# Kkuntal990/video-to-video-diffusion

Measured on AMD Instinct MI355X. Metric: ddim_steps_per_sec, higher is better.
Workload: dtype bf16; 1 GPU; DDIM-50 step (U-Net eval + update) on latent [1, 8, 48, 128, 128] = 8->48 slices @512x512, effective 264.66M U-Net (128x(1,2,4,4), latent 8), one volume per GPU, hipGraph-captured step; volumes_per_gpu=1, parallelism=dp1, full=False, finite_outputs=True

## Files before the change

include/ctsi.h:

```cpp
#ifndef CTSI_H
#define CTSI_H

#include <stddef.h>
#include <stdint.h>

#ifdef __cplusplus
extern "C" {
#endif

#define CTSI_OK 0
#define CTSI_ERR_INVALID (-1)
#define CTSI_ERR_UNSUPPORTED (-2)
#define CTSI_ERR_HIP (-3)

int ctsi_version(void);
int ctsi_ablation_build(void);
const char* ctsi_last_error(void);
int ctsi_device_available(void);

int ctsi_ncdhw_f32_to_ndhwc_bf16(const float* src, void* dst, int n, int c, int d, int h, int w,
                                 int c_total, int c_off, void* stream);
int ctsi_ndhwc_bf16_to_ncdhw_f32(const void* src, float* dst, int n, int c, int d, int h, int w,
                                 void* stream);
int ctsi_ncdhw_f32_to_ndhwc_f32(const float* src, float* dst, int n, int c, int d, int h, int w,
                                void* stream);
int ctsi_ndhwc_f32_to_ncdhw_f32(const float* src, float* dst, int n, int c, int d, int h, int w,
                                void* stream);

typedef struct ctsi_conv_plan ctsi_conv_plan;

typedef struct ctsi_conv_desc {
    int transposed;
    int kd, kh, kw;
    int sh, sw;
    int pd, ph, pw;
    int n, c1, c2;
    int cout;
    int di, hi, wi;
    int halo_d;
} ctsi_conv_desc;

typedef struct ctsi_conv_out {
    void* y;
    int mode;
    int cout_stride;
    int c_off;
    long long sn, sc, sd, sh, sw;
    int act;
    float* colsum;
    const void* gn_x;
    const double* gn_sums;
    const float* gn_gamma;
    const float* gn_beta;
    int gn_groups;
    float gn_eps;
    long long gn_count;
    int gn_silu;
    void* workspace;
} ctsi_conv_out;

int ctsi_conv_plan_create(ctsi_conv_plan** plan, const ctsi_conv_desc* desc);
int ctsi_conv_plan_set_weight_cin(ctsi_conv_plan* plan, int cin_w);
int ctsi_conv_plan_set_stream_tail(ctsi_conv_plan* plan, int on);
void ctsi_conv_plan_destroy(ctsi_conv_plan* plan);
int ctsi_conv_plan_out_dims(const ctsi_conv_plan* plan, int* d_out, int* h_out, int* w_out);
size_t ctsi_conv_plan_weight_bytes(const ctsi_conv_plan* plan);
int ctsi_conv_plan_tiles(const ctsi_conv_plan* plan);
int ctsi_conv_plan_tiles_per_sample(const ctsi_conv_plan* plan);
int ctsi_conv_plan_cout_pad(const ctsi_conv_plan* plan);
size_t ctsi_conv_plan_workspace_bytes(const ctsi_conv_plan* plan);
double ctsi_conv_plan_flops(const ctsi_conv_plan* plan);
int ctsi_conv_plan_config(const ctsi_conv_plan* plan, int* bm, int* bn, int* mode);
int ctsi_conv_plan_form(const ctsi_conv_plan* plan, int out[8]);
#define CTSI_PACK_GATHER 1
#define CTSI_PACK_GATHER_SMALL 2
#define CTSI_PACK_HALO 3
#define CTSI_PACK_K32 4
#define CTSI_PACK_HEAD 5
#define CTSI_PACK_STREAM_TAIL 6
#define CTSI_PACK_STEM 7
int ctsi_conv_plan_pack_layout(const ctsi_conv_plan* plan);
int ctsi_conv_plan_pack_weights(const ctsi_conv_plan* plan, const float* w_f32, void* packed,
                                void* stream);
int ctsi_conv_fwd(const ctsi_conv_plan* plan, const void* x1, const void* x2, const void* packed_w,
                  const float* bias, const ctsi_conv_out* out, void* stream);

int ctsi_gn_colsum(const void* x_bf16, float* colsum, int n, int c, int d, int h, int w,
                   int* tiles_per_sample, void* stream);
int ctsi_gn_colsum_tiles(int d, int h, int w);
int ctsi_gn_finalize(const float* colsum, double* sums, int n, int c, int c_pad, int groups,
                     int tiles_per_sample, int nclass, int accumulate, void* stream);
int ctsi_gn_apply(const void* x_bf16, void* y_bf16, const double* sums, const float* gamma,
                  const float* beta, int n, int c, int d, int h, int w, int d_stat, int groups, float eps,
                  int silu_pre, const float* tbias, int tbias_stride, const int* step_ptr,
                  const void* residual_bf16, int silu_post, void* stream);

int ctsi_attn_pv_supported(int c, int groups);
int ctsi_attn_pv(const float* depthsum, const double* sums, const float* gamma, const float* beta, const void* w_bf16,
                 const float* bias, void* out, int n, int c, int d, int h, int w, int groups, float eps, void* stream);

int ctsi_attn_depthsum(const void* x_bf16, float* depthsum, float* colsum, int n, int c, int d,
                       int h, int w, void* stream);
int ctsi_attn_depthsum_tiles(int c, int h, int w);
int ctsi_attn_normsum(const float* depthsum, const double* sums, const float* gamma,
                      const float* beta, void* out_bf16, int n, int c, int d, int h, int w,
                      int groups, float eps, void* stream);
int ctsi_attn_broadcast_add(const void* x_bf16, const void* p_bf16, const float* rowsum, int heads,
                            void* y_bf16, int n, int c, int d, int h, int w, void* stream);
int ctsi_attn_softmax_rowsum(const void* qk_bf16, float* rowsum, int n, int c, int d, int h, int w,
                             int heads, void* stream);

int ctsi_attn_core(const void* qkv_bf16, void* out_bf16, int n, int c, int d, int h, int w, int heads, void* stream);
int ctsi_attn_core_bwd(const void* qkv_bf16, const void* da_bf16, void* dqkv_bf16, int n, int c, int d, int h, int w, int heads,
                       void* stream);

int ctsi_attn_plane(const void* qkv_bf16, void* out_bf16, float* lse, int n, int c, int d, int h, int w, int heads, void* stream);
int ctsi_attn_plane_bwd(const void* qkv_bf16, const void* out_bf16, const void* da_bf16, const float* lse,
                        void* dqkv_bf16, int n, int c, int d, int h, int w, int heads, void* stream);

int ctsi_time_embed_fwd(const int* t_rows, int rows, int dim, int time_dim, const float* w1,
                        const float* b1, const float* w2, const float* b2, const float* w_all,
                        const float* b_all, int total_out, float* scratch, float* tbias_out,
                        void* stream);

int ctsi_time_embed_fwd_tf(const float* t_rows, int rows, int dim, int time_dim, const float* w1,
                           const float* b1, const float* w2, const float* b2, const float* w_all,
                           const float* b_all, int total_out, float* scratch, float* tbias_out,
                           void* stream);

int ctsi_trilinear_depth_fwd(const float* src_f32_ncdhw, void* dst_bf16_ndhwc, int n, int c,
                             int d_in, int d_out, int h, int w, int c_total, int c_off,
                             float* dst_f32_ncdhw, void* stream);

int ctsi_ddim_step(float* z, const float* eps, const float* noise_ncdhw, void* zin_bf16,
                   int c_total, int c_off, const float* coef, const int* step_ptr, int n, int c,
                   int d, int h, int w, int* nonfinite, void* stream);
int ctsi_ddpm_step(float* z, const float* eps, const float* noise_ncdhw, void* zin_bf16,
                   int c_total, int c_off, const float* coef, const int* step_ptr, int n, int c,
                   int d, int h, int w, void* stream);
int ctsi_ddpm_posterior(const float* z, const float* eps, const float* noise, float* z0_out, float* out,
                        const float* coef, int n, long long per_sample, int clip, void* stream);
int ctsi_step_advance(int* step_ptr, void* stream);
int ctsi_nan_to_num_f32(float* x, long long count, void* stream);
int ctsi_count_nonfinite_f32(float* x, long long count, int sanitize, int* counts, void* stream);

typedef struct ctsi_wgrad_desc {
    int kd, kh, kw;
    int sh, sw;
    int pd, ph, pw;
    int n;
    int dr, hr, wr;
    int dg, hg, wg;
    int cr, cr_stride;
    int cg, cg_stride;
} ctsi_wgrad_desc;
size_t ctsi_wgrad_workspace_bytes(const ctsi_wgrad_desc* desc);
double ctsi_wgrad_flops(const ctsi_wgrad_desc* desc);
int ctsi_wgrad(const ctsi_wgrad_desc* desc, const void* r, const void* g, void* workspace, size_t workspace_bytes, float* dw,
               long long stride_r, long long stride_g, long long stride_t, float scale, void* stream);

int ctsi_weight_dgrad_layout(const float* w, float* out, int cout, int cin, int taps, int ci_off, int ci_cnt,
                             void* stream);

int ctsi_linear_wgrad_multi(const void* entries, const void* blocks, int n_blocks, void* stream);

int ctsi_gn_bwd_tiles(int d, int h, int w);
size_t ctsi_gn_bwd_workspace_floats(int n, int c, int d, int h, int w, int groups);
int ctsi_gn_bwd(const void* x, const void* dy, int dy_bcast_d, const double* sums, const float* gamma,
                const float* beta, int n, int c, int d, int h, int w, int groups, float eps, int silu_pre,
                const void* residual, int silu_post, const void* add, void* g_buf, void* dx, float* workspace,
                float* dgamma, float* dbeta, float* dtbias, long long dtbias_stride, float* dxsum, void* stream);

size_t ctsi_channel_sum_workspace_floats(long long rows, int c);
int ctsi_channel_sum(const void* x, long long rows, int c, int c_stride, float* workspace, float* out, float scale,
                     void* stream);
int ctsi_add_bf16(void* a, const void* b, long long count, void* stream);
int ctsi_f32_to_bf16(const float* src, void* dst, long long count, void* stream);

int ctsi_vae_head_grad(const float* g, const float* y, int n, int c, int d, int h, int w, float scale, int mode, void* dst,
                       int c_stride, void* stream);
size_t ctsi_thin_wgrad_workspace_bytes(int n, int c, int d, int h, int w);
int ctsi_thin_wgrad_supported(int c, int w, int kd, int kh, int kw);
int ctsi_thin_wgrad(const void* wide, int c, int c_stride, const void* thin, int thin_stride, int head, int n, int d, int h,
                    int w, int kd, int kh, int kw, void* workspace, size_t workspace_bytes, float* dw, float scale,
                    void* stream);

int ctsi_q_sample(const float* z0, const float* noise, const float* sqrt_ac, const float* sqrt_1mac, const int* t,
                  void* dst, int n, int c, int d, int h, int w, int c_total, int c_off, void* stream);
size_t ctsi_mse_loss_workspace_doubles(int n);
int ctsi_mse_loss_fwd(const float* pred, const float* noise, const float* mask, const float* norm, int n, int c,
                      int d, int h, int w, double* workspace, float* loss_out, void* stream);
int ctsi_mse_loss_bwd(const float* pred, const float* noise, const float* mask, const float* norm,
                      const float* gscale, int n, int c, int d, int h, int w, void* dpred, int c_stride, void* stream);

int ctsi_time_embed_train_fwd(const int* t_rows, int rows, int dim, int time_dim, const float* w1, const float* b1,
                              const float* w2, const float* b2, const float* w_all, const float* b_all,
                              int total_out, float* scratch, float* tbias_out, void* stream);
int ctsi_linear_bwd(const float* x, const float* w, const float* dy, int rows, int in_dim, int out_dim, int silu_in,
                    float* dw, float* db, float* dx, void* stream);

int ctsi_blend_accumulate(float* acc, float* wsum, const float* patch, const float* wd, const float* wh,
                          const float* ww, int nc, int pd, int ph, int pw, int d_full, int h_full, int w_full,
                          int d0, int h0, int w0, void* stream);
int ctsi_blend_normalize(float* acc, const float* wsum, long long count, void* stream);

size_t ctsi_slice_metrics_workspace_doubles(int n, int c, int d, int h, int w);
int ctsi_slice_metrics(const float* a, const float* b, int n, int c, int d, int h, int w, int window, float max_val,
                       double* workspace, double* out, void* stream);

int ctsi_memset_async(void* ptr, int value, size_t bytes, void* stream);

int ctsi_adamw_chunk_elems(void);
int ctsi_adamw_multi(const void* tensors, const void* groups, const void* chunks, int nchunks, void* stream);
int ctsi_copy_scale_multi(const void* segs, const void* pieces, int npieces, void* stream);

int ctsi_ema_multi(const void* tensors, const void* weights, const void* chunks, int nchunks, void* stream);
int ctsi_swap_multi(const void* pairs, const void* chunks, int nchunks, void* stream);
int ctsi_grad_norm_multi(const void* tensors, const void* chunks, int nchunks, double* partials, void* stream);
int ctsi_grad_norm_finalize(const double* partials, int nchunks, float max_norm, float* out, void* stream);
int ctsi_grad_scale_multi(const void* tensors, const void* chunks, int nchunks, const float* dev_scale, void* stream);
int ctsi_adamw_ema_multi(const void* tensors, const void* groups, const void* chunks, int nchunks,
                         const float* dev_grad_scale, const float* ema_weights, void* stream);

size_t ctsi_msssim_workspace_bytes(int planes, int h, int w, int window, int want_grad);
int ctsi_msssim_fwd(const float* pred, const float* target, int planes, int h, int w, int window, int want_grad,
                    void* workspace, float* out, void* stream);
int ctsi_msssim_bwd(const float* pred, const float* target, int planes, int h, int w, int window, void* workspace,
                    const float* grad_loss, float* grad_pred, void* stream);

int ctsi_device_error_status(unsigned int* count, unsigned int* detail, int reset);

int ctsi_conv_f32_supported(const ctsi_conv_desc* desc);
size_t ctsi_conv_f32_weight_bytes(const ctsi_conv_desc* desc);
double ctsi_conv_f32_flops(const ctsi_conv_desc* desc);
int ctsi_conv_f32_geometry(const ctsi_conv_desc* desc, int* d_out, int* h_out, int* w_out, int* tiles_per_sample,
                           int* nclass, int* cout_pad);
int ctsi_conv_f32_pack_weights(const ctsi_conv_desc* desc, const float* w_f32, void* packed, void* stream);
int ctsi_conv_f32_fwd(const ctsi_conv_desc* desc, const float* x1, const float* x2, const void* packed_w, const float* bias,
                      const float* residual, const ctsi_conv_out* out, void* stream);
int ctsi_conv_bf16x3_supported(const ctsi_conv_desc* desc);
size_t ctsi_conv_bf16x3_weight_bytes(const ctsi_conv_desc* desc);
double ctsi_conv_bf16x3_flops(const ctsi_conv_desc* desc);
int ctsi_conv_bf16x3_geometry(const ctsi_conv_desc* desc, int* d_out, int* h_out, int* w_out, int* tiles_per_sample,
                              int* nclass, int* cout_pad);
int ctsi_conv_bf16x3_pack_weights(const ctsi_conv_desc* desc, const float* w_f32, void* packed, void* stream);
int ctsi_conv_bf16x3_fwd(const ctsi_conv_desc* desc, const float* x1, const float* x2, const void* packed_w, const float* bias,
                         const float* residual, const ctsi_conv_out* out, void* stream);
int ctsi_gn_colsum_f32_tiles(int d, int h, int w);
int ctsi_gn_colsum_f32(const float* x, float* colsum, int n, int c, int d, int h, int w, int* tiles_per_sample, void* stream);
int ctsi_gn_apply_f32(const float* x, float* y, const double* sums, const float* gamma, const float* beta, int n, int c,
                      int d, int h, int w, int d_stat, int groups, float eps, int silu_pre, const float* tbias,
                      int tbias_stride, const int* step_ptr, const float* residual, int silu_post, void* stream);
int ctsi_gn_apply_mod(const void* x_bf16, void* y_bf16, const double* sums, const float* gamma, const float* beta, int n,
                      int c, int d, int h, int w, int d_stat, int groups, float eps, int silu_pre, const float* tbias,
                      int tbias_stride, const int* step_ptr, const void* residual_bf16, int silu_post, int film,
                      int p_thr16, float inv_keep, const void* seed, int layer_id, void* stream);
int ctsi_gn_apply_mod_f32(const float* x, float* y, const double* sums, const float* gamma, const float* beta, int n, int c,
                          int d, int h, int w, int d_stat, int groups, float eps, int silu_pre, const float* tbias,
                          int tbias_stride, const int* step_ptr, const float* residual, int silu_post, int film,
                          void* stream);
size_t ctsi_gn_bwd_mod_workspace_floats(int n, int c, int d, int h, int w, int groups);
int ctsi_gn_bwd_mod(const void* x, const void* dy, const double* sums, const float* gamma, const float* beta, int n, int c,
                    int d, int h, int w, int groups, float eps, const float* tbias, int tbias_stride, int film, int p_thr16,
                    float inv_keep, const void* seed, int layer_id, void* dx, float* workspace, float* dgamma,
                    float* dbeta, float* dtbias, long long dtbias_stride, float* dxsum, void* stream);
int ctsi_dropout_mask(const void* seed, int layer_id, int p_thr16, long long count, void* out_u8, void* stream);
int ctsi_dropout_mask_host(unsigned long long seed, int layer_id, int p_thr16, long long count, void* out_u8);
int ctsi_philox4x32_10_host(const uint32_t* ctr, const uint32_t* key, uint32_t* out);
int ctsi_attn_depthsum_f32_tiles(int h, int w);
int ctsi_attn_depthsum_f32(const float* x, float* depthsum, float* colsum, int n, int c, int d, int h, int w, void* stream);
int ctsi_attn_normsum_f32(const float* depthsum, const double* sums, const float* gamma, const float* beta, float* out,
                          int n, int c, int d, int h, int w, int groups, float eps, void* stream);
int ctsi_attn_broadcast_add_f32(const float* x, const float* p, float* y, int n, int c, int d, int h, int w, void* stream);
int ctsi_ddim_step_f32(float* z, const float* eps, const float* noise, float* zin, int c_total, int c_off, const float* coef,
                       const int* step_ptr, int n, int c, int d, int h, int w, int* nonfinite, void* stream);
int ctsi_ddpm_step_f32(float* z, const float* eps, const float* noise, float* zin, int c_total, int c_off, const float* coef,
                       const int* step_ptr, int n, int c, int d, int h, int w, void* stream);

int ctsi_dpm_step(float* z, const float* eps, float* x0_prev, void* zin_bf16, int c_total, int c_off, const float* coef,
                  const int* step_ptr, int n, int c, int d, int h, int w, int* nonfinite, void* stream);
int ctsi_dpm_step_f32(float* z, const float* eps, float* x0_prev, float* zin, int c_total, int c_off, const float* coef,
                      const int* step_ptr, int n, int c, int d, int h, int w, int* nonfinite, void* stream);

int ctsi_heun_step(float* z, const float* eps, float* d1, const float* noise, void* zin_bf16, int c_total, int c_off,
                   const float* coef, const int* step_ptr, int n, int c, int d, int h, int w, int* nonfinite,
                   void* stream);
int ctsi_heun_step_f32(float* z, const float* eps, float* d1, const float* noise, float* zin, int c_total, int c_off,
                       const float* coef, const int* step_ptr, int n, int c, int d, int h, int w, int* nonfinite,
                       void* stream);

int ctsi_cfg_stats_blocks(long long per_sample);
int ctsi_cfg_combine(float* eps, const float* scale, const int* step_ptr, const double* stats, int n, int c, int d, int h,
                     int w, void* stream);
int ctsi_cfg_stats(const float* eps, const float* scale, const int* step_ptr, double* partials, int n, int c, int d, int h,
                   int w, void* stream);
int ctsi_cfg_stats_finalize(const double* partials, double* stats, int n, int c, int d, int h, int w, void* stream);
int ctsi_cfg_mirror(const void* src, void* dst, long long rows, int row_bytes, int stride_bytes, void* stream);

int ctsi_pred_to_eps(float* out, const float* z, const float* hist, const float* rows, const int* step_ptr,
                     int rows_per_step, int n, int z_rows, long long per_sample, void* stream);
int ctsi_q_sample_v(const float* z0, const float* noise, const float* sqrt_ac, const float* sqrt_1mac, const int* t,
                    void* dst, float* v_target, int n, int c, int d, int h, int w, int c_total, int c_off, void* stream);

int ctsi_x0_step(float* z, const float* v, float* hist, const float* noise_ncdhw, void* zin_bf16, int c_total, int c_off,
                 const float* coef, const int* step_ptr, int n, int c, int d, int h, int w, int* nonfinite, void* stream);
int ctsi_x0_step_f32(float* z, const float* v, float* hist, const float* noise_ncdhw, float* zin, int c_total, int c_off,
                     const float* coef, const int* step_ptr, int n, int c, int d, int h, int w, int* nonfinite,
                     void* stream);

int ctsi_sigma_split(const float* out2, float* eps, float* vraw, int n, int n_keep, int L, int d, int h, int w, void* stream);
int ctsi_ddpm_lv_step(float* z, const float* eps, const float* vraw, const float* noise_ncdhw, void* zin_bf16, int c_total,
                      int c_off, const float* coef, const int* step_ptr, int n, int c, int d, int h, int w, void* stream);
int ctsi_ddpm_lv_step_f32(float* z, const float* eps, const float* vraw, const float* noise_ncdhw, float* zin, int c_total,
                          int c_off, const float* coef, const int* step_ptr, int n, int c, int d, int h, int w, void* stream);
int ctsi_ddpm_posterior_lv(const float* z, const float* eps, const float* vraw, const float* noise, float* out,
                           float* logvar_out, const float* coef, int n, long long per_sample, void* stream);
size_t ctsi_hybrid_loss_workspace_doubles(int n);
int ctsi_hybrid_loss_fwd(const float* pred2, const float* z0, const float* noise, const int* t, const float* sched,
                         int timesteps, int v_pred, const float* mask, const float* norm, const float* norm_vb, int n, int L,
                         int d, int h, int w, double* workspace, float* loss_out, void* stream);
int ctsi_hybrid_loss_bwd(const float* pred2, const float* z0, const float* noise, const int* t, const float* sched,
                         int timesteps, int v_pred, const float* mask, const float* norm, const float* norm_vb,
                         const float* gscale, int n, int L, int d, int h, int w, void* dpred_bf16, int c_stride, void* stream);

int ctsi_vgg_prep(const float* x, const int* slices, const float* norm, void* dst, int b, int d, int num, int h, int w,
                  void* stream);
int ctsi_vgg_prep_bwd(const void* g, const int* slices, const float* norm, float* grad_pred, int b, int d, int num, int h,
                      int w, void* stream);
int ctsi_maxpool2_fwd(const void* x, void* y, int n, int h, int w, int c, void* stream);
int ctsi_maxpool2_bwd(const void* x, const void* gy, void* gx, int n, int h, int w, int c, void* stream);
int ctsi_relu_bf16(void* x, long long count, void* stream);
int ctsi_feat_loss_blocks(void);
int ctsi_feat_loss_fwd(const void* pred, const void* target, long long count, int squared, double* partials, void* stream);
int ctsi_feat_loss_finalize(const double* partials, const long long* counts, int layers, float* out, void* stream);
int ctsi_feat_grad_relu_bwd(const void* g_in, const void* y, const void* target, void* g_out, long long count, float coef,
                            int kind, int relu, const float* grad_loss, void* stream);

int ctsi_lpips_blocks(void);
int ctsi_lpips_prep(const float* x, void* dst, int n, int c, int h, int w, int normalize, void* stream);
int ctsi_lpips_prep_bwd(const void* g, float* grad, int n, int c, int h, int w, int normalize, void* stream);
int ctsi_lpips_dist_fwd(const void* y, const void* target, const float* w, int images, long long positions, int c,
                        double* partials, void* stream);
int ctsi_lpips_finalize(const double* partials, const long long* positions, int taps, int images, float* out,
                        float* tap_means, void* stream);
int ctsi_lpips_grad_relu_bwd(const void* g_in, const void* y, const void* target, const float* w, void* g_out, int images,
                             long long positions, int c, const float* grad_out, void* stream);

typedef struct ctsi_graph ctsi_graph;
int ctsi_graph_begin_capture(void* stream);
int ctsi_graph_end_capture(void* stream, ctsi_graph** graph);
int ctsi_graph_launch(ctsi_graph* graph, void* stream);
void ctsi_graph_destroy(ctsi_graph* graph);

int ctsi_window_gather(const void* src_bf16, void* dst_bf16, const int* starts, int batch, int halves, int nw, int D, int H,
                       int W, int td, int lh, int lw, int L, int src_c_total, int dst_c_total, void* stream);
int ctsi_window_gather_f32(const float* src, float* dst, const int* starts, int batch, int halves, int nw, int D, int H, int W,
                           int td, int lh, int lw, int L, int src_c_total, int dst_c_total, void* stream);
int ctsi_window_blend(const float* win, float* full, const int* tab_i, const float* tab_w, int batch, int halves, int nwd,
                      int nwh, int nww, int D, int H, int W, int td, int lh, int lw, int C, int kd, int kh, int kw, void* stream);

int ctsi_z0_pred(const float* z0, const float* noise, const float* pred, int c_stride, const float* sqrt_ac,
                 const float* sqrt_1mac, const int* t, const int* active, int v_prediction, int n, int c, int d, int h, int w,
                 float* out, void* stream);
int ctsi_loss_bwd_z0(const float* pred, const float* target, const float* mask, const float* norm, const float* gscale,
                     const float* g_z0, const int* active, const float* coef, int n, int c, int d, int h, int w, void* dpred,
                     int c_stride, void* stream);

typedef struct ctsi_event ctsi_event;
int ctsi_event_create(ctsi_event** ev);
int ctsi_event_record(ctsi_event* ev, void* stream);
int ctsi_stream_wait_event(void* stream, ctsi_event* ev);
int ctsi_event_elapsed_ms(ctsi_event* start, ctsi_event* stop, float* ms);
void ctsi_event_destroy(ctsi_event* ev);

int ctsi_depth_measure(const float* x, const float* W, const int* band, float* y_out, int planes, int d_in, int d_out,
                       int hw, void* stream);
int ctsi_depth_measure_adj(const float* g_y, const float* W, const int* band, float* g_x, float scale, int accumulate,
                           int planes, int d_in, int d_out, int hw, void* stream);
int ctsi_depth_project(float* x, const float* y, const float* W, const float* P, const int* band_w, const int* band_p,
                       int iters, float clamp_lo, float clamp_hi, int clamp_mode, double* partials, int planes, int d_in,
                       int d_out, int hw, void* stream);
int ctsi_depth_project_blocks(int planes, int hw);
int ctsi_depth_project_finalize(const double* partials, double* stats, int planes, int hw, int d_in, void* stream);

int ctsi_ensemble_accumulate(const float* x, int rows, long long count, int seen, float* mean, float* m2, void* stream);
int ctsi_ensemble_blocks(int planes, long long plane);
int ctsi_ensemble_finalize(const float* m2, float* std_out, int members, int unbiased, int planes, long long plane,
                           double* partials, double* stats, void* stream);
int ctsi_ensemble_calibration(const float* mean, const float* std_in, const float* target, int planes, long long plane,
                              double* partials, double* stats, void* stream);

int ctsi_guide_z0(const float* z_t, const float* eps, float alpha, float sigma, int mode, float clip, float* z0_out, int n,
                  int c, int d, int h, int w, void* stream);
int ctsi_depth_residual_adj(const float* x, const float* y, const float* W, const int* band, float* g_x, double* partials,
                            double* sumsq, int n, int c, int d_in, int d_out, int hw, void* stream);
int ctsi_guide_apply(float* z, float* hist, const float* g_z, const double* sumsq, float coef_z, float coef_hist,
                     int normalize, void* zin, int c_total, int c_off, int n, int c, int d, int h, int w, void* stream);

typedef struct ctsi_comm ctsi_comm;
int ctsi_comm_unique_id(void* id128);
int ctsi_comm_init(ctsi_comm** comm, const void* id128, int rank, int world);
void ctsi_comm_destroy(ctsi_comm* comm);
int ctsi_comm_rank(const ctsi_comm* comm);
int ctsi_comm_world(const ctsi_comm* comm);
int ctsi_halo_exchange(ctsi_comm* comm, const void* lo_own, const void* hi_own, void* lo_halo, void* hi_halo,
                       size_t bytes, void* stream);
int ctsi_halo_exchange_reduce(ctsi_comm* comm, const void* lo_own, const void* hi_own, void* lo_halo, void* hi_halo,
                              size_t bytes, double* sums, int nsums, float* f32, long long nf32, void* stream);
int ctsi_gn_allreduce(ctsi_comm* comm, double* sums, int nsums, float* f32, long long nf32, void* stream);
int ctsi_comm_allgather(ctsi_comm* comm, const void* send, void* recv, size_t bytes, void* stream);

#ifdef __cplusplus
}
#endif
#endif
```

video-to-video-diffusion_amd/csrc/conv3_halo_k32.hip:

```cpp
#include "conv3_halo_common.h"
#include <stdlib.h>
#include <type_traits>

template <int NJ, bool DIRECT>
__device__ __forceinline__ int hk_col(int j, int r16) { return DIRECT ? r16 * NJ + j : j * 16 + r16; }

template <int TD_, int TH_, int TW_ = 32, int BN_ = 128, int UPS_ = 2, bool PL_ = false>
struct HkCfg {
    static constexpr int TD = TD_, TH = TH_, TW = TW_, UPS = UPS_;
    static constexpr int HD = PL_ ? TD : TD + 2, HH = TH + 2, HW = TW + 2;
    static constexpr int HV = HD * HH * HW;
    static constexpr int HALO_INSTR = (HV + 31) / 32;
    static constexpr int HALO_BYTES = HALO_INSTR * 1024;
    static constexpr int BM = TD * TH * TW;
    static constexpr int BN = BN_;
    static constexpr int NJ = BN / 16;
    static constexpr int TAP_BYTES = BN * 32;
    static constexpr int STEP_TAPS = 2 * UPS;
    static constexpr int WSLOT_BYTES = STEP_TAPS * TAP_BYTES;
    static constexpr int NWS = 4;
    static constexpr int NWAVE = 8;
    static constexpr int MA = BM / 128;
    static constexpr int NTH = 64 * NWAVE;
    static constexpr int NPIECE = (HALO_INSTR + NWAVE - 1) / NWAVE;
    static constexpr int OFF_W = 2 * HALO_BYTES;
    static constexpr int LOOP_END = OFF_W + NWS * WSLOT_BYTES;
    static constexpr int BNP = BN + 8;
    static constexpr int OFF_ROW = LOOP_END > BM * BNP * 2 ? LOOP_END : BM * BNP * 2;
    static constexpr int OFF_CS = OFF_ROW + BM * 8;
    static constexpr int LDS_BYTES = OFF_CS + NWAVE * BN * 8;
    static constexpr int LPW = 64 / TW;
    static constexpr bool STRADDLE = TW % 16 != 0;
    static_assert(BM % 128 == 0 && (MA == 3 || (MA == 4 && TH % LPW == 0 && !STRADDLE)) && NPIECE <= 5 && LDS_BYTES <= 160 * 1024 &&
                      WSLOT_BYTES == 16384 && (UPS == 2 || UPS == 4), "unsupported tile");
    static constexpr int a_imm(int i) { return (((16 * i) / TW) * HW + (16 * i) % TW) * 32; }
};

__device__ __forceinline__ void hk_wait_vm(int allowed) {
    switch (allowed) {
        case 0: asm volatile("s_waitcnt vmcnt(0) lgkmcnt(0)" ::: "memory"); break;
        case 1: asm volatile("s_waitcnt vmcnt(1) lgkmcnt(0)" ::: "memory"); break;
        case 2: asm volatile("s_waitcnt vmcnt(2) lgkmcnt(0)" ::: "memory"); break;
        case 3: asm volatile("s_waitcnt vmcnt(3) lgkmcnt(0)" ::: "memory"); break;
        case 4: asm volatile("s_waitcnt vmcnt(4) lgkmcnt(0)" ::: "memory"); break;
        case 5: asm volatile("s_waitcnt vmcnt(5) lgkmcnt(0)" ::: "memory"); break;
        case 6: asm volatile("s_waitcnt vmcnt(6) lgkmcnt(0)" ::: "memory"); break;
        default: asm volatile("s_waitcnt vmcnt(7) lgkmcnt(0)" ::: "memory"); break;
    }
}

__device__ unsigned int g_hk_device_error[2] = {0u, 0u};
#define HK_NSTAMP 4096
__device__ unsigned long long g_hk_stamps[HK_NSTAMP][8];
#define HK_STAMP(K)                                                                                              \
    if ((CTSI_DBG(p.dbg, 4096)) && tid == 0 && blockIdx.x < HK_NSTAMP) g_hk_stamps[blockIdx.x][K] = __builtin_amdgcn_s_memtime();

template <int TD_, int TH_, int TW_ = 32, int BN_ = 128, int UPS_ = 2, bool TR = false, bool SK = false, bool DS = false, bool DIRECT = false>
__global__ void __attribute__((amdgpu_flat_work_group_size(1, 512)))
conv3_halo_k32_kernel(const Conv3HaloParams p) {
    constexpr bool PL = false, RELU = false;
#include "conv3_halo_k32_body.inc"
}

template <int TD_, int TH_, int TW_, bool RELU>
__global__ void __attribute__((amdgpu_flat_work_group_size(1, 512)))
conv3_planar_k32_kernel(const Conv3HaloParams p) {
    constexpr int BN_ = 128, UPS_ = 2;
    constexpr bool TR = false, SK = false, DS = false, DIRECT = true, PL = true;
#include "conv3_halo_k32_body.inc"
}

__global__ void conv3_halo_k32_pack_kernel(const float* __restrict__ w, bf16_t* __restrict__ out, int Cout, int CoutPad,
                                           int CinW, int nchunks, long long per_class, int form, int bn, int direct) {
    const bool transposed = form == 1;
    const int taps = form == 3 ? 9 : form ? 12 : 27;
    const int Q = nchunks * taps;
    const long long total = per_class * (transposed ? 4 : 1);
    for (long long idx = (long long)blockIdx.x * blockDim.x + threadIdx.x; idx < total;
         idx += (long long)gridDim.x * blockDim.x) {
        const int cls = (int)(idx / per_class);
        const long long in_class = idx - cls * per_class;
        const int e = (int)(in_class & 15);
        const long long row = in_class >> 4;
        const int co_p = (int)(row % CoutPad);
        const int co = direct ? (co_p / bn) * bn + (co_p % 16) * (bn / 16) + (co_p % bn) / 16 : co_p;
        const long long q = row / CoutPad;
        float v = 0.0f;
        if (q < Q) {
            const int t = (int)(q % taps), cc = (int)(q / taps);
            const int ci = (form == 2 ? (cc >> 2) : cc) * 16 + e;
            if (co < Cout && ci < CinW) {
                if (form == 2) {
                    const int py = (cc >> 1) & 1, px = cc & 1;
                    const int a = t >> 2, b = (t >> 1) & 1, c = t & 1;
                    v = w[((long long)co * CinW + ci) * 48 + (a * 4 + 2 * b + 1 - py) * 4 + 2 * c + 1 - px];
                } else if (transposed) {
                    const int py = cls >> 1, px = cls & 1;
                    const int a = 2 - (t >> 2), b = (t >> 1) & 1, c = t & 1;
                    const int ky = py ? (b ? 0 : 2) : (b ? 3 : 1), kx = px ? (c ? 0 : 2) : (c ? 3 : 1);
                    v = w[((long long)ci * Cout + co) * 48 + (a * 4 + ky) * 4 + kx];
                } else {
                    v = w[((long long)co * CinW + ci) * taps + t];
                }
            }
        }
        out[idx] = f32_to_bf16(v);
    }
}

extern "C" size_t ctsi_conv3_halo_k32_weight_bytes(int cin, int cout_pad, int bn, int form) {
    const long long q = (long long)(cin / 16) * (form == 3 ? 9 : form == 2 ? 48 : form == 1 ? 12 : 27), step = bn == 64 ? 8 : 4;
    return (size_t)(((q + step - 1) / step) * step * cout_pad * 32) * (form == 1 ? 4 : 1);
}

extern "C" int ctsi_conv3_halo_k32_pack(const float* w, void* packed, int cout, int cout_pad, int cin, int cin_w, int bn,
                                        int form, int direct, void* stream) {
    CTSI_CHECK_ARG(w && packed && cin % 16 == 0 && (bn == 64 || bn == 128) && cout_pad % bn == 0 && (form != 1 || cin_w == cin) &&
                       form >= 0 && form <= 3,
                   "ctsi_conv3_halo_k32_pack: bad arguments");
    const int nchunks = (cin / 16) * (form == 2 ? 4 : 1);
    const int transposed = form;
    const long long total = (long long)ctsi_conv3_halo_k32_weight_bytes(cin, cout_pad, bn, form) / 2;
    const long long per_class = form == 1 ? total / 4 : total;
    const int blocks = (int)((total + 255) / 256 > 4096 ? 4096 : (total + 255) / 256);
    hipLaunchKernelGGL(conv3_halo_k32_pack_kernel, dim3(blocks), dim3(256), 0, (hipStream_t)stream, w, (bf16_t*)packed,
                       cout, cout_pad, cin_w, nchunks, per_class, transposed, bn, direct);
    CTSI_LAUNCH_CHECK();
    return CTSI_OK;
}

extern "C" int ctsi_conv3_halo_k32_direct(int tile, int ksplit, int ds) {
#ifdef HK_STAGED_EPILOGUE
    return 0;
#else
    const bool t512 = tile == 0 || tile == 2, narrow = tile == 6 || tile == 7, planar = tile >= 16;
    return (t512 || narrow || planar || (tile == 5 && ksplit == 2 && !ds)) ? 1 : 0;
#endif
}

template <int TD, int TH, int TW, int BN, int UPS, bool TR, bool SK = false, bool DS = false>
static void hk_launch(const Conv3HaloParams* hp, hipStream_t stream) {
    using Cfg = HkCfg<TD, TH, TW, BN, UPS>;
#ifdef HK_STAGED_EPILOGUE
    constexpr bool DIRECT = false;
#else
    constexpr bool DIRECT = TD * TH * TW == 512 || TW == 24 || TW == 12 || (SK && !DS);
#endif
    auto k = conv3_halo_k32_kernel<TD, TH, TW, BN, UPS, TR, SK, DS, DIRECT>;
    static CtsiPerDeviceOnce attr_once;
    if (attr_once.first()) hipFuncSetAttribute((const void*)k, hipFuncAttributeMaxDynamicSharedMemorySize, 160 * 1024);
    hipLaunchKernelGGL(k, dim3((TR ? 4 : 1) * (SK ? 2 : 1) * hp->mtiles * hp->ntiles_n), dim3(Cfg::NTH), Cfg::LDS_BYTES, stream,
                       *hp);
}

extern "C" size_t ctsi_conv3_halo_k32_splitk_bytes(int tiles) {
    const size_t sync = ((size_t)tiles * 8 + 255) / 256 * 256;
    return sync + (size_t)tiles * (4 * 8 * 4) * 512 * sizeof(float);
}

extern "C" int ctsi_conv3_halo_k32_launch(const Conv3HaloParams* hp, int tile ,
                                          int bn, void* stream) {
    CTSI_CHECK_ARG(bn == 128 && (tile == 0 || tile == 2 || tile == 3 || tile == 5 || tile == 6 || tile == 7),
                   "ctsi_conv3_halo_k32_launch: bad BN %d / tile %d", bn, tile);
    if (tile == 6 || tile == 7) {
        CTSI_CHECK_ARG(!(hp->ds && hp->tr) && !(hp->ksplit == 2 && (hp->ds || hp->tr)),
                       "ctsi_conv3_halo_k32_launch: tile %d has no split-K form for strided / transposed layers", tile);
        if (hp->ksplit == 2) {
            CTSI_CHECK_ARG(hp->sk_ws && hp->sk_sync && hp->nchunks % 8 == 0, "ctsi_conv3_halo_k32_launch: split-K needs its workspace");
            if (tile == 6)
                hk_launch<4, 4, 24, 128, 2, false, true>(hp, (hipStream_t)stream);
            else
                hk_launch<8, 4, 12, 128, 2, false, true>(hp, (hipStream_t)stream);
        } else if (hp->ds) {
            CTSI_CHECK_ARG(hp->Hi == 2 * hp->Ho && hp->Wi == 2 * hp->Wo && hp->C2 == 0 && hp->nchunks % 4 == 0,
                           "ctsi_conv3_halo_k32_launch: the Downsample form needs even input planes and one source");
            if (tile == 6)
                hk_launch<4, 4, 24, 128, 2, false, false, true>(hp, (hipStream_t)stream);
            else
                hk_launch<8, 4, 12, 128, 2, false, false, true>(hp, (hipStream_t)stream);
        } else if (hp->tr) {
            if (tile == 6)
                hk_launch<4, 4, 24, 128, 2, true>(hp, (hipStream_t)stream);
            else
                hk_launch<8, 4, 12, 128, 2, true>(hp, (hipStream_t)stream);
        } else if (tile == 6) {
            hk_launch<4, 4, 24, 128, 2, false>(hp, (hipStream_t)stream);
        } else {
            hk_launch<8, 4, 12, 128, 2, false>(hp, (hipStream_t)stream);
        }
        CTSI_LAUNCH_CHECK();
        return CTSI_OK;
    }
    if (hp->ds) {
        CTSI_CHECK_ARG(!hp->tr && hp->Hi == 2 * hp->Ho && hp->Wi == 2 * hp->Wo && hp->C2 == 0 && hp->nchunks % 4 == 0,
                       "ctsi_conv3_halo_k32_launch: the Downsample form needs even input planes and one source");
        if (hp->ksplit == 2) {
            CTSI_CHECK_ARG(tile == 5 && hp->sk_ws && hp->sk_sync && hp->nchunks % 8 == 0, "ctsi_conv3_halo_k32_launch: split-K needs its workspace");
            hk_launch<3, 8, 16, 128, 2, false, true, true>(hp, (hipStream_t)stream);
        } else if (tile == 5) {
            hk_launch<3, 8, 16, 128, 2, false, false, true>(hp, (hipStream_t)stream);
        } else if (tile == 3) {
            hk_launch<3, 4, 32, 128, 2, false, false, true>(hp, (hipStream_t)stream);
        } else if (tile == 2) {
            hk_launch<4, 8, 16, 128, 2, false, false, true>(hp, (hipStream_t)stream);
        } else {
            hk_launch<4, 4, 32, 128, 2, false, false, true>(hp, (hipStream_t)stream);
        }
    } else if (hp->tr && tile == 5) {
        hk_launch<3, 8, 16, 128, 2, true>(hp, (hipStream_t)stream);
    } else if (hp->tr && tile == 3) {
        hk_launch<3, 4, 32, 128, 2, true>(hp, (hipStream_t)stream);
    } else if (tile == 5) {
        if (hp->ksplit == 2) {
            CTSI_CHECK_ARG(hp->sk_ws && hp->sk_sync && hp->nchunks % 8 == 0, "ctsi_conv3_halo_k32_launch: split-K needs its workspace");
            hk_launch<3, 8, 16, 128, 2, false, true>(hp, (hipStream_t)stream);
        } else {
            hk_launch<3, 8, 16, 128, 2, false, false>(hp, (hipStream_t)stream);
        }
    } else if (tile == 3) {
        hk_launch<3, 4, 32, 128, 2, false>(hp, (hipStream_t)stream);
    } else if (tile == 0 && hp->ksplit == 2) {
        CTSI_CHECK_ARG(hp->sk_ws && hp->sk_sync && hp->nchunks % 8 == 0, "ctsi_conv3_halo_k32_launch: split-K needs its workspace");
        hk_launch<4, 4, 32, 128, 2, false, true>(hp, (hipStream_t)stream);
    } else if (hp->tr) {
        if (tile == 2)
            hk_launch<4, 8, 16, 128, 2, true>(hp, (hipStream_t)stream);
        else
            hk_launch<4, 4, 32, 128, 2, true>(hp, (hipStream_t)stream);
    } else if (tile == 2) {
        hk_launch<4, 8, 16, 128, 2, false>(hp, (hipStream_t)stream);
    } else {
        hk_launch<4, 4, 32, 128, 2, false>(hp, (hipStream_t)stream);
    }
    CTSI_LAUNCH_CHECK();
    return CTSI_OK;
}

template <int TD, int TH, int TW>
static void hk_launch_planar(const Conv3HaloParams* hp, int relu, hipStream_t stream) {
    using Cfg = HkCfg<TD, TH, TW, 128, 2, true>;
    static CtsiPerDeviceOnce attr_once;
    if (attr_once.first()) {
        hipFuncSetAttribute((const void*)conv3_planar_k32_kernel<TD, TH, TW, false>, hipFuncAttributeMaxDynamicSharedMemorySize, 160 * 1024);
        hipFuncSetAttribute((const void*)conv3_planar_k32_kernel<TD, TH, TW, true>, hipFuncAttributeMaxDynamicSharedMemorySize, 160 * 1024);
    }
    const dim3 grid(hp->mtiles * hp->ntiles_n), block(Cfg::NTH);
    if (relu)
        hipLaunchKernelGGL((conv3_planar_k32_kernel<TD, TH, TW, true>), grid, block, Cfg::LDS_BYTES, stream, *hp);
    else
        hipLaunchKernelGGL((conv3_planar_k32_kernel<TD, TH, TW, false>), grid, block, Cfg::LDS_BYTES, stream, *hp);
}

extern "C" int ctsi_conv3_planar_k32_launch(const Conv3HaloParams* hp, int tile, int relu, void* stream) {
    CTSI_CHECK_ARG(tile >= 16 && tile <= 20, "ctsi_conv3_planar_k32_launch: bad tile %d", tile);
    CTSI_CHECK_ARG(!hp->tr && !hp->ds && hp->ksplit != 2 && hp->dshift == 0 && hp->colsum == nullptr && hp->Di == hp->Do &&
                       hp->Hi == hp->Ho && hp->Wi == hp->Wo && hp->C1 % 16 == 0 && hp->C2 % 16 == 0,
                   "ctsi_conv3_planar_k32_launch: the planar form is a plain stride-1 (1,3,3) conv without column sums");
    hipStream_t st = (hipStream_t)stream;
    switch (tile) {
    case 16: hk_launch_planar<1, 16, 32>(hp, relu, st); break;
    case 17: hk_launch_planar<2, 16, 16>(hp, relu, st); break;
    case 18: hk_launch_planar<4, 8, 16>(hp, relu, st); break;
    case 19: hk_launch_planar<4, 4, 24>(hp, relu, st); break;
    default: hk_launch_planar<8, 4, 12>(hp, relu, st); break;
    }
    CTSI_LAUNCH_CHECK();
    return CTSI_OK;
}

extern "C" int ctsi_debug_k32_stamps(unsigned long long* out, int nblocks) {
    if (nblocks > HK_NSTAMP) nblocks = HK_NSTAMP;
    CTSI_HIP(hipMemcpyFromSymbol(out, HIP_SYMBOL(g_hk_stamps), (size_t)nblocks * 8 * sizeof(unsigned long long)));
    return CTSI_OK;
}

extern "C" int ctsi_device_error_status(unsigned int* count, unsigned int* detail, int reset) {
    CTSI_CHECK_ARG(count, "ctsi_device_error_status: null argument");
    unsigned int h[2] = {0u, 0u};
    CTSI_HIP(hipMemcpyFromSymbol(h, HIP_SYMBOL(g_hk_device_error), sizeof(h)));
    *count = h[0];
    if (detail) *detail = h[1];
    if (reset && h[0]) {
        const unsigned int z[2] = {0u, 0u};
        CTSI_HIP(hipMemcpyToSymbol(HIP_SYMBOL(g_hk_device_error), z, sizeof(z)));
    }
    return CTSI_OK;
}
```

video-to-video-diffusion_amd/csrc/conv3_halo_k32_body.inc:

```
#if defined(__HIP_DEVICE_COMPILE__)
    using Cfg = HkCfg<TD_, TH_, TW_, BN_, UPS_, PL>;
    constexpr int UPS = Cfg::UPS, NJ = Cfg::NJ, NJH = Cfg::NJ / 2, STEP_TAPS = Cfg::STEP_TAPS;
    constexpr int TAPS = PL ? 9 : (TR || DS) ? 12 : 27;
    constexpr int DOFF = PL ? 0 : 1;
    static_assert(!(TR && DS) && !(PL && (TR || DS || SK)) && (PL || !RELU) && (!RELU || DIRECT), "one form at a time");
    constexpr int MA = Cfg::MA;
    constexpr int TH = Cfg::TH, TW = Cfg::TW, HH = Cfg::HH, HW = Cfg::HW, HV = Cfg::HV;
    constexpr int HALO_INSTR = Cfg::HALO_INSTR, HALO_BYTES = Cfg::HALO_BYTES, BM = Cfg::BM, BN = Cfg::BN;
    constexpr int TAP_BYTES = Cfg::TAP_BYTES, WSLOT_BYTES = Cfg::WSLOT_BYTES, NWS = Cfg::NWS, NWAVE = Cfg::NWAVE;
    constexpr int NTH = Cfg::NTH, NPIECE = Cfg::NPIECE, OFF_W = Cfg::OFF_W, OFF_ROW = Cfg::OFF_ROW, OFF_CS = Cfg::OFF_CS;
    constexpr int BNP = Cfg::BNP;
    extern __shared__ __attribute__((aligned(16))) char smem[];
    long long* s_rowoff = reinterpret_cast<long long*>(smem + OFF_ROW);
    float* s_cs = reinterpret_cast<float*>(smem + OFF_CS);

    const int tid = threadIdx.x;
    const int lane = tid & 63;
    const int wave = __builtin_amdgcn_readfirstlane(tid >> 6);

    HK_STAMP(0);
    if ((CTSI_DBG(p.dbg, 4096)) && tid == 0 && blockIdx.x < HK_NSTAMP)
        g_hk_stamps[blockIdx.x][7] = ((unsigned long long)__builtin_amdgcn_s_getreg((31 << 11) | (0 << 6) | 20) << 32) |
                                     (unsigned)__builtin_amdgcn_s_getreg((31 << 11) | (0 << 6) | 4);
    int bid = xcd_remap_h(blockIdx.x, gridDim.x);
    const int khalf = SK ? (bid & 1) : 0;
    if (SK) bid >>= 1;
    int mt, nt, cls = 0;
    if (TR) {
        const int ns = 4 * p.ntiles_n;
        const int G = (p.n_major > 0 && p.n_major < ns && ns % p.n_major == 0) ? p.n_major : ns;
        const int per_g = p.mtiles * G;
        const int sg = bid / per_g;
        const int rem = bid - sg * per_g;
        mt = rem / G;
        const int sib = sg * G + (rem - mt * G);
        cls = sib / p.ntiles_n;
        nt = sib - cls * p.ntiles_n;
    } else {
        h3_decode_tile(bid, p.mtiles, p.ntiles_n, p.n_major, &mt, &nt);
    }
    const int py = cls >> 1, px = cls & 1;
    const int n0 = nt * BN;
    const int nchunks = SK ? p.nchunks / 2 : p.nchunks;
    const int cbase = khalf * nchunks;
    const int nb = mt / p.tps;
    int r0 = mt - nb * p.tps;
    int tD, tH, tW;
    if (p.tile_order == 1) {
        tH = r0 / (p.tilesD * p.tilesW);
        r0 -= tH * p.tilesD * p.tilesW;
        tD = r0 / p.tilesW;
        tW = r0 - tD * p.tilesW;
    } else if (p.tile_order == 2 && (p.tilesW & 3) == 0 && (p.tilesH & 7) == 0) {
        tD = r0 / (p.tilesH * p.tilesW);
        r0 -= tD * p.tilesH * p.tilesW;
        const int st = r0 >> 5, in = r0 & 31, spr = p.tilesW >> 2;
        tW = (st % spr) * 4 + (in & 3);
        tH = (st / spr) * 8 + (in >> 2);
    } else {
        tD = r0 / (p.tilesH * p.tilesW);
        r0 -= tD * p.tilesH * p.tilesW;
        tH = r0 / p.tilesW;
        tW = r0 - tH * p.tilesW;
    }
    const int d0 = tD * Cfg::TD, h0 = tH * TH, w0 = tW * TW;

    int dlo = d0 + p.dshift - DOFF;
    dlo = dlo < 0 ? 0 : dlo;
    const long long basevox = ((long long)(nb * p.Di + dlo) * p.Hi) * p.Wi;
    const v4i_t rs1 = h3_make_rsrc(reinterpret_cast<const char*>(p.x1) + basevox * p.C1 * 2, 0x7fffffffu);
    const v4i_t rs2 = h3_make_rsrc(reinterpret_cast<const char*>(p.x2) + basevox * p.C2 * 2, 0x7fffffffu);
    const long long w_class = (long long)((p.nchunks * TAPS + STEP_TAPS - 1) / STEP_TAPS) * STEP_TAPS * p.CoutPad * 32;
    const v4i_t rsw = h3_make_rsrc(reinterpret_cast<const char*>(p.w) + cls * w_class + (long long)n0 * 32 +
                                       (long long)cbase * TAPS * p.CoutPad * 32, 0x7fffffffu);
    const unsigned lds0 = (unsigned)(unsigned long long)(lptr3_t)smem;

    const int C1 = p.C1, C2 = p.C2, CoutPad = p.CoutPad;
    const int Q = nchunks * TAPS;
    const int S = (Q + STEP_TAPS - 1) / STEP_TAPS;
    const unsigned w_voff = (unsigned)lane * 16u;
    auto issue_weights = [&](int s) {
        const unsigned slot = lds0 + OFF_W + (s % NWS) * WSLOT_BYTES;
#pragma unroll
        for (int k = 0; k < 2; ++k) {
            const int piece = wave + NWAVE * k;
            constexpr int PPT = TAP_BYTES / 1024;
            const int e = piece / PPT, quarter = piece % PPT;
            const unsigned soff = (unsigned)__builtin_amdgcn_readfirstlane(((s * STEP_TAPS + e) * CoutPad) * 32 + quarter * 1024);
            const unsigned dst = (unsigned)__builtin_amdgcn_readfirstlane((int)(slot + piece * 1024));
            h3_dma16(rsw, dst, w_voff, soff);
        }
    };

    const bool has_bias = p.bias != nullptr && khalf == 0;
    if (has_bias && wave == 0) {
        const int left = p.Cout - n0;
        const v4i_t rsb = h3_make_rsrc(p.bias + n0, (unsigned)(left > 0 ? left * 4 : 0));
        h3_dma16(rsb, (unsigned)__builtin_amdgcn_readfirstlane((int)(lds0 + OFF_CS)), (unsigned)lane * 16u, 0u);
    }
    if (S > 0) issue_weights(0);

    int hrel[NPIECE];
#pragma unroll
    for (int i = 0; i < NPIECE; ++i) {
        const int j = wave + NWAVE * i;
        const int v = j * 32 + (lane >> 1);
        const int hd = v / (HH * HW), rem = v - hd * (HH * HW);
        const int hh = rem / HW, hw = rem - hh * HW;
        const int gd = d0 + p.dshift - DOFF + hd, gh = h0 - 1 + hh, gw = w0 - 1 + hw;
        if (DS) {
            const bool ok = (j < HALO_INSTR) && (v < HV) && gd >= 0 && gd < p.Di && gh >= 0 && gh < p.Ho && gw >= 0 && gw < p.Wo;
            hrel[i] = ok ? ((gd - dlo) * p.Hi + 2 * gh) * p.Wi + 2 * gw : -1;
        } else {
            const bool ok = (j < HALO_INSTR) && (v < HV) && gd >= 0 && gd < p.Di && gh >= 0 && gh < p.Hi && gw >= 0 && gw < p.Wi;
            hrel[i] = ok ? ((gd - dlo) * p.Hi + gh) * p.Wi + gw : -1;
        }
    }
    const unsigned hq16 = (unsigned)((lane & 1) * 16);

    auto issue_halo = [&](int cc, int i) -> int {
        const int j = wave + NWAVE * i;
        if (j >= HALO_INSTR) return 0;
        const int vc = cbase + cc;
        const int ch0 = (DS ? (vc >> 2) : vc) * 16;
        const int cadd = DS ? ((vc >> 1) & 1) * p.Wi + (vc & 1) : 0;
        const bool second = ch0 >= C1;
        const unsigned cbytes = (unsigned)((second ? C2 : C1) * 2);
        const unsigned soff = (unsigned)__builtin_amdgcn_readfirstlane((second ? ch0 - C1 : ch0) * 2);
        int hsel = hrel[0];
#pragma unroll
        for (int q = 1; q < NPIECE; ++q) {
            int cand = hrel[q];
            asm("" : "+v"(cand));
            hsel = (i == q) ? cand : hsel;
        }
        const unsigned voff = hsel >= 0 ? (unsigned)(hsel + cadd) * cbytes + hq16 : 0x80000000u;
        const unsigned dst = (unsigned)__builtin_amdgcn_readfirstlane((int)(lds0 + (cc & 1) * HALO_BYTES + j * 1024));
        if (second)
            h3_dma16(rs2, dst, voff, soff);
        else
            h3_dma16(rs1, dst, voff, soff);
        return 1;
    };
    const int r16 = lane & 15, kg = lane >> 4;
    const bool tap1 = kg >= 2;
    constexpr bool VPERM = DIRECT && TR;
    const int v16 = VPERM ? 4 * (r16 & 3) + (r16 >> 2) : r16;
    int a_lane, b_lane;
    int aoff[MA];
    {
        auto hv = [&](int row) {
            const int line = row / TW, wofs = row % TW;
            return ((line / TH) * HH + (line % TH)) * HW + wofs;
        };
        const int row0 = wave * 16 * MA;
        const int vbase = hv(row0);
        if constexpr (Cfg::STRADDLE) {
            const int v0 = hv(row0 + v16);
#pragma unroll
            for (int i = 0; i < MA; ++i) aoff[i] = (hv(row0 + 16 * i + v16) - v0) * 32;
            a_lane = v0 * 32 + (kg & 1) * 16;
        } else {
#pragma unroll
            for (int i = 0; i < MA; ++i) {
                if constexpr (MA == 4)
                    aoff[i] = Cfg::a_imm(i);
                else
                    aoff[i] = (hv(row0 + 16 * i) - vbase) * 32;
            }
            a_lane = (vbase + v16) * 32 + (kg & 1) * 16;
        }
        b_lane = OFF_W + (kg >> 1) * TAP_BYTES + r16 * 32 + (kg & 1) * 16;
    }
    auto tap_off = [&](int q) -> int {
        q = q < Q ? q : Q - 1;
        const int cc = q / TAPS, t = q - cc * TAPS;
        int kd, kh, kw;
        if (TR) {
            kd = t >> 2;
            kh = ((t >> 1) & 1) ? (py ? 2 : 0) : 1;
            kw = (t & 1) ? (px ? 2 : 0) : 1;
        } else if (DS) {
            kd = t >> 2;
            kh = ((t >> 1) & 1) + 1 - ((cc >> 1) & 1);
            kw = (t & 1) + 1 - (cc & 1);
        } else if (PL) {
            kd = 0;
            kh = t / 3;
            kw = t - kh * 3;
        } else {
            kd = t / 9;
            const int t2 = t - kd * 9;
            kh = t2 / 3;
            kw = t2 - kh * 3;
        }
        return (cc & 1) * HALO_BYTES + ((kd * HH + kh) * HW + kw) * 32;
    };

    f32x4 acc[MA][NJ];

    bf16x8 fa0[MA], fa1[MA], fbl[NJH], fbh[NJH];

#define HK_LOAD_A(FA, I0, AADDR)                                                                               \
    {                                                                                                          \
        _Pragma("unroll") for (int i_ = (I0); i_ < ((I0) == 0 ? 2 : MA); ++i_)                                 \
            FA[i_] = *reinterpret_cast<const bf16x8*>(smem + (AADDR) + aoff[i_]);                              \
    }
#define HK_LOAD_B(FB, J0, BADDR, UU)                                                                           \
    {                                                                                                          \
        _Pragma("unroll") for (int j_ = 0; j_ < NJH; ++j_)                                                     \
            FB[j_] = *reinterpret_cast<const bf16x8*>(smem + (BADDR) + (UU) * 2 * TAP_BYTES + ((J0) + j_) * 512); \
    }
#define HK_MFMA(FA, FB, J0)                                                                                    \
    {                                                                                                          \
        _Pragma("unroll") for (int j_ = 0; j_ < NJH; ++j_) _Pragma("unroll") for (int i_ = 0; i_ < MA; ++i_)    \
            acc[i_][(J0) + j_] = __builtin_amdgcn_mfma_f32_16x16x32_bf16(FA[i_], FB[j_], acc[i_][(J0) + j_], 0, 0, 0); \
    }
#define HK_SCHED()                                                                                             \
    {                                                                                                          \
        __builtin_amdgcn_sched_group_barrier(0x002, 4, 0);                                                     \
        _Pragma("unroll") for (int q_ = 0; q_ < NJH + 2; ++q_) {                                               \
            __builtin_amdgcn_sched_group_barrier(0x008, 1, 0);                                                 \
            __builtin_amdgcn_sched_group_barrier(0x100, 1, 0);                                                 \
        }                                                                                                      \
        __builtin_amdgcn_sched_group_barrier(0x008, MA * NJH - (NJH + 2), 0);                                  \
        __builtin_amdgcn_sched_barrier(0);                                                                     \
    }

#pragma unroll
    for (int i = 0; i < NPIECE; ++i) issue_halo(0, i);
    int n_trail = 0;
#pragma unroll
    for (int s = 1; s < NWS - 1; ++s)
        if (s < S) {
            issue_weights(s);
            n_trail += 2;
        }
    if (tid < BM) {
        const int mm = tid % TW, line = tid / TW;
        const int d = d0 + line / TH, h = h0 + line % TH, w = w0 + mm;
        long long off = -1;
        if (TR) {
            if (d < p.Do && 2 * h < p.Ho && 2 * w < p.Wo)
                off = ((((long long)nb * p.Do + d) * p.Ho + 2 * h + py) * p.Wo + 2 * w + px) * p.cout_stride + p.c_off;
        } else if (d < p.Do && h < p.Ho && w < p.Wo) {
            off = ((((long long)nb * p.Do + d) * p.Ho + h) * p.Wo + w) * p.cout_stride + p.c_off;
        }
        s_rowoff[tid] = off;
    }

    int n_late = 0;
    {
        constexpr int NEED = (Cfg::TD * HH * HW + 31) / 32;
#pragma unroll
        for (int i = 0; i < NPIECE; ++i) n_late += (wave + NWAVE * i >= NEED && wave + NWAVE * i < HALO_INSTR) ? 1 : 0;
    }
    hk_wait_vm(n_trail == 4 ? n_trail + n_late : n_trail);
    __syncthreads();
    HK_STAMP(1);
#pragma unroll
    for (int j = 0; j < NJ; ++j) {
        const float bv = has_bias ? s_cs[hk_col<NJ, DIRECT>(j, r16)] : 0.0f;
#pragma unroll
        for (int i = 0; i < MA; ++i)
#pragma unroll
            for (int q = 0; q < 4; ++q) acc[i][j][q] = bv;
    }
    {
        const int oa = tap_off(0), ob = tap_off(1);
        const int aaddr = a_lane + (tap1 ? ob : oa);
        HK_LOAD_A(fa0, 0, aaddr);
        HK_LOAD_A(fa0, 2, aaddr);
        HK_LOAD_B(fbl, 0, b_lane, 0);
    }
    if (CTSI_DBG(p.dbg, 128)) {
#pragma unroll
        for (int j = 0; j < NJH; ++j) fbh[j] = fbl[j];
    }
    __builtin_amdgcn_sched_barrier(0);

    int n_prev = n_trail == 4 ? 2 : 0;
    int hc = 1, hp = 0, hfree = 0;
    constexpr int H_FIRST = PL ? NPIECE : (UPS == 2 && !TR && !DS) ? 2 : 3, H_LATER = PL ? NPIECE : (UPS == 2 && !TR && !DS) ? 1 : 3;
    auto issue_group = [&](int s) {
        int n_halo = 0, n_w = 0;
        bool urgent = false;
        if (hc < nchunks && s >= hfree && !(CTSI_DBG(p.dbg, 1))) {
            urgent = s + 2 >= ((TAPS * hc) >> 1) / UPS;
            const int cnt = hp == 0 ? H_FIRST : H_LATER;
#pragma unroll
            for (int k = 0; k < (H_FIRST > H_LATER ? H_FIRST : H_LATER); ++k)
                if (k < cnt && hp < NPIECE) {
                    n_halo += issue_halo(hc, hp);
                    ++hp;
                }
            if (hp >= NPIECE) {
                hp = 0;
                hfree = ((TAPS * hc - 1) >> 1) / UPS;
                ++hc;
            }
        }
        if (s + NWS - 1 < S && !(CTSI_DBG(p.dbg, 2))) {
            issue_weights(s + NWS - 1);
            n_w = 2;
        }
        n_prev = urgent ? n_w : n_w + n_halo;
        __builtin_amdgcn_sched_barrier(0);
    };
#define HK_UNIT(FAc, FAn, BADDR, UU, BADDR_N, UU_N, AADDR_N, MID)                                              \
    {                                                                                                          \
        if (!(CTSI_DBG(p.dbg, 128))) HK_LOAD_B(fbh, NJH, BADDR, UU);    \
        HK_LOAD_A(FAn, 0, AADDR_N);                                                                            \
        HK_MFMA(FAc, fbl, 0);                                                                                  \
        HK_SCHED();                                                                                            \
        MID;                                                                                                   \
        HK_LOAD_A(FAn, 2, AADDR_N);                                                                            \
        HK_LOAD_B(fbl, 0, BADDR_N, UU_N);                                                                      \
        HK_MFMA(FAc, fbh, NJH);                                                                                \
        HK_SCHED();                                                                                            \
    }
    for (int s = 0; s < S; ++s) {
        const int baddr = b_lane + (s % NWS) * WSLOT_BYTES;
        const int baddr_n = b_lane + ((s + 1) % NWS) * WSLOT_BYTES;
        const int q0 = STEP_TAPS * s;
        int an[UPS];
#pragma unroll
        for (int k = 0; k < UPS; ++k) {
            const int oa = tap_off(q0 + 2 * k + 2), ob = tap_off(q0 + 2 * k + 3);
            an[k] = a_lane + (tap1 ? ob : oa);
        }
        HK_UNIT(fa0, fa1, baddr, 0, baddr, 1, an[0], );
        if constexpr (UPS == 4) {
            HK_UNIT(fa1, fa0, baddr, 1, baddr, 2, an[1], );
            HK_UNIT(fa0, fa1, baddr, 2, baddr, 3, an[2], );
        }
        hk_wait_vm(n_prev);
        if (!(CTSI_DBG(p.dbg, 64))) __builtin_amdgcn_s_barrier();
        __builtin_amdgcn_sched_barrier(0);
        HK_UNIT(fa1, fa0, baddr, UPS - 1, baddr_n, 0, an[UPS - 1], if (wave < 4 || (CTSI_DBG(p.dbg, 16))) issue_group(s));
        if (wave >= 4 && !(CTSI_DBG(p.dbg, 16))) issue_group(s);
    }
#undef HK_UNIT
#undef HK_LOAD_A
#undef HK_LOAD_B
#undef HK_MFMA
#undef HK_SCHED
    HK_STAMP(2);
    asm volatile("s_waitcnt vmcnt(0) lgkmcnt(0)" ::: "memory");
    if (!(DIRECT && !SK) || (p.dbg_epi_barrier != 0)) __syncthreads();
    HK_STAMP(3);

    if (CTSI_DBG(p.dbg, 8)) return;
    if (SK) {
        const int tile = mt * p.ntiles_n + nt;
        constexpr int NREG = MA * NJ * 4;
        float* wsl = p.sk_ws + (size_t)tile * NREG * NTH + tid;
        int* s_role = reinterpret_cast<int*>(s_cs);
        if (tid == 0) {
            const int tk = __hip_atomic_fetch_add(p.sk_sync + 2 * tile, 1, __ATOMIC_RELAXED, __HIP_MEMORY_SCOPE_AGENT);
            if (tk >= 2) {
                atomicAdd(&g_hk_device_error[0], 1u);
                g_hk_device_error[1] = (unsigned)tile;
            }
            *s_role = tk & 1;
        }
        __syncthreads();
        const int role = *s_role;
        __syncthreads();
        if (role == 0) {
#pragma unroll
            for (int i = 0; i < MA; ++i)
#pragma unroll
                for (int j = 0; j < NJ; ++j)
#pragma unroll
                    for (int q = 0; q < 4; ++q)
                        __hip_atomic_store(wsl + (size_t)((i * NJ + j) * 4 + q) * NTH, acc[i][j][q], __ATOMIC_RELAXED,
                                           __HIP_MEMORY_SCOPE_AGENT);
            asm volatile("s_waitcnt vmcnt(0)" ::: "memory");
            __syncthreads();
            if (tid == 0) __hip_atomic_store(p.sk_sync + 2 * tile + 1, 1, __ATOMIC_RELAXED, __HIP_MEMORY_SCOPE_AGENT);
            return;
        }
        if (tid == 0) {
            int spins = 0;
            while (__hip_atomic_load(p.sk_sync + 2 * tile + 1, __ATOMIC_RELAXED, __HIP_MEMORY_SCOPE_AGENT) == 0 && spins < (1 << 22)) {
                __builtin_amdgcn_s_sleep(4);
                ++spins;
            }
            if (spins >= (1 << 22)) {
                atomicAdd(&g_hk_device_error[0], 1u);
                g_hk_device_error[1] = (unsigned)tile;
            } else {
                __hip_atomic_store(p.sk_sync + 2 * tile, 0, __ATOMIC_RELAXED, __HIP_MEMORY_SCOPE_AGENT);
                __hip_atomic_store(p.sk_sync + 2 * tile + 1, 0, __ATOMIC_RELAXED, __HIP_MEMORY_SCOPE_AGENT);
            }
        }
        __syncthreads();
#pragma unroll
        for (int i = 0; i < MA; ++i)
#pragma unroll
            for (int j = 0; j < NJ; ++j)
#pragma unroll
                for (int q = 0; q < 4; ++q)
                    acc[i][j][q] += __hip_atomic_load(wsl + (size_t)((i * NJ + j) * 4 + q) * NTH, __ATOMIC_RELAXED,
                                                      __HIP_MEMORY_SCOPE_AGENT);
    }
    bf16_t* s_tile = reinterpret_cast<bf16_t*>(smem);
    const bool want_sums = p.colsum != nullptr;
    unsigned vbits = 0;
#pragma unroll
    for (int i = 0; i < MA; ++i)
#pragma unroll
        for (int q = 0; q < 4; ++q)
            vbits |= (unsigned)(s_rowoff[wave * 16 * MA + 16 * i + (VPERM ? 4 * q + kg : 4 * kg + q)] >= 0) << (4 * i + q);
    auto tile_out = [&](auto masked_tag, auto sums_tag) {
        constexpr bool MASKED = decltype(masked_tag)::value, SUMS = decltype(sums_tag)::value;
#pragma unroll
        for (int j = 0; j < NJ; ++j) {
            const int col = hk_col<NJ, DIRECT>(j, r16);
            float s1 = 0.0f, s2 = 0.0f;
#pragma unroll
            for (int i = 0; i < MA; ++i) {
                bf16_t* trow = s_tile + (wave * 16 * MA + 16 * i + 4 * kg) * BNP + col;
#pragma unroll
                for (int q = 0; q < 4; q += 2) {
                    const float v0 = acc[i][j][q], v1 = acc[i][j][q + 1];
                    const uint32_t pk = pack_bf16x2_v(f32x2_t{v0, v1});
                    trow[q * BNP] = (bf16_t)(pk & 0xffffu);
                    trow[(q + 1) * BNP] = (bf16_t)(pk >> 16);
                    if (SUMS) {
                        const float m0 = (!MASKED || ((vbits >> (4 * i + q)) & 1u)) ? v0 : 0.0f;
                        const float m1 = (!MASKED || ((vbits >> (4 * i + q + 1)) & 1u)) ? v1 : 0.0f;
                        s1 += m0;
                        s2 = __builtin_fmaf(m0, m0, s2);
                        s1 += m1;
                        s2 = __builtin_fmaf(m1, m1, s2);
                    }
                }
            }
            if (SUMS) {
                s1 += __shfl_xor(s1, 16);
                s2 += __shfl_xor(s2, 16);
                s1 += __shfl_xor(s1, 32);
                s2 += __shfl_xor(s2, 32);
                if (kg == 0) {
                    s_cs[(wave * BN + col) * 2 + 0] = s1;
                    s_cs[(wave * BN + col) * 2 + 1] = s2;
                }
            }
        }
    };
    bf16_t* y = reinterpret_cast<bf16_t*>(p.y);
    if constexpr (DIRECT) {
        static_assert(NJ == 8, "a lane's couts of one voxel are one 16-byte piece");
        const int co = n0 + r16 * NJ;
        const bool co_ok = co < p.Cout;
        auto direct_out = [&](auto masked_tag, auto sums_tag) {
            constexpr bool MASKED = decltype(masked_tag)::value, SUMS = decltype(sums_tag)::value;
            float s1[NJ], s2[NJ];
#pragma unroll
            for (int j = 0; j < NJ; ++j) s1[j] = s2[j] = 0.0f;
#pragma unroll
            for (int i = 0; i < MA; ++i)
#pragma unroll
                for (int q = 0; q < 4; ++q) {
                    const long long off = s_rowoff[wave * 16 * MA + 16 * i + (VPERM ? 4 * q + kg : 4 * kg + q)];
                    if (SUMS) {
                        const bool live = !MASKED || ((vbits >> (4 * i + q)) & 1u);
#pragma unroll
                        for (int j = 0; j < NJ; ++j) {
                            const float m = live ? acc[i][j][q] : 0.0f;
                            s1[j] += m;
                            s2[j] = __builtin_fmaf(m, m, s2[j]);
                        }
                    }
                    if (off >= 0 && co_ok && !(CTSI_DBG(p.dbg, 4))) {
                        typedef unsigned int u4_t __attribute__((ext_vector_type(4)));
                        u4_t w4;
                        auto out_v = [](float v) { return RELU ? __builtin_fmaxf(v, 0.0f) : v; };
                        w4.x = pack_bf16x2_v(f32x2_t{out_v(acc[i][0][q]), out_v(acc[i][1][q])});
                        w4.y = pack_bf16x2_v(f32x2_t{out_v(acc[i][2][q]), out_v(acc[i][3][q])});
                        w4.z = pack_bf16x2_v(f32x2_t{out_v(acc[i][4][q]), out_v(acc[i][5][q])});
                        w4.w = pack_bf16x2_v(f32x2_t{out_v(acc[i][6][q]), out_v(acc[i][7][q])});
                        if (p.nt_store)
                            __builtin_nontemporal_store(w4, reinterpret_cast<u4_t*>(y + off + co));
                        else
                            *reinterpret_cast<u4_t*>(y + off + co) = w4;
                    }
                }
            if (SUMS) {
#pragma unroll
                for (int j = 0; j < NJ; ++j) {
                    float a1 = s1[j], a2 = s2[j];
                    a1 += __shfl_xor(a1, 16);
                    a2 += __shfl_xor(a2, 16);
                    a1 += __shfl_xor(a1, 32);
                    a2 += __shfl_xor(a2, 32);
                    if (kg == 0) {
                        s_cs[(wave * BN + r16 * NJ + j) * 2 + 0] = a1;
                        s_cs[(wave * BN + r16 * NJ + j) * 2 + 1] = a2;
                    }
                }
            }
        };
        using T = std::true_type;
        using F = std::false_type;
        const bool ragged = __builtin_amdgcn_ballot_w64(vbits != (1u << (4 * MA)) - 1u) != 0ull;
        if (!want_sums) direct_out(F{}, F{});
        else if (ragged) direct_out(T{}, T{});
        else direct_out(F{}, T{});
    } else {
        using T = std::true_type;
        using F = std::false_type;
        const bool ragged = __builtin_amdgcn_ballot_w64(vbits != (1u << (4 * MA)) - 1u) != 0ull;
        if (!want_sums) tile_out(F{}, F{});
        else if (ragged) tile_out(T{}, T{});
        else tile_out(F{}, T{});
    }
    HK_STAMP(4);
    constexpr int CPR = BN / 8;
    if constexpr (!DIRECT) {
        constexpr int RPW = 16 * MA;
#pragma unroll 4
        for (int k = 0; k < RPW * CPR / 64; ++k) {
            const int c = k * 64 + lane;
            const int row = wave * RPW + c / CPR, ch = c % CPR;
            const long long off = s_rowoff[row];
            const int co = n0 + ch * 8;
            if (off >= 0 && co < p.Cout && !(CTSI_DBG(p.dbg, 4))) {
                const uint4 v = *reinterpret_cast<const uint4*>(s_tile + row * BNP + ch * 8);
                if (p.nt_store) {
                    typedef unsigned int u4_t __attribute__((ext_vector_type(4)));
                    const u4_t w4 = {v.x, v.y, v.z, v.w};
                    __builtin_nontemporal_store(w4, reinterpret_cast<u4_t*>(y + off + co));
                } else {
                    *reinterpret_cast<uint4*>(y + off + co) = v;
                }
            }
        }
    }
    HK_STAMP(5);
    if (want_sums) {
        __syncthreads();
        if (tid < BN) {
            const int col = tid;
            float t1 = 0.0f, t2 = 0.0f;
#pragma unroll
            for (int q = 0; q < NWAVE; ++q) {
                t1 += s_cs[(q * BN + col) * 2 + 0];
                t2 += s_cs[(q * BN + col) * 2 + 1];
            }
            const long long slab = (long long)(TR ? 4 : 1) * p.mtiles * CoutPad;
            const long long tg = (long long)cls * p.mtiles + mt;
            p.colsum[tg * CoutPad + n0 + col] = t1;
            p.colsum[slab + tg * CoutPad + n0 + col] = t2;
        }
    }
    HK_STAMP(6);
#endif
```

video-to-video-diffusion_amd/csrc/conv_mfma.hip:

```cpp
#include <type_traits>
#include "conv3_halo_common.h"
#include "conv_plan.h"
#include <string.h>
#include <stdlib.h>
#include <math.h>


__device__ __attribute__((aligned(256))) uint32_t g_ctsi_zero_page[64];

struct ConvKParams {
    const bf16_t* x1;
    const bf16_t* x2;
    const bf16_t* w;
    const float* bias;
    void* y;
    float* colsum;
    int C1, C2, Cin;
    int Di, Hi, Wi;
    int Dr, Hr, Wr;
    int sH, sW;
    int lTH, lTW;
    int linear;
    int tilesD, tilesH, tilesW, tps, mtiles;
    int ntiles_n;
// ... 509 lines not shown
            if (var < 0.0) var = 0.0;
            const float rstd = (float)(1.0 / sqrt(var + (double)p.gn_eps));
            sc = p.gn_gamma[co] * rstd;
            sh = p.gn_beta[co] - (float)mean * sc;
        }
        s_cs[tid] = sc;
        s_cs[BN + tid] = sh;
    }
    __syncthreads();
    if (p.colsum != nullptr && tid < BN) {
        float t1 = 0.0f, t2 = 0.0f;
#pragma unroll
        for (int m = 0; m < WM; ++m) {
            t1 += s_cs[(m * BN + tid) * 2 + 0];
            t2 += s_cs[(m * BN + tid) * 2 + 1];
        }
        const long long tg = (long long)cls * p.mtiles + mt;
        const long long slab = (long long)p.nclass * p.mtiles * p.CoutPad;
        p.colsum[tg * p.CoutPad + n0 + tid] = t1;
        p.colsum[slab + tg * p.CoutPad + n0 + tid] = t2;
    }
    if (p.out_mode == 0) {
        constexpr int CPR = BN / 8;
        constexpr int ITER = (BM * CPR) / NTH;
        static_assert((BM * CPR) % NTH == 0, "store loop assumes whole iterations");
        bf16_t* y = reinterpret_cast<bf16_t*>(p.y);
        if (p.gn_x != nullptr) {
            uint4 hreg[ITER];
#pragma unroll
            for (int it = 0; it < ITER; ++it) {
                const int c = tid + it * NTH;
                const int row = c / CPR, cc = c - row * CPR;
                const long long off = s_rowoff[row];
                const int co = n0 + cc * 8;
                hreg[it] = (off >= 0 && co < p.Cout) ? *reinterpret_cast<const uint4*>(p.gn_x + off + co)
                                                     : make_uint4(0, 0, 0, 0);
            }
            static_assert(NTH % CPR == 0, "a thread's chunk must not depend on the iteration");
            const int cc0 = tid % CPR;
            float gsc[8], gsh[8];
            *reinterpret_cast<float4*>(gsc) = *reinterpret_cast<const float4*>(s_cs + cc0 * 8);
            *reinterpret_cast<float4*>(gsc + 4) = *reinterpret_cast<const float4*>(s_cs + cc0 * 8 + 4);
            *reinterpret_cast<float4*>(gsh) = *reinterpret_cast<const float4*>(s_cs + BN + cc0 * 8);
            *reinterpret_cast<float4*>(gsh + 4) = *reinterpret_cast<const float4*>(s_cs + BN + cc0 * 8 + 4);
            auto tail = [&](auto silu_tag) {
                constexpr bool SILU = decltype(silu_tag)::value;
#pragma unroll
                for (int it = 0; it < ITER; ++it) {
                    const int c = tid + it * NTH;
                    const int row = c / CPR, cc = c - row * CPR;
                    const long long off = s_rowoff[row];
                    const int co = n0 + cc * 8;
                    if (off >= 0 && co < p.Cout) {
                        const uint4 v = *reinterpret_cast<const uint4*>(s_tile + row * BN + cc * 8);
                        const uint4 h = hreg[it];
                        const uint32_t hw[4] = {h.x, h.y, h.z, h.w}, rw[4] = {v.x, v.y, v.z, v.w};
                        uint32_t ow[4];
#pragma unroll
                        for (int k = 0; k < 4; ++k) {
                            f32x2_t a = {__uint_as_float(hw[k] << 16), __uint_as_float(hw[k] & 0xffff0000u)};
                            a = a * f32x2_t{gsc[2 * k], gsc[2 * k + 1]} + f32x2_t{gsh[2 * k], gsh[2 * k + 1]} +
                                f32x2_t{__uint_as_float(rw[k] << 16), __uint_as_float(rw[k] & 0xffff0000u)};
                            if (SILU) a = silu2_f(a);
                            ow[k] = pack_bf16x2_v(a);
                        }
                        *reinterpret_cast<uint4*>(y + off + co) = make_uint4(ow[0], ow[1], ow[2], ow[3]);
                    }
                }
            };
            if (p.gn_silu) tail(std::true_type{});
            else tail(std::false_type{});
        } else {
            for (int c = tid; c < BM * CPR; c += NTH) {
                const int row = c / CPR, cc = c - row * CPR;
                const long long off = s_rowoff[row];
                const int co = n0 + cc * 8;
                if (off >= 0 && co < p.Cout && !(CTSI_DBG_RT(p.dbg, 1))) {
                    const uint4 v = *reinterpret_cast<const uint4*>(s_tile + row * BN + cc * 8);
                    *reinterpret_cast<uint4*>(y + off + co) = v;
                }
            }
        }
    }
#endif
}

struct PackParams {
    const float* w;
    bf16_t* out;
    int nclass, T, Cout, CoutPad, Cin, CinW, Ktot, small, kc_per_tap, lcpt;
    long long s_co, s_ci;
    int tapk[CTSI_MAX_TAPS];
};

__global__ void conv_pack_weights_kernel(const PackParams q) {
    const long long total = (long long)q.nclass * q.CoutPad * q.Ktot;
    for (long long idx = (long long)blockIdx.x * blockDim.x + threadIdx.x; idx < total;
         idx += (long long)gridDim.x * blockDim.x) {
        const int k = (int)(idx % q.Ktot);
        const long long rc = idx / q.Ktot;
        const int co = (int)(rc % q.CoutPad);
        const int cls = (int)(rc / q.CoutPad);
        int tap, ci;
        if (q.small) {
            const int g = k >> 3;
            tap = g >> q.lcpt;
            ci = ((g & ((1 << q.lcpt) - 1)) << 3) + (k & 7);
        } else {
            const int s = k >> 6;
            tap = s % q.T;
            ci = (s / q.T) * 64 + (k & 63);
        }
        float v = 0.0f;
        if (tap < q.T && ci < q.CinW && co < q.Cout)
            v = q.w[(long long)co * q.s_co + (long long)ci * q.s_ci + q.tapk[cls * q.T + tap]];
        q.out[idx] = f32_to_bf16(v);
    }
}

extern "C" int ctsi_conv_plan_pack_weights(const ctsi_conv_plan* p, const float* w, void* packed,
                                           void* stream) {
    CTSI_CHECK_ARG(p && w && packed, "ctsi_conv_plan_pack_weights: null argument");
    if (p->stem) return ctsi_conv3_stem_pack(w, packed, p->d.cout, p->CoutPad, p->CinW, stream);
    if (p->stream1) return ctsi_conv1_stream_pack(w, packed, p->d.cout, p->Cin, p->CinW, p->stream1, stream);
    const ConvFamily family = conv_family(p);
    if (family == CONV_K32)
        return ctsi_conv3_halo_k32_pack(w, packed, p->d.cout, p->CoutPad, p->Cin, p->CinW, p->BN, conv_k32_image(p),
                                        conv_k32_direct(p), stream);
    if (family == CONV_HEAD) {
        hipMemsetAsync((char*)packed + head1_bytes(p) - 1280, 0, 1280, (hipStream_t)stream);
        if (ctsi_conv3_head2_supported(p->Cin, p->d.cout)) {
            const int rc = ctsi_conv3_head2_pack(w, (char*)packed + head1_bytes(p), p->d.cout, p->Cin, p->CinW, stream);
            if (rc != CTSI_OK) return rc;
        }
        return ctsi_conv3_halo_pack(w, packed, p->d.cout, p->d.cout <= 8 ? 8 : 16, p->Cin, p->CinW, stream);
    }
    if (family == CONV_HALO32) return ctsi_conv3_halo_pack(w, packed, p->d.cout, p->CoutPad, p->Cin, p->CinW, stream);
    PackParams q;
    memset(&q, 0, sizeof(q));
    q.w = w;
    q.out = (bf16_t*)packed;
    q.nclass = p->nclass;
    q.T = p->T;
    q.Cout = p->d.cout;
    q.CoutPad = p->CoutPad;
    q.Cin = p->Cin;
    q.CinW = p->CinW;
    q.Ktot = p->Ktot;
    q.small = p->small;
    q.kc_per_tap = p->kc_per_tap;
    q.lcpt = p->lcpt;
    const long long KK = (long long)p->d.kd * p->d.kh * p->d.kw;
    if (!p->d.transposed) {
        q.s_co = (long long)p->CinW * KK;
        q.s_ci = KK;
    } else {
        q.s_ci = (long long)p->d.cout * KK;
        q.s_co = KK;
    }
    memcpy(q.tapk, p->tapk, sizeof(q.tapk));
    const long long total = (long long)q.nclass * q.CoutPad * q.Ktot;
    const int blocks = (int)((total + 255) / 256 > 4096 ? 4096 : (total + 255) / 256);
    hipLaunchKernelGGL(conv_pack_weights_kernel, dim3(blocks), dim3(256), 0, (hipStream_t)stream, q);
    CTSI_LAUNCH_CHECK();
    return CTSI_OK;
}

template <int WM, int WN, int TM, int TN>
static int launch_conv(const ConvKParams& k, int mode, int grid, hipStream_t st) {
    constexpr int BM = WM * TM * 32, BN = WN * TN * 32;
    constexpr size_t lds = 2 * (BM * 128 + BN * 128) + BM * 8 + WM * BN * 8;
    constexpr int STAGE = BM * 128 + BN * 128;
    constexpr int NSTG = STAGE <= 32768 ? 4 : (STAGE <= 49152 ? 3 : 2);
    constexpr size_t lds_ring = (size_t)NSTG * STAGE + BM * 8 + WM * BN * 8;
    static CtsiPerDeviceOnce attr_once;
    if (attr_once.first()) {
        hipFuncSetAttribute((const void*)conv_gather_mfma_kernel<WM, WN, TM, TN, 3>,
                            hipFuncAttributeMaxDynamicSharedMemorySize, (int)lds_ring);
        hipFuncSetAttribute((const void*)conv_gather_mfma_kernel<WM, WN, TM, TN, 0>,
                            hipFuncAttributeMaxDynamicSharedMemorySize, (int)lds);
        hipFuncSetAttribute((const void*)conv_gather_mfma_kernel<WM, WN, TM, TN, 1>,
                            hipFuncAttributeMaxDynamicSharedMemorySize, (int)lds);
        hipFuncSetAttribute((const void*)conv_gather_mfma_kernel<WM, WN, TM, TN, 2>,
                            hipFuncAttributeMaxDynamicSharedMemorySize, (int)lds);
    }
    const dim3 g(grid), b(WM * WN * 64);
    if (mode == 1)
        hipLaunchKernelGGL((conv_gather_mfma_kernel<WM, WN, TM, TN, 1>), g, b, lds, st, k);
    else if (mode == 3)
        hipLaunchKernelGGL((conv_gather_mfma_kernel<WM, WN, TM, TN, 3>), g, b, lds_ring, st, k);
    else if (mode == 2)
        hipLaunchKernelGGL((conv_gather_mfma_kernel<WM, WN, TM, TN, 2>), g, b, lds, st, k);
    else
        hipLaunchKernelGGL((conv_gather_mfma_kernel<WM, WN, TM, TN, 0>), g, b, lds, st, k);
    CTSI_LAUNCH_CHECK();
    return CTSI_OK;
}

extern "C" int ctsi_conv_fwd(const ctsi_conv_plan* p, const void* x1, const void* x2, const void* packed_w,
                             const float* bias, const ctsi_conv_out* o, void* stream) {
    CTSI_CHECK_ARG(p && x1 && packed_w && o && o->y, "ctsi_conv_fwd: null argument");
    CTSI_CHECK_ARG(p->d.c2 == 0 || x2 != nullptr, "ctsi_conv_fwd: plan has two sources but x2 is null");
    CTSI_CHECK_ARG(o->mode == 0 || o->mode == 1, "ctsi_conv_fwd: bad output mode %d", o->mode);
    if (o->mode == 0) {
        CTSI_CHECK_ARG(p->d.cout % 8 == 0 && o->cout_stride % 8 == 0 && o->c_off % 8 == 0 &&
                           o->cout_stride >= o->c_off + p->d.cout,
                       "ctsi_conv_fwd: bf16 output needs cout, cout_stride, c_off multiples of 8 "
                       "(cout=%d stride=%d off=%d)", p->d.cout, o->cout_stride, o->c_off);
    }
    const ConvFamily family = conv_family(p);
    CTSI_CHECK_ARG(o->act != 2 || (p->planar && o->mode == 0 && o->colsum == nullptr && o->gn_x == nullptr),
                   "ctsi_conv_fwd: the ReLU epilogue (act = 2) exists on planar (1,3,3) halo-tile plans with plain bf16 output "
                   "only (ctsi_conv_plan_form: bit 16 of out[4])");
    CTSI_CHECK_ARG(!p->planar || o->colsum == nullptr, "ctsi_conv_fwd: a planar (1,3,3) halo-tile plan writes no column sums");
    if (p->stem && o->mode == 0 && o->act == 0 && o->gn_x == nullptr) {
        StemParams q;
        memset(&q, 0, sizeof(q));
        q.x = (const bf16_t*)x1;
        q.w = (const bf16_t*)packed_w;
        q.bias = bias;
        q.y = (bf16_t*)o->y;
        q.colsum = (float*)o->colsum;
        q.cx = p->d.c1;
        q.D = p->d.di; q.H = p->d.hi; q.W = p->d.wi;
        q.Cout = p->d.cout; q.CoutPad = p->CoutPad;
        q.cout_stride = o->cout_stride; q.c_off = o->c_off;
        q.tilesD = p->tilesD; q.tilesH = p->tilesH; q.tilesW = p->tilesW; q.tps = p->tps; q.mtiles = p->mtiles;
        return ctsi_conv3_stem_launch(&q, stream);
    }
    CTSI_CHECK_ARG(!p->stem, "ctsi_conv_fwd: a one-channel stem plan writes bf16 without activation or fused tail");
    if (p->stream1) {
        CTSI_CHECK_ARG(o->mode == 0 && o->act == 0 && o->colsum == nullptr,
                       "ctsi_conv_fwd: a streaming 1x1x1 plan writes bf16 without activation or column sums");
        Conv1StreamParams q;
        memset(&q, 0, sizeof(q));
        q.x1 = (const bf16_t*)x1;
        q.x2 = (const bf16_t*)(x2 ? x2 : x1);
        q.w = (const bf16_t*)packed_w;
        q.bias = bias;
        q.h = (const bf16_t*)o->gn_x;
        q.y = (bf16_t*)o->y;
        if (o->gn_x != nullptr) {
            CTSI_CHECK_ARG(o->gn_sums && o->gn_gamma && o->gn_beta && o->gn_groups > 0 && p->d.cout % o->gn_groups == 0 &&
                               o->gn_count > 0,
                           "ctsi_conv_fwd: bad fused GroupNorm arguments (groups=%d, cout=%d)", o->gn_groups, p->d.cout);
            q.gn_sums = (const double*)o->gn_sums;
            q.gn_gamma = (const float*)o->gn_gamma;
            q.gn_beta = (const float*)o->gn_beta;
            q.gn_groups = o->gn_groups;
            q.gn_eps = o->gn_eps;
            q.gn_count = (double)o->gn_count;
            q.gn_silu = o->gn_silu;
        }
        q.C1 = p->d.c1; q.C2 = p->d.c2; q.Cout = p->d.cout;
        q.cout_stride = o->cout_stride; q.c_off = o->c_off;
        q.V = (long long)p->Do * p->Ho * p->Wo;
        return ctsi_conv1_stream_launch(&q, p->d.n, p->stream1, stream);
    }
    if (o->gn_x != nullptr) {
        CTSI_CHECK_ARG(!p->form && o->mode == 0 && o->act == 0 && o->colsum == nullptr && p->nclass == 1,
                       "ctsi_conv_fwd: the fused GroupNorm tail needs a gather-kernel plan, bf16 output, no act / colsum");
        CTSI_CHECK_ARG(o->gn_sums && o->gn_gamma && o->gn_beta && o->gn_groups > 0 && p->d.cout % o->gn_groups == 0 &&
                           o->gn_count > 0,
                       "ctsi_conv_fwd: bad fused GroupNorm arguments (groups=%d, cout=%d)", o->gn_groups, p->d.cout);
    }
    if (p->form && (family == CONV_HEAD || (o->mode == 0 && (o->act == 0 || o->act == 2)))) {
        Conv3HaloParams h;
        memset(&h, 0, sizeof(h));
        h.x1 = (const bf16_t*)x1;
        h.x2 = (const bf16_t*)(x2 ? x2 : x1);
        h.w = (const bf16_t*)packed_w;
        h.bias = bias;
        h.y = o->y;
        h.colsum = o->colsum;
        h.C1 = p->d.c1; h.C2 = p->d.c2;
        h.Di = p->d.di; h.Hi = p->d.hi; h.Wi = p->d.wi;
        h.Do = p->Do; h.Ho = p->Ho; h.Wo = p->Wo;
        h.dshift = p->dshift;
        h.tilesD = p->tilesD; h.tilesH = p->tilesH; h.tilesW = p->tilesW; h.tps = p->tps; h.mtiles = p->mtiles;
        h.ntiles_n = p->ntiles_n;
        h.nchunks = p->Cin / (family == CONV_K32 ? 16 : 32) * (p->ds ? 4 : 1);
        h.ds = p->ds;
        h.Cout = p->d.cout; h.CoutPad = p->CoutPad;
        h.cout_stride = o->cout_stride; h.c_off = o->c_off;
        {
            static const char* nts = getenv("CTSI_CONV_NT_STORE");
            const long long out_bytes = (long long)p->d.n * p->Do * p->Ho * p->Wo * o->cout_stride * 2;
            h.nt_store = nts ? atoi(nts) != 0 : out_bytes >= (128ll << 20);
        }
        {
            const char* nm = getenv("CTSI_CONV_NMAJOR");
            h.n_major = nm ? atoi(nm) : 0;
            if (p->d.transposed && !nm) h.n_major = 4;
        }
        {
            h.dbg = ctsi_debug_flags();
            h.nchunks = ctsi_debug_ksteps(h.nchunks);
        }
        {
            const char* to = getenv("CTSI_CONV_TILE_ORDER");
            h.tile_order = to ? atoi(to) : 2;
            const char* eb = getenv("CTSI_CONV_EPI_BARRIER");
            h.dbg_epi_barrier = eb ? atoi(eb) : 0;
        }
        if (family == CONV_HEAD) {
            if (p->head2 && o->colsum == nullptr)
                return ctsi_conv3_head2_launch(&h, p->d.n, (const char*)packed_w + head1_bytes(p), o->mode, o->act, o->sn, o->sc, o->sd,
                                               o->sh, o->sw, stream);
            return ctsi_conv3_head_launch(&h, p->d.cout <= 8 ? 8 : 16, o->mode, o->act, o->sn, o->sc, o->sd, o->sh, o->sw, stream);
        }
        h.tr = p->d.transposed;
        if (family == CONV_K32 && p->ksplit == 2) {
            CTSI_CHECK_ARG(o->workspace, "ctsi_conv_fwd: this plan needs ctsi_conv_out.workspace (ctsi_conv_plan_workspace_bytes)");
            const int tiles = p->mtiles * p->ntiles_n;
            h.ksplit = 2;
            h.sk_sync = (int*)o->workspace;
            h.sk_ws = (float*)((char*)o->workspace + ((size_t)tiles * 8 + 255) / 256 * 256);
        }
        if (p->planar) return ctsi_conv3_planar_k32_launch(&h, p->form->code, o->act == 2, stream);
        if (family == CONV_K32) return ctsi_conv3_halo_k32_launch(&h, p->form->code, p->BN, stream);
        return ctsi_conv3_halo_launch(&h, p->form->code, stream);
    }
    CTSI_CHECK_ARG(!p->form, "ctsi_conv_fwd: the 3x3x3 halo-tile plan supports bf16 NDHWC output without activation");
    ConvKParams k;
    memset(&k, 0, sizeof(k));
    k.x1 = (const bf16_t*)x1;
    k.x2 = (const bf16_t*)(x2 ? x2 : x1);
    k.w = (const bf16_t*)packed_w;
    k.bias = bias;
    k.y = o->y;
    k.colsum = o->colsum;
    k.C1 = p->d.c1; k.C2 = p->d.c2; k.Cin = p->Cin;
    k.Di = p->d.di; k.Hi = p->d.hi; k.Wi = p->d.wi;
    k.Dr = p->Dr; k.Hr = p->Hr; k.Wr = p->Wr;
    k.sH = p->sH; k.sW = p->sW;
    k.lTH = p->lTH; k.lTW = p->lTW;
    k.linear = p->linear;
    k.tilesD = p->tilesD; k.tilesH = p->tilesH; k.tilesW = p->tilesW; k.tps = p->tps; k.mtiles = p->mtiles;
    k.ntiles_n = p->ntiles_n;
    k.T = p->T; k.ksteps = p->ksteps; k.kc_per_tap = p->kc_per_tap; k.lcpt = p->lcpt;
    k.Cout = p->d.cout; k.CoutPad = p->CoutPad; k.Ktot = p->Ktot;
    k.Do = p->Do; k.Ho = p->Ho; k.Wo = p->Wo; k.uH = p->uH; k.uW = p->uW;
    k.nclass = p->nclass;
    k.out_mode = o->mode; k.cout_stride = o->cout_stride; k.c_off = o->c_off; k.act = o->act;
    k.osn = o->sn; k.osc = o->sc; k.osd = o->sd; k.osh = o->sh; k.osw = o->sw;
    memcpy(k.tapdelta, p->tapdelta, sizeof(k.tapdelta));
    k.NA = p->NA; k.NB = p->NB; k.NC = p->NC;
    memcpy(k.ad, p->ad, sizeof(k.ad));
    memcpy(k.bh, p->bh, sizeof(k.bh));
    memcpy(k.cw, p->cw, sizeof(k.cw));
    for (int c = 0; c < 4; ++c) { k.pH[c] = p->pH[c]; k.pW[c] = p->pW[c]; }
    int grid = p->nclass * p->mtiles * p->ntiles_n;
    if (p->gsplit >= 2 && o->workspace != nullptr && !(p->BM != 128 || p->BN != 128)) {
        const size_t tiles = (size_t)grid;
        k.ksplit = p->gsplit;
        k.sk_sync = (int*)o->workspace;
        k.sk_ws = (float*)((char*)o->workspace + (tiles * 4 + 255) / 256 * 256);
        grid *= p->gsplit;
    }
    hipStream_t st = (hipStream_t)stream;
    k.ksteps = ctsi_debug_ksteps(k.ksteps);
    k.dbg = ctsi_debug_flags();
    k.gn_x = (const bf16_t*)o->gn_x;
    k.gn_sums = o->gn_sums;
    k.gn_gamma = o->gn_gamma;
    k.gn_beta = o->gn_beta;
    k.gn_groups = o->gn_groups;
    k.gn_silu = o->gn_silu;
    k.gn_eps = o->gn_eps;
    k.gn_count = (double)o->gn_count;
    k.dshift = p->dshift;
    memcpy(k.tap_margin, p->tap_margin, sizeof(k.tap_margin));
    memcpy(k.ad_min, p->ad_min, sizeof(k.ad_min));
    int mode = p->small ? 1 : (p->fast ? 2 : 0);
    {
        const char* ring = getenv("CTSI_CONV_RING");
        const bool small_grid = grid <= 256 && !(p->BM == 256 && p->BN == 256);
        if (mode == 2 && ((small_grid && !(ring && !strcmp(ring, "0"))) || (ring && !strcmp(ring, "1")))) mode = 3;
    }
    if (p->BM == 256 && p->BN == 256) return launch_conv<2, 4, 4, 2>(k, mode, grid, st);
    if (p->BM == 256 && p->BN == 128) return launch_conv<4, 2, 2, 2>(k, mode, grid, st);
    if (p->BN == 128) return launch_conv<2, 2, 2, 2>(k, mode, grid, st);
    return launch_conv<4, 1, 1, 1>(k, mode, grid, st);
}
```

video-to-video-diffusion_amd/csrc/conv_plan.h:

```cpp
#pragma once
#include "ctsi_internal.h"

#define CTSI_MAX_TAPS 48
#define CTSI_BK 64

enum ConvFamily {
    CONV_GATHER,
    CONV_HALO32,
    CONV_K32,
    CONV_HEAD,
};

struct ConvForm {
    ConvFamily family;
    int mode;
    int td, th, tw;
    int bn;
    int code;
    double eff;
    const char* name;
};

struct ctsi_conv_plan {
    ctsi_conv_desc d;
    int Cin, CinW;
    int Do, Ho, Wo;
    int Dr, Hr, Wr, sH, sW, uH, uW;
    int nclass, T;
    int small, lcpt, kc_per_tap, ksteps, Ktot;
    int BM, BN, CoutPad, ntiles_n;
    int lTH, lTW, TD, TH, TW, tilesD, tilesH, tilesW, tps, mtiles;
    int linear;
    int tapk[CTSI_MAX_TAPS];
    int tapdelta[CTSI_MAX_TAPS];
    int8_t od[CTSI_MAX_TAPS], oh[CTSI_MAX_TAPS], ow[CTSI_MAX_TAPS];
    int NA, NB, NC;
    int ad[4][4], bh[4][4], cw[4][4];
    int8_t pH[4], pW[4];
    int tap_margin[4], ad_min[4];
    int fast, dshift;
    const ConvForm* form;
    int gsplit;
    int ds;
    int head2;
    int planar;
    int ksplit;
    int stem;
    int stream1;
    double flops;
};

static inline ConvFamily conv_family(const ctsi_conv_plan* p) { return p->form ? p->form->family : CONV_GATHER; }
static inline int conv_k32_image(const ctsi_conv_plan* p) { return p->planar ? 3 : p->ds ? 2 : p->d.transposed; }
static inline int conv_k32_direct(const ctsi_conv_plan* p) { return ctsi_conv3_halo_k32_direct(p->form->code, p->ksplit, p->ds); }
static inline size_t head1_bytes(const ctsi_conv_plan* p) {
    return ((size_t)p->Cin * 27 * (p->d.cout <= 8 ? 8 : 16) * 2 + 1024 + 255) / 256 * 256;
}
```

video-to-video-diffusion_amd/csrc/conv_plan.hip:

```cpp
#include "conv_plan.h"
#include <string.h>
#include <stdlib.h>

static const double EFF_HALO32 = 1.0, EFF_HALO32_192 = 0.95, EFF_K32_512 = 1.15, EFF_K32_384 = 1.1, EFF_K32_NARROW = 1.07;
static const double EFF_PICK_W16 = 0.85, EFF_PICK_512 = 1.1, EFF_PICK_512_W16 = 1.0;
static const double EFF_ST_512 = 1.0, EFF_ST_384 = 0.96;
static const double EFF_GATHER_STANDIN = 0.6;

enum FormId { H32_4x2x32, H32_4x4x16, H32_3x4x16, K32_4x4x32, K32_4x8x16, K32_3x4x32, K32_3x8x16, K32_4x4x24, K32_8x4x12, HEAD_4x2x16,
              PL_1x16x32, PL_2x16x16, PL_4x8x16, PL_4x4x24, PL_8x4x12, N_FORMS };
static const ConvForm FORMS[N_FORMS] = {
    {CONV_HALO32, 4, 4, 2, 32, 128, 1, EFF_HALO32, "halo32 4x2x32"},
    {CONV_HALO32, 4, 4, 4, 16, 128, 3, EFF_HALO32, "halo32 4x4x16"},
    {CONV_HALO32, 4, 3, 4, 16, 128, 4, EFF_HALO32_192, "halo32 3x4x16"},
    {CONV_K32, 9, 4, 4, 32, 128, 0, EFF_K32_512, "k32 4x4x32"},
    {CONV_K32, 9, 4, 8, 16, 128, 2, EFF_K32_512, "k32 4x8x16"},
    {CONV_K32, 9, 3, 4, 32, 128, 3, EFF_K32_384, "k32 3x4x32"},
    {CONV_K32, 9, 3, 8, 16, 128, 5, EFF_K32_384, "k32 3x8x16"},
    {CONV_K32, 9, 4, 4, 24, 128, 6, EFF_K32_NARROW, "k32 4x4x24"},
    {CONV_K32, 9, 8, 4, 12, 128, 7, EFF_K32_NARROW, "k32 8x4x12"},
    {CONV_HEAD, 8, 4, 2, 16, 16, 0, 1.0, "head 4x2x16"},
    {CONV_K32, 9, 1, 16, 32, 128, 16, EFF_K32_512, "planar 1x16x32"},
    {CONV_K32, 9, 2, 16, 16, 128, 17, EFF_K32_512, "planar 2x16x16"},
    {CONV_K32, 9, 4, 8, 16, 128, 18, EFF_K32_512, "planar 4x8x16"},
    {CONV_K32, 9, 4, 4, 24, 128, 19, EFF_K32_NARROW, "planar 4x4x24"},
    {CONV_K32, 9, 8, 4, 12, 128, 20, EFF_K32_NARROW, "planar 8x4x12"},
};
static int form_voxels(const ConvForm& f) { return f.td * f.th * f.tw; }
static const ConvForm* k32_sized(const ConvForm* f, bool v384) {
    return &FORMS[f->tw == 16 ? (v384 ? K32_3x8x16 : K32_4x8x16) : (v384 ? K32_3x4x32 : K32_4x4x32)];
}

enum Tri { UNSET = -1, OFF = 0, ON = 1 };
enum SplitK { SK_UNSET, SK_OFF, SK_ON, SK_PLAIN, SK_512 };
struct PlanEnv {
    bool no_halo3, force_halo3, no_c16, no_head3, no_head2, no_fast;
    Tri m512, m512w16, k32_384, k32t, k32d, narrow, narrow_sk, linear;
    int planar;
    int halo_tile;
    int h32w16;
    SplitK splitk;
    int sk384_min, sk512_min;
    bool has_gsplit; int gsplit;
    int tile_bm, tile_bn;
};
static Tri env_tri(const char* name) {
    const char* e = getenv(name);
    return e && !strcmp(e, "0") ? OFF : e && !strcmp(e, "1") ? ON : UNSET;
}
static int env_int(const char* name, int unset) {
    const char* e = getenv(name);
    return e ? atoi(e) : unset;
}
static PlanEnv read_plan_env() {
    PlanEnv e;
    e.no_halo3 = getenv("CTSI_CONV_NO_HALO3") != nullptr;
    e.force_halo3 = getenv("CTSI_CONV_FORCE_HALO3") != nullptr;
    e.no_c16 = getenv("CTSI_CONV_NO_C16") != nullptr;
    e.no_head3 = getenv("CTSI_CONV_NO_HEAD3") != nullptr;
    e.no_head2 = getenv("CTSI_CONV_NO_HEAD2") != nullptr;
    e.no_fast = getenv("CTSI_CONV_NO_FAST") != nullptr;
    e.m512 = env_tri("CTSI_CONV_M512");
    e.m512w16 = env_tri("CTSI_CONV_M512W16");
    e.k32_384 = env_tri("CTSI_CONV_K32_384");
    e.k32t = env_tri("CTSI_CONV_K32T");
    e.k32d = env_tri("CTSI_CONV_K32D");
    {
        const char* pl = getenv("CTSI_CONV_PLANAR");
        e.planar = -1;
        if (pl && (!strcmp(pl, "0") || !strcmp(pl, "1"))) e.planar = pl[0] - '0';
        for (int f = PL_1x16x32; pl && f <= PL_8x4x12; ++f)
            if (!strcmp(pl, FORMS[f].name + 7)) e.planar = FORMS[f].code;
    }
    e.narrow = env_tri("CTSI_CONV_K32_NARROW");
    e.narrow_sk = env_tri("CTSI_CONV_K32_NARROW_SK");
    e.linear = env_tri("CTSI_CONV_LINEAR");
    const char* hv = getenv("CTSI_CONV_HALO_TILE");
    e.halo_tile = hv && !strcmp(hv, "16") ? 16 : hv && !strcmp(hv, "32") ? 32 : 0;
    const char* hw = getenv("CTSI_CONV_H32W16");
    e.h32w16 = hw && !strcmp(hw, "1") ? 1 : hw && !strcmp(hw, "2") ? 2 : 0;
    const char* sk = getenv("CTSI_CONV_K32_SPLITK");
    e.splitk = !sk ? SK_UNSET : !strcmp(sk, "0") ? SK_OFF : !strcmp(sk, "1") ? SK_ON : !strcmp(sk, "plain") ? SK_PLAIN
               : !strcmp(sk, "512") ? SK_512 : SK_UNSET;
    e.sk384_min = env_int("CTSI_CONV_K32_SK384_MIN", 256);
    e.sk512_min = env_int("CTSI_CONV_K32_SK512_MIN", 512);
    const char* gs = getenv("CTSI_CONV_GSPLIT");
    e.has_gsplit = gs != nullptr;
    e.gsplit = gs ? atoi(gs) : 0;
    const char* tile = getenv("CTSI_CONV_TILE");
    e.tile_bm = tile && !strcmp(tile, "128x128") ? 128 : tile && (!strcmp(tile, "256x128") || !strcmp(tile, "256x256")) ? 256 : 0;
    e.tile_bn = tile && !strcmp(tile, "256x256") ? 256 : 128;
    return e;
}

static double cu_rounds(long long b) { return (double)(((b + 255) / 256) * 256); }
static double cu_fill(long long b) { return (double)b / cu_rounds(b); }
static long long plan_rows(const ctsi_conv_plan* p) { return (long long)p->Dr * p->Hr * p->Wr; }
static long long padded_rows(const ctsi_conv_plan* p, const ConvForm& f) {
    return (long long)ceil_div(p->Dr, f.td) * ceil_div(p->Hr, f.th) * ceil_div(p->Wr, f.tw) * form_voxels(f);
}
struct TileFit { long long blocks; double useful, score; };
static TileFit fit(const ctsi_conv_plan* p, const ConvForm& f, int kmul, int classes, double eff) {
    const long long t = (long long)p->d.n * ceil_div(p->Dr, f.td) * ceil_div(p->Hr, f.th) * ceil_div(p->Wr, f.tw);
    TileFit r;
    r.blocks = t * classes * ceil_div(p->d.cout, 128) * kmul;
    r.useful = (double)plan_rows(p) * p->d.n / ((double)t * f.td * f.th * f.tw);
    r.score = r.useful * (double)r.blocks / cu_rounds(r.blocks) * eff;
    return r;
}
static double score(const ctsi_conv_plan* p, FormId f, int kmul, double eff) { return fit(p, FORMS[f], kmul, 1, eff).score; }
static double defended(const ctsi_conv_plan* p) { return fit(p, *p->form, p->ksplit == 2 ? 2 : 1, 1, p->form->eff).score; }

static int ilog2(int v) {
    int l = 0;
    while ((1 << l) < v) ++l;
    return l;
}

static void choose_box_tile(ctsi_conv_plan* p) {
    long long best = -1;
    int bsurf = 0;
    const int lb = ilog2(p->BM);
    for (int lw = 0; lw <= lb; ++lw)
        for (int lh = 0; lh + lw <= lb; ++lh) {
            const int tw = 1 << lw, th = 1 << lh, td = p->BM >> (lw + lh);
            const long long tiles = (long long)ceil_div(p->Dr, td) * ceil_div(p->Hr, th) * ceil_div(p->Wr, tw);
            const int surf = (td + 2) * (th + 2) * (tw + 2);
            if (best < 0 || tiles < best || (tiles == best && surf < bsurf)) {
                best = tiles;
                bsurf = surf;
                p->TD = td; p->TH = th; p->TW = tw;
            }
        }
}

static int plan_geometry(ctsi_conv_plan* p) {
    const ctsi_conv_desc& d = p->d;
    auto unsupported = [](auto... msg) {
        ctsi_set_error(msg...);
        return (int)CTSI_ERR_UNSUPPORTED;
    };
    p->dshift = d.halo_d ? 1 : 0;
    const int di_own = d.di - 2 * p->dshift;
    if (d.halo_d && (d.kd != 3 || d.pd != 1 || di_own < 1))
        return unsupported("ctsi_conv_plan_create: halo_d needs kd=3, pd=1 and di >= 3");
    p->Cin = d.c1 + d.c2;
    p->CinW = p->Cin;
    const int KK = d.kd * d.kh * d.kw;
    if (!d.transposed) {
        p->Do = di_own + 2 * d.pd - d.kd + 1;
        p->Ho = (d.hi + 2 * d.ph - d.kh) / d.sh + 1;
        p->Wo = (d.wi + 2 * d.pw - d.kw) / d.sw + 1;
        if (KK > CTSI_MAX_TAPS || p->Do <= 0 || p->Ho <= 0 || p->Wo <= 0 || d.kd > 3 || d.kh > 4 || d.kw > 4)
            return unsupported("ctsi_conv_plan_create: unsupported Conv3d geometry k=(%d,%d,%d)", d.kd, d.kh, d.kw);
        p->nclass = 1; p->T = KK;
        p->Dr = p->Do; p->Hr = p->Ho; p->Wr = p->Wo;
        p->sH = d.sh; p->sW = d.sw; p->uH = 1; p->uW = 1;
        p->pH[0] = 0; p->pW[0] = 0;
        p->NA = d.kd; p->NB = d.kh; p->NC = d.kw;
        for (int a = 0; a < d.kd; ++a) p->ad[0][a] = a - d.pd;
        for (int b = 0; b < d.kh; ++b) p->bh[0][b] = b - d.ph;
        for (int c = 0; c < d.kw; ++c) p->cw[0][c] = c - d.pw;
        int t = 0;
        for (int a = 0; a < d.kd; ++a)
            for (int b = 0; b < d.kh; ++b)
                for (int c = 0; c < d.kw; ++c, ++t) {
                    p->od[t] = (int8_t)(a - d.pd);
                    p->oh[t] = (int8_t)(b - d.ph);
                    p->ow[t] = (int8_t)(c - d.pw);
                    p->tapk[t] = (a * d.kh + b) * d.kw + c;
                }
        p->flops = 2.0 * d.n * (double)p->Do * p->Ho * p->Wo * p->Cin * d.cout * KK;
    } else {
        if (!(d.sh == 2 && d.sw == 2 && d.kh == 4 && d.kw == 4 && d.ph == 1 && d.pw == 1 && d.kd == 3 && d.pd == 1))
            return unsupported("ctsi_conv_plan_create: ConvTranspose3d supports k=(3,4,4) s=(1,2,2) p=1 only");
        p->Do = di_own; p->Ho = d.hi * 2; p->Wo = d.wi * 2;
        p->nclass = 4; p->T = 12;
        p->Dr = di_own; p->Hr = d.hi; p->Wr = d.wi;
        p->sH = 1; p->sW = 1; p->uH = 2; p->uW = 2;
        for (int cls = 0; cls < 4; ++cls) {
            const int py = cls >> 1, px = cls & 1;
            p->pH[cls] = (int8_t)py; p->pW[cls] = (int8_t)px;
            const int ky[2] = {py == 0 ? 1 : 2, py == 0 ? 3 : 0};
            const int oy[2] = {0, py == 0 ? -1 : 1};
            const int kx[2] = {px == 0 ? 1 : 2, px == 0 ? 3 : 0};
            const int ox[2] = {0, px == 0 ? -1 : 1};
            p->NA = 3; p->NB = 2; p->NC = 2;
            for (int a = 0; a < 3; ++a) p->ad[cls][a] = 1 - a;
            for (int b = 0; b < 2; ++b) { p->bh[cls][b] = oy[b]; p->cw[cls][b] = ox[b]; }
            int t = cls * 12;
            for (int a = 0; a < 3; ++a)
                for (int b = 0; b < 2; ++b)
                    for (int c = 0; c < 2; ++c, ++t) {
                        p->od[t] = (int8_t)(1 - a);
                        p->oh[t] = (int8_t)oy[b];
                        p->ow[t] = (int8_t)ox[c];
                        p->tapk[t] = (a * 4 + ky[b]) * 4 + kx[c];
                    }
        }
        p->flops = 2.0 * d.n * (double)di_own * d.hi * d.wi * p->Cin * d.cout * KK;
    }
    for (int t = 0; t < p->nclass * p->T; ++t)
        p->tapdelta[t] = (p->od[t] * d.hi + p->oh[t]) * d.wi + p->ow[t];
    for (int c = 0; c < p->nclass; ++c) {
        int mn = 0, dmin = 0;
        for (int t = 0; t < p->T; ++t) {
            if (p->tapdelta[c * p->T + t] < mn) mn = p->tapdelta[c * p->T + t];
            if (p->od[c * p->T + t] < dmin) dmin = p->od[c * p->T + t];
        }
        p->tap_margin[c] = -mn;
        p->ad_min[c] = dmin;
    }
    return CTSI_OK;
}

static void plan_k_walk(ctsi_conv_plan* p) {
    if (p->Cin <= 32 && (p->Cin & (p->Cin - 1)) == 0) {
        p->small = 1;
        p->lcpt = ilog2(p->Cin / 8);
        p->ksteps = ceil_div(p->T << p->lcpt, 8);
    } else {
        p->kc_per_tap = ceil_div(p->Cin, 64);
        p->ksteps = p->T * p->kc_per_tap;
    }
    p->Ktot = p->ksteps * CTSI_BK;
}

static void choose_gather_tile(ctsi_conv_plan* p, const PlanEnv& e) {
    const ctsi_conv_desc& d = p->d;
    const long long rows = d.n * plan_rows(p) * p->nclass;
    p->BM = 128; p->BN = d.cout <= 32 ? 32 : 128;
    if (d.cout <= 32) return;
    const long long wg_256x256 = (rows / 256) * ceil_div(d.cout, 256);
    const long long wg_256x128 = (rows / 256) * ceil_div(d.cout, 128);
    if (d.cout >= 256 && d.cout % 256 == 0 && wg_256x256 >= 640) {
        p->BM = 256; p->BN = 256;
    } else if (wg_256x128 >= 640) {
        p->BM = 256; p->BN = 128;
    }
    if (e.tile_bm && (e.tile_bn != 256 || d.cout % 256 == 0)) { p->BM = e.tile_bm; p->BN = e.tile_bn; }
}

static bool halo_fits(const ctsi_conv_plan* p) {
    return 8.0 * p->d.hi * p->d.wi * (p->d.c1 > p->d.c2 ? p->d.c1 : p->d.c2) * 2.0 < 2.0e9;
}
static bool is_k3(const ctsi_conv_desc& d) {
    return !d.transposed && d.kd == 3 && d.kh == 3 && d.kw == 3 && d.sh == 1 && d.sw == 1 && d.pd == 1 && d.ph == 1 && d.pw == 1;
}
static bool covers_70(const ctsi_conv_plan* p, FormId f) { return plan_rows(p) * 10 >= padded_rows(p, FORMS[f]) * 7; }
static bool narrow_fits(const ctsi_conv_plan* p, const ConvForm& f) { return p->Wr % f.tw == 0 && p->Wr % 16 != 0; }
static bool splitk_channels(const ctsi_conv_plan* p) { return p->Cin % 128 == 0 && p->d.c1 % 16 == 0 && p->d.c2 % 16 == 0; }

static void choose_k3_form(ctsi_conv_plan* p, const PlanEnv& e) {
    const ctsi_conv_desc& d = p->d;
    const bool c32 = !p->small && d.c1 % 32 == 0 && d.c2 % 32 == 0;
    const bool c16 = d.c1 % 16 == 0 && d.c2 % 16 == 0 && !e.no_c16;
    if (!((c32 || c16) && d.cout >= 64 && d.cout % 8 == 0 && halo_fits(p) && !e.no_halo3)) return;
    if (covers_70(p, H32_4x4x16) || e.force_halo3) {
        const double s16 = score(p, H32_4x4x16, 1, EFF_PICK_W16), s32 = score(p, H32_4x2x32, 1, EFF_HALO32),
                     s512 = score(p, K32_4x4x32, 1, EFF_PICK_512);
        const double s512w = e.m512w16 == OFF ? 0.0 : score(p, K32_4x8x16, 1, EFF_PICK_512_W16);
        enum { W16, W32, M512 } pick = s16 >= s32 && s16 >= s512 ? W16 : (s32 >= s512 ? W32 : M512);
        bool use_w16 = (s512w > s16 && s512w > s32 && s512w > s512) || e.m512w16 == ON;
        if (e.halo_tile == 16) pick = W16;
        if (e.halo_tile == 32 && pick == W16) pick = s32 >= s512 ? W32 : M512;
        if (e.m512 == OFF && pick == M512) pick = W32;
        if (e.m512 == ON && pick != W16) pick = M512;
        if (!c32 && pick != M512) {
            pick = M512;
            use_w16 = s512w > s512;
        }
        if (use_w16 && (!c32 || (e.halo_tile != 16 && e.m512 != OFF))) {
            p->form = &FORMS[K32_4x8x16];
        } else if (pick == M512) {
            p->form = &FORMS[K32_4x4x32];
        } else if (pick == W16) {
            const bool t192 = score(p, H32_3x4x16, 1, EFF_HALO32_192) > score(p, H32_4x4x16, 1, EFF_HALO32);
            p->form = &FORMS[(e.h32w16 ? e.h32w16 == 2 : t192) ? H32_3x4x16 : H32_4x4x16];
        } else {
            p->form = &FORMS[H32_4x2x32];
        }
        const bool use384 = e.k32_384 == UNSET ? score(p, K32_3x4x32, 1, EFF_K32_384) > defended(p) : e.k32_384 == ON;
        if (use384) p->form = &FORMS[K32_3x4x32];
        const bool sk_ok = splitk_channels(p);
        bool use_sk = sk_ok && p->Cin >= e.sk384_min && score(p, K32_3x8x16, 2, EFF_K32_384) > defended(p);
        if (e.splitk == SK_OFF) use_sk = false;
        if (e.splitk == SK_ON && sk_ok) use_sk = true;
        const long long b512 = fit(p, FORMS[K32_4x4x32], 1, 1, 1.0).blocks;
        const bool sk512 = sk_ok && p->Cin >= e.sk512_min && p->Wr % 32 == 0 && p->Hr % 4 == 0 && p->Dr % 4 == 0 &&
                           cu_fill(b512) < 0.8 && cu_fill(2 * b512) >= 0.95 && e.splitk != SK_OFF;
        if ((e.splitk == SK_512 && sk_ok) || (sk512 && e.splitk != SK_ON && e.splitk != SK_PLAIN)) {
            p->form = &FORMS[K32_4x4x32];
            p->ksplit = 2;
        } else if (use_sk || e.splitk == SK_PLAIN) {
            p->form = &FORMS[K32_3x8x16];
            p->ksplit = use_sk ? 2 : 1;
        }
    }
    const double cur = p->form ? defended(p) : EFF_GATHER_STANDIN;
    const bool nsk_ok = splitk_channels(p) && e.narrow_sk != OFF;
    for (const FormId c : {K32_4x4x24, K32_8x4x12}) {
        if (e.narrow == OFF || !narrow_fits(p, FORMS[c])) continue;
        const double s1 = score(p, c, 1, EFF_K32_NARROW), s2 = nsk_ok ? score(p, c, 2, EFF_K32_NARROW) : 0.0;
        const bool sk2 = nsk_ok && (e.narrow_sk == ON || (p->Cin >= e.sk384_min && s2 > 1.1 * s1));
        if (e.narrow == ON || (sk2 ? s2 : s1) > 1.05 * cur) {
            p->form = &FORMS[c];
            p->ksplit = sk2 ? 2 : 0;
            break;
        }
    }
}

static void choose_k32_strided_form(ctsi_conv_plan* p, const PlanEnv& e) {
    const ctsi_conv_desc& d = p->d;
    const bool ds = !d.transposed;
    if (!(d.kd == 3 && d.kh == 4 && d.kw == 4 && d.sh == 2 && d.sw == 2 && d.pd == 1 && d.ph == 1 && d.pw == 1 && d.c2 == 0 &&
          d.c1 % 16 == 0 && d.cout >= 64 && d.cout % 8 == 0 && halo_fits(p) && (!ds || (d.hi % 2 == 0 && d.wi % 2 == 0))))
        return;
    const ConvForm* best = nullptr;
    TileFit bf = {0, 0.0, -1.0};
    for (int fi = K32_4x4x32; fi <= K32_8x4x12; ++fi) {
        const ConvForm& c = FORMS[fi];
        if (c.tw % 16 != 0 && (!narrow_fits(p, c) || e.narrow == OFF)) continue;
        const TileFit f = fit(p, c, 1, ds ? 1 : 4, form_voxels(c) == 512 ? EFF_ST_512 : EFF_ST_384);
        if (ds && f.useful < 0.7 && !e.force_halo3) continue;
        if (f.score > bf.score) { best = &c; bf = f; }
    }
    if (!(bf.useful >= 0.7 || e.force_halo3) || (ds ? e.k32d : e.k32t) == OFF || e.no_halo3) return;
    p->form = best;
    p->ds = ds;
    if (e.m512w16 != UNSET) p->form = &FORMS[e.m512w16 == ON ? K32_4x8x16 : K32_4x4x32];
    if (e.k32_384 != UNSET) p->form = k32_sized(p->form, e.k32_384 == ON);
    if (ds) {
        const long long t5 = fit(p, FORMS[K32_3x8x16], 1, 1, 1.0).blocks;
        bool use_sk = p->Cin % 32 == 0 && p->Cin >= 256 && bf.blocks <= 160 && 2 * t5 <= 512;
        if (e.splitk == SK_OFF) use_sk = false;
        if (e.splitk == SK_ON && p->Cin % 32 == 0) use_sk = true;
        if (use_sk) {
            p->form = &FORMS[K32_3x8x16];
            p->ksplit = 2;
        }
    }
}

static void choose_planar_form(ctsi_conv_plan* p, const PlanEnv& e) {
    const ctsi_conv_desc& d = p->d;
    if (!(!d.transposed && d.kd == 1 && d.kh == 3 && d.kw == 3 && d.sh == 1 && d.sw == 1 && d.pd == 0 && d.ph == 1 && d.pw == 1 &&
          !p->dshift && d.c1 % 16 == 0 && d.c2 % 16 == 0 && d.cout >= 64 && d.cout % 8 == 0 && halo_fits(p)))
        return;
    if (e.planar == 0 || e.no_halo3) return;
    const ConvForm* best = nullptr;
    TileFit bf = {0, 0.0, -1.0};
    for (int f = PL_1x16x32; f <= PL_8x4x12; ++f) {
        const ConvForm& c = FORMS[f];
        if (c.tw % 16 != 0 && !narrow_fits(p, c)) continue;
        if (e.planar >= 16 && c.code != e.planar) continue;
        const TileFit t = fit(p, c, 1, 1, c.eff);
        if (t.useful < 0.7 && e.planar < 16) continue;
        if (t.score > bf.score) { best = &c; bf = t; }
    }
    if (!best) return;
    if (e.planar < 1 && bf.blocks <= 128 && p->Cin >= 256) return;
    p->form = best;
    p->planar = 1;
}

static void choose_head_form(ctsi_conv_plan* p, const PlanEnv& e) {
    const ctsi_conv_desc& d = p->d;
    if (p->form || !is_k3(d) || p->small || d.c2 != 0 || d.c1 % 32 != 0 || d.cout > 16 || !halo_fits(p) || e.no_head3) return;
    if (!covers_70(p, HEAD_4x2x16) && !e.force_halo3) return;
    p->form = &FORMS[HEAD_4x2x16];
    p->head2 = ctsi_conv3_head2_supported(p->Cin, d.cout) && !e.no_head2;
}

static void finish_tiles(ctsi_conv_plan* p) {
    p->CoutPad = ceil_div(p->d.cout, p->BN) * p->BN;
    p->ntiles_n = p->CoutPad / p->BN;
    p->lTH = ilog2(p->TH); p->lTW = ilog2(p->TW);
    p->tilesD = ceil_div(p->Dr, p->TD);
    p->tilesH = ceil_div(p->Hr, p->TH);
    p->tilesW = ceil_div(p->Wr, p->TW);
    p->tps = p->tilesD * p->tilesH * p->tilesW;
    p->mtiles = p->d.n * p->tps;
}

static void choose_linear_rows(ctsi_conv_plan* p, const PlanEnv& e) {
    const long long rows = plan_rows(p), boxed = (long long)p->tps * p->BM;
    if (!((boxed * 100 > rows * 115 && e.linear != OFF) || e.linear == ON)) return;
    p->linear = 1;
    p->tps = (int)((rows + p->BM - 1) / p->BM);
    p->mtiles = p->d.n * p->tps;
    p->TD = (int)(p->BM / ((long long)p->Hr * p->Wr)) + 2;
}

static void choose_gather_split(ctsi_conv_plan* p, const PlanEnv& e) {
    if (p->small || p->BM != 128 || p->BN != 128) return;
    const long long blocks = (long long)p->nclass * p->mtiles * p->ntiles_n;
    int S = 0;
    if (blocks * 2 <= 256 && p->ksteps >= 32) {
        S = (int)(256 / blocks);
        if (S > 4) S = 4;
        while (S > 1 && p->ksteps / S < 16) --S;
    } else if (blocks <= 256 && p->ksteps >= 64) {
        S = 2;
    }
    if (e.has_gsplit) S = e.gsplit >= 2 && e.gsplit <= 8 && p->ksteps >= e.gsplit ? e.gsplit : 0;
    p->gsplit = S >= 2 ? S : 0;
}

extern "C" int ctsi_conv_plan_create(ctsi_conv_plan** out, const ctsi_conv_desc* desc) {
    CTSI_CHECK_ARG(out && desc, "ctsi_conv_plan_create: null argument");
    const ctsi_conv_desc& d = *desc;
    CTSI_CHECK_ARG(d.n > 0 && d.c1 > 0 && d.c2 >= 0 && d.cout > 0 && d.di > 0 && d.hi > 0 && d.wi > 0,
                   "ctsi_conv_plan_create: bad sizes n=%d c1=%d c2=%d cout=%d in=%dx%dx%d", d.n, d.c1,
                   d.c2, d.cout, d.di, d.hi, d.wi);
    CTSI_CHECK_ARG(d.c1 % 8 == 0 && d.c2 % 8 == 0,
                   "ctsi_conv_plan_create: source channel counts must be multiples of 8 (got %d, %d); "
                   "pad the tensor at the layout boundary", d.c1, d.c2);
    CTSI_CHECK_ARG(d.kd >= 1 && d.kh >= 1 && d.kw >= 1 && d.sh >= 1 && d.sw >= 1,
                   "ctsi_conv_plan_create: bad kernel/stride");
    ctsi_conv_plan* p = (ctsi_conv_plan*)calloc(1, sizeof(ctsi_conv_plan));
    CTSI_CHECK_ARG(p, "ctsi_conv_plan_create: out of host memory");
    p->d = d;
    const int rc = plan_geometry(p);
    if (rc != CTSI_OK) {
        free(p);
        return rc;
    }
    const PlanEnv e = read_plan_env();
    plan_k_walk(p);
    choose_gather_tile(p, e);
    if (is_k3(d)) choose_k3_form(p, e);
    else if (d.kd == 1 && d.kh == 3) choose_planar_form(p, e);
    else choose_k32_strided_form(p, e);
    choose_head_form(p, e);
    if (p->form) {
        p->BM = form_voxels(*p->form);
        p->BN = p->form->bn;
        p->TD = p->form->td; p->TH = p->form->th; p->TW = p->form->tw;
    } else {
        choose_box_tile(p);
    }
    finish_tiles(p);
    if (!p->form) choose_linear_rows(p, e);
    {
        const int cmax = d.c1 > d.c2 ? d.c1 : d.c2;
        const double extent = ((double)(p->TD + 4) * d.hi * d.wi + 2.0 * d.wi + 8) * cmax * 2.0;
        p->fast = !p->small && d.c1 % 64 == 0 && d.c2 % 64 == 0 && extent < 2.0e9 && !e.no_fast;
    }
    if (!p->form) choose_gather_split(p, e);
    *out = p;
    return CTSI_OK;
}

extern "C" void ctsi_conv_plan_destroy(ctsi_conv_plan* plan) { free(plan); }

extern "C" int ctsi_conv_plan_out_dims(const ctsi_conv_plan* p, int* d, int* h, int* w) {
    CTSI_CHECK_ARG(p, "ctsi_conv_plan_out_dims: null plan");
    if (d) *d = p->Do;
    if (h) *h = p->Ho;
    if (w) *w = p->Wo;
    return CTSI_OK;
}
extern "C" size_t ctsi_conv_plan_weight_bytes(const ctsi_conv_plan* p) {
    if (!p) return 0;
    if (p->stem) return ctsi_conv3_stem_weight_bytes(p->CoutPad);
    if (p->stream1) return (size_t)p->d.cout * p->Cin * 2;
    switch (conv_family(p)) {
    case CONV_HEAD:
        return head1_bytes(p) + (ctsi_conv3_head2_supported(p->Cin, p->d.cout) ? ctsi_conv3_head2_weight_bytes(p->d.cout) : 0);
    case CONV_K32: return ctsi_conv3_halo_k32_weight_bytes(p->Cin, p->CoutPad, p->BN, conv_k32_image(p));
    case CONV_HALO32: return (size_t)p->Cin * 27 * p->CoutPad * 2;
    default: return (size_t)p->nclass * p->CoutPad * p->Ktot * 2;
    }
}
extern "C" int ctsi_conv_plan_tiles(const ctsi_conv_plan* p) { return p ? p->nclass * p->mtiles : 0; }
extern "C" int ctsi_conv_plan_tiles_per_sample(const ctsi_conv_plan* p) { return p ? p->tps : 0; }
extern "C" int ctsi_conv_plan_cout_pad(const ctsi_conv_plan* p) { return p ? p->CoutPad : 0; }
extern "C" double ctsi_conv_plan_flops(const ctsi_conv_plan* p) { return p ? p->flops : 0.0; }
extern "C" size_t ctsi_conv_plan_workspace_bytes(const ctsi_conv_plan* p) {
    if (p && !p->form && p->gsplit >= 2) {
        const size_t tiles = (size_t)p->nclass * p->mtiles * p->ntiles_n;
        return (tiles * 4 + 255) / 256 * 256 + tiles * p->gsplit * (size_t)(128 * 128) * sizeof(float);
    }
    if (!p || p->ksplit != 2) return 0;
    return ctsi_conv3_halo_k32_splitk_bytes(p->mtiles * p->ntiles_n);
}
extern "C" int ctsi_conv_plan_config(const ctsi_conv_plan* p, int* bm, int* bn, int* mode) {
    CTSI_CHECK_ARG(p, "ctsi_conv_plan_config: null plan");
    if (bm) *bm = p->stream1 ? 16 : p->BM;
    if (bn) *bn = p->stream1 ? p->stream1 * 16 : p->BN;
    if (mode) *mode = p->stem ? 11 : p->stream1 ? 10 : (p->form ? p->form->mode : (p->small ? 1 : (p->fast ? 2 : 0)));
    return CTSI_OK;
}

extern "C" int ctsi_conv_plan_form(const ctsi_conv_plan* p, int out[8]) {
    CTSI_CHECK_ARG(p && out, "ctsi_conv_plan_form: null argument");
    memset(out, 0, 8 * sizeof(int));
    out[0] = p->TD; out[1] = p->TH; out[2] = p->TW;
    if (!p->stem && !p->stream1) out[3] = conv_family(p) == CONV_K32 ? p->ksplit : (p->form ? 0 : p->gsplit);
    out[4] = (p->linear ? 1 : 0) | (p->fast ? 2 : 0) | (p->head2 ? 4 : 0) | (p->ds ? 8 : 0) | (p->planar ? 16 : 0);
    return CTSI_OK;
}

extern "C" int ctsi_conv_plan_pack_layout(const ctsi_conv_plan* p) {
    if (!p) return 0;
    if (p->stem) return CTSI_PACK_STEM;
    if (p->stream1) return CTSI_PACK_STREAM_TAIL | (p->stream1 << 8);
    switch (conv_family(p)) {
    case CONV_K32: return CTSI_PACK_K32 | (conv_k32_image(p) << 4) | (conv_k32_direct(p) << 6) | ((p->BN / 16) << 8);
    case CONV_HEAD: return CTSI_PACK_HEAD | (ctsi_conv3_head2_supported(p->Cin, p->d.cout) ? 1 << 4 : 0);
    case CONV_HALO32: return CTSI_PACK_HALO;
    default: return p->small ? CTSI_PACK_GATHER_SMALL : CTSI_PACK_GATHER;
    }
}

extern "C" int ctsi_conv_plan_set_stream_tail(ctsi_conv_plan* p, int on) {
    CTSI_CHECK_ARG(p, "ctsi_conv_plan_set_stream_tail: null plan");
    p->stream1 = 0;
    if (!on || ctsi_conv1_stream_switch() == 0) return CTSI_OK;
    const ctsi_conv_desc& d = p->d;
    if (d.transposed || d.kd != 1 || d.kh != 1 || d.kw != 1 || d.sh != 1 || d.sw != 1 || d.pd || d.ph || d.pw || p->dshift)
        return CTSI_OK;
    p->stream1 = ctsi_conv1_stream_nt(d.c1, d.c2, d.cout);
    return CTSI_OK;
}

extern "C" int ctsi_conv_plan_set_weight_cin(ctsi_conv_plan* p, int cin_w) {
    CTSI_CHECK_ARG(p && cin_w > 0 && cin_w <= p->Cin, "ctsi_conv_plan_set_weight_cin: bad cin %d", cin_w);
    p->CinW = cin_w;
    const ctsi_conv_desc& d = p->d;
    if (cin_w == 1 && is_k3(d) && d.c2 == 0 && d.c1 == 8 && d.cout >= 64 && d.cout % 8 == 0 && !p->dshift &&
        !getenv("CTSI_CONV_NO_STEM")) {
        p->stem = 1;
        p->form = nullptr;
        p->gsplit = 0; p->linear = 0;
        p->BM = 512; p->BN = 128;
        ctsi_conv3_stem_tile(&p->TD, &p->TH, &p->TW);
        finish_tiles(p);
    }
    return CTSI_OK;
}
```

video-to-video-diffusion_amd/csrc/ctsi_internal.h:

```cpp
#pragma once
#include <hip/hip_runtime.h>
#include <stdint.h>
#include <stdio.h>
#include <stdarg.h>
#include "../../include/ctsi.h"

typedef uint16_t bf16_t;

typedef __attribute__((ext_vector_type(8))) short bf16x8;
typedef __attribute__((ext_vector_type(4))) float f32x4;
typedef __attribute__((ext_vector_type(16))) float f32x16;

void ctsi_set_error(const char* fmt, ...);

#define CTSI_CHECK_ARG(cond, ...)            \
    do {                                     \
        if (!(cond)) {                       \
            ctsi_set_error(__VA_ARGS__);     \
            return CTSI_ERR_INVALID;         \
        }                                    \
    } while (0)

struct CtsiPerDeviceOnce {
    bool done[64] = {};
    bool first() {
        int d = 0;
        if (hipGetDevice(&d) != hipSuccess || d < 0 || d >= 64) return true;
        if (done[d]) return false;
        done[d] = true;
        return true;
    }
};

#define CTSI_HIP(call)                                                                  \
    do {                                                                                \
        hipError_t e_ = (call);                                                         \
        if (e_ != hipSuccess) {                                                         \
            ctsi_set_error("%s failed: %s (%s:%d)", #call, hipGetErrorString(e_),       \
                           __FILE__, __LINE__);                                         \
            return CTSI_ERR_HIP;                                                        \
        }                                                                               \
    } while (0)

#define CTSI_LAUNCH_CHECK()                                                             \
    do {                                                                                \
        hipError_t e_ = hipGetLastError();                                              \
        if (e_ != hipSuccess) {                                                         \
            ctsi_set_error("kernel launch failed: %s (%s:%d)", hipGetErrorString(e_),   \
                           __FILE__, __LINE__);                                         \
            return CTSI_ERR_HIP;                                                        \
        }                                                                               \
    } while (0)

#ifdef CTSI_ABLATE
#define CTSI_DBG(flags, bit) ((flags) & (bit))
#define CTSI_DBG_MASK (~0)
#else
#define CTSI_DBG(flags, bit) (((bit) == 4096) ? ((flags) & 4096) : 0)
#define CTSI_DBG_MASK 4096
#endif
#define CTSI_DBG_RT(flags, bit) ((flags) & (bit))
int ctsi_debug_flags();
int ctsi_debug_ksteps(int n);

__device__ __forceinline__ float bf16_to_f32(bf16_t v) {
    return __uint_as_float(((uint32_t)v) << 16);
}
__device__ __forceinline__ bf16_t f32_to_bf16(float f) {
    __bf16 b = (__bf16)f;
    return *reinterpret_cast<bf16_t*>(&b);
}
__device__ __forceinline__ uint32_t pack_bf16x2(float lo, float hi) {
    return (uint32_t)f32_to_bf16(lo) | ((uint32_t)f32_to_bf16(hi) << 16);
}
__device__ __forceinline__ float silu_f(float x) {
    return x * __builtin_amdgcn_rcpf(1.0f + __builtin_amdgcn_exp2f(-1.4426950408889634f * x));
}

typedef float f32x2_t __attribute__((ext_vector_type(2)));
typedef __bf16 bf16x2_t __attribute__((ext_vector_type(2)));
__device__ __forceinline__ f32x2_t silu2_f(f32x2_t x) {
    f32x2_t t = x * -1.4426950408889634f;
    t.x = __builtin_amdgcn_exp2f(t.x);
    t.y = __builtin_amdgcn_exp2f(t.y);
    t = 1.0f + t;
    t.x = __builtin_amdgcn_rcpf(t.x);
    t.y = __builtin_amdgcn_rcpf(t.y);
    return x * t;
}
__device__ __forceinline__ uint32_t pack_bf16x2_v(f32x2_t v) {
    const bf16x2_t b = __builtin_convertvector(v, bf16x2_t);
    return *reinterpret_cast<const uint32_t*>(&b);
}

__device__ __forceinline__ float nan_to_num_f(float v) {
    if (v != v) return 0.0f;
    if (v == __builtin_inff()) return 1.0f;
    if (v == -__builtin_inff()) return -1.0f;
    return v;
}

static inline int ceil_div(int a, int b) { return (a + b - 1) / b; }

struct Conv3HaloParams {
    const bf16_t* x1;
    const bf16_t* x2;
    const bf16_t* w;
    const float* bias;
    void* y;
    float* colsum;
    int C1, C2;
    int Di, Hi, Wi;
    int Do, Ho, Wo;
    int dshift;
    int tilesD, tilesH, tilesW, tps, mtiles, ntiles_n;
    int nchunks;
    int Cout, CoutPad;
    int cout_stride, c_off;
    int n_major;
    int dbg;
    const double* nin_sums;
    const float* nin_gamma;
    const float* nin_beta;
    const float* nin_tbias;
    const int* nin_step_ptr;
    int nin_tb_stride, nin_groups, nin_silu, nin_n_total;
    int nin_pad_lo, nin_pad_hi;
    float nin_eps;
    double nin_count;
    int ksplit;
    float* sk_ws;
    int* sk_sync;
    int tr;
    int ds;
    int tile_order;
    int nt_store;
    int dbg_epi_barrier;
};

extern "C" int ctsi_conv3_halo_pack(const float* w, void* packed, int cout, int cout_pad, int cin, int cin_w,
                                    void* stream);
extern "C" int ctsi_conv3_halo_launch(const Conv3HaloParams* hp, int wide, void* stream);
extern "C" int ctsi_conv3_head_launch(const Conv3HaloParams* hp, int rows, int out_mode, int act, long long sn, long long sc,
                                      long long sd, long long sh, long long sw, void* stream);
extern "C" int ctsi_conv3_head2_supported(int cin, int cout);
extern "C" size_t ctsi_conv3_head2_weight_bytes(int cout);
extern "C" int ctsi_conv3_head2_pack(const float* w, void* packed, int cout, int cin, int cin_w, void* stream);
extern "C" int ctsi_conv3_head2_launch(const Conv3HaloParams* hp, int n, const void* packed, int out_mode, int act, long long sn,
                                       long long sc, long long sd, long long sh, long long sw, void* stream);
struct StemParams {
    const bf16_t* x;
    const bf16_t* w;
    const float* bias;
    bf16_t* y;
    float* colsum;
    int cx, D, H, W;
    int Cout, CoutPad, cout_stride, c_off;
    int tilesD, tilesH, tilesW, tps, mtiles;
};
extern "C" void ctsi_conv3_stem_tile(int* td, int* th, int* tw);
extern "C" size_t ctsi_conv3_stem_weight_bytes(int cout_pad);
extern "C" int ctsi_conv3_stem_pack(const float* w, void* packed, int cout, int cout_pad, int cin_w, void* stream);
extern "C" int ctsi_conv3_stem_launch(const StemParams* q, void* stream);

struct Conv1StreamParams {
    const bf16_t* x1;
    const bf16_t* x2;
    const bf16_t* w;
    const float* bias;
    const bf16_t* h;
    bf16_t* y;
    const double* gn_sums;
    const float* gn_gamma;
    const float* gn_beta;
    int gn_groups, gn_silu;
    float gn_eps;
    double gn_count;
    int C1, C2, Cout, cout_stride, c_off;
    long long V;
    int tiles;
    int P;
};
extern "C" int ctsi_conv1_stream_switch();
extern "C" int ctsi_conv1_stream_nt(int c1, int c2, int cout);
extern "C" int ctsi_conv1_stream_pack(const float* w, void* packed, int cout, int cin, int cin_w, int nt, void* stream);
extern "C" int ctsi_conv1_stream_launch(Conv1StreamParams* q, int n, int nt, void* stream);
extern "C" size_t ctsi_conv3_halo_k32_weight_bytes(int cin, int cout_pad, int bn, int transposed);
extern "C" int ctsi_conv3_halo_k32_pack(const float* w, void* packed, int cout, int cout_pad, int cin, int cin_w, int bn,
                                        int transposed, int direct, void* stream);
extern "C" int ctsi_conv3_halo_k32_direct(int tile, int ksplit, int ds);
extern "C" size_t ctsi_conv3_halo_k32_splitk_bytes(int tiles);
extern "C" int ctsi_conv3_halo_k32_launch(const Conv3HaloParams* hp, int tile, int bn, void* stream);
extern "C" int ctsi_conv3_planar_k32_launch(const Conv3HaloParams* hp, int tile, int relu, void* stream);
```

video-to-video-diffusion_amd/lib.py:

```python
from __future__ import annotations

import ctypes as C
import os
import subprocess
from pathlib import Path

_PKG_DIR = Path(__file__).resolve().parent
LIB_PATH = _PKG_DIR / "libctsi.so"
CSRC_DIR = _PKG_DIR / "csrc"
HEADER_PATH = _PKG_DIR.parent / "include" / "ctsi.h"


class CtsiError(RuntimeError):
    """Raised when libctsi is unavailable or one of its entry points reports an error."""


class ConvDesc(C.Structure):
    _fields_ = [
        ("transposed", C.c_int),
        ("kd", C.c_int), ("kh", C.c_int), ("kw", C.c_int),
        ("sh", C.c_int), ("sw", C.c_int),
        ("pd", C.c_int), ("ph", C.c_int), ("pw", C.c_int),
        ("n", C.c_int), ("c1", C.c_int), ("c2", C.c_int),
        ("cout", C.c_int),
        ("di", C.c_int), ("hi", C.c_int), ("wi", C.c_int),
        ("halo_d", C.c_int),
    ]


class ConvOut(C.Structure):
    _fields_ = [
        ("y", C.c_void_p),
        ("mode", C.c_int),
        ("cout_stride", C.c_int),
        ("c_off", C.c_int),
        ("sn", C.c_longlong), ("sc", C.c_longlong), ("sd", C.c_longlong),
        ("sh", C.c_longlong), ("sw", C.c_longlong),
        ("act", C.c_int),
        ("colsum", C.c_void_p),
        ("gn_x", C.c_void_p), ("gn_sums", C.c_void_p), ("gn_gamma", C.c_void_p), ("gn_beta", C.c_void_p),
        ("gn_groups", C.c_int), ("gn_eps", C.c_float), ("gn_count", C.c_longlong), ("gn_silu", C.c_int),
        ("workspace", C.c_void_p),
    ]


class WgradDesc(C.Structure):
    _fields_ = [
        ("kd", C.c_int), ("kh", C.c_int), ("kw", C.c_int),
        ("sh", C.c_int), ("sw", C.c_int),
        ("pd", C.c_int), ("ph", C.c_int), ("pw", C.c_int),
        ("n", C.c_int),
        ("dr", C.c_int), ("hr", C.c_int), ("wr", C.c_int),
        ("dg", C.c_int), ("hg", C.c_int), ("wg", C.c_int),
        ("cr", C.c_int), ("cr_stride", C.c_int),
        ("cg", C.c_int), ("cg_stride", C.c_int),
    ]


_vp, _i, _f, _ll, _sz = C.c_void_p, C.c_int, C.c_float, C.c_longlong, C.c_size_t
_ip = C.POINTER(C.c_int)

SIGNATURES = {
    "ctsi_version": (_i, [], False),
    "ctsi_ablation_build": (_i, [], False),
    "ctsi_last_error": (C.c_char_p, [], False),
    "ctsi_device_available": (_i, [], False),
    "ctsi_ncdhw_f32_to_ndhwc_bf16": (_i, [_vp, _vp, _i, _i, _i, _i, _i, _i, _i, _vp], True),
    "ctsi_ndhwc_bf16_to_ncdhw_f32": (_i, [_vp, _vp, _i, _i, _i, _i, _i, _vp], True),
    "ctsi_ncdhw_f32_to_ndhwc_f32": (_i, [_vp, _vp, _i, _i, _i, _i, _i, _vp], True),
    "ctsi_ndhwc_f32_to_ncdhw_f32": (_i, [_vp, _vp, _i, _i, _i, _i, _i, _vp], True),
    "ctsi_conv_plan_create": (_i, [C.POINTER(_vp), C.POINTER(ConvDesc)], True),
    "ctsi_conv_plan_set_weight_cin": (_i, [_vp, _i], True),
    "ctsi_conv_plan_set_stream_tail": (_i, [_vp, _i], True),
    "ctsi_conv_plan_destroy": (None, [_vp], False),
    "ctsi_conv_plan_out_dims": (_i, [_vp, _ip, _ip, _ip], True),
    "ctsi_conv_plan_weight_bytes": (_sz, [_vp], False),
    "ctsi_conv_plan_workspace_bytes": (_sz, [_vp], False),
    "ctsi_conv_plan_tiles": (_i, [_vp], False),
    "ctsi_conv_plan_tiles_per_sample": (_i, [_vp], False),
    "ctsi_conv_plan_cout_pad": (_i, [_vp], False),
    "ctsi_conv_plan_flops": (C.c_double, [_vp], False),
    "ctsi_conv_plan_config": (_i, [_vp, _ip, _ip, _ip], True),
    "ctsi_conv_plan_pack_layout": (_i, [_vp], False),
    "ctsi_conv_plan_form": (_i, [_vp, _ip], True),
    "ctsi_conv_plan_pack_weights": (_i, [_vp, _vp, _vp, _vp], True),
    "ctsi_conv_fwd": (_i, [_vp, _vp, _vp, _vp, _vp, C.POINTER(ConvOut), _vp], True),
    "ctsi_gn_colsum": (_i, [_vp, _vp, _i, _i, _i, _i, _i, _ip, _vp], True),
    "ctsi_gn_colsum_tiles": (_i, [_i, _i, _i], False),
    "ctsi_gn_finalize": (_i, [_vp, _vp, _i, _i, _i, _i, _i, _i, _i, _vp], True),
    "ctsi_gn_apply": (_i, [_vp, _vp, _vp, _vp, _vp, _i, _i, _i, _i, _i, _i, _i, _f, _i, _vp, _i, _vp, _vp,
                           _i, _vp], True),
    "ctsi_attn_depthsum": (_i, [_vp, _vp, _vp, _i, _i, _i, _i, _i, _vp], True),
    "ctsi_attn_depthsum_tiles": (_i, [_i, _i, _i], False),
    "ctsi_attn_normsum": (_i, [_vp, _vp, _vp, _vp, _vp, _i, _i, _i, _i, _i, _i, _f, _vp], True),
    "ctsi_attn_pv_supported": (_i, [_i, _i], False),
    "ctsi_attn_pv": (_i, [_vp, _vp, _vp, _vp, _vp, _vp, _vp, _i, _i, _i, _i, _i, _i, _f, _vp], True),
    "ctsi_attn_broadcast_add": (_i, [_vp, _vp, _vp, _i, _vp, _i, _i, _i, _i, _i, _vp], True),
    "ctsi_attn_softmax_rowsum": (_i, [_vp, _vp, _i, _i, _i, _i, _i, _i, _vp], True),
    "ctsi_attn_core": (_i, [_vp, _vp, _i, _i, _i, _i, _i, _i, _vp], True),
    "ctsi_attn_core_bwd": (_i, [_vp, _vp, _vp, _i, _i, _i, _i, _i, _i, _vp], True),
    "ctsi_attn_plane": (_i, [_vp, _vp, _vp, _i, _i, _i, _i, _i, _i, _vp], True),
    "ctsi_attn_plane_bwd": (_i, [_vp, _vp, _vp, _vp, _vp, _i, _i, _i, _i, _i, _i, _vp], True),
    "ctsi_time_embed_fwd": (_i, [_vp, _i, _i, _i, _vp, _vp, _vp, _vp, _vp, _vp, _i, _vp, _vp, _vp], True),
    "ctsi_time_embed_fwd_tf": (_i, [_vp, _i, _i, _i, _vp, _vp, _vp, _vp, _vp, _vp, _i, _vp, _vp, _vp], True),
    "ctsi_trilinear_depth_fwd": (_i, [_vp, _vp, _i, _i, _i, _i, _i, _i, _i, _i, _vp, _vp], True),
    "ctsi_ddim_step": (_i, [_vp, _vp, _vp, _vp, _i, _i, _vp, _vp, _i, _i, _i, _i, _i, _vp, _vp], True),
    "ctsi_ddpm_step": (_i, [_vp, _vp, _vp, _vp, _i, _i, _vp, _vp, _i, _i, _i, _i, _i, _vp], True),
    "ctsi_ddpm_posterior": (_i, [_vp, _vp, _vp, _vp, _vp, _vp, _i, _ll, _i, _vp], True),
    "ctsi_step_advance": (_i, [_vp, _vp], True),
    "ctsi_nan_to_num_f32": (_i, [_vp, _ll, _vp], True),
    "ctsi_count_nonfinite_f32": (_i, [_vp, _ll, _i, _vp, _vp], True),
    "ctsi_wgrad_workspace_bytes": (_sz, [C.POINTER(WgradDesc)], False),
    "ctsi_wgrad_flops": (C.c_double, [C.POINTER(WgradDesc)], False),
    "ctsi_wgrad": (_i, [C.POINTER(WgradDesc), _vp, _vp, _vp, _sz, _vp, _ll, _ll, _ll, _f, _vp], True),
    "ctsi_weight_dgrad_layout": (_i, [_vp, _vp, _i, _i, _i, _i, _i, _vp], True),
    "ctsi_linear_wgrad_multi": (_i, [_vp, _vp, _i, _vp], True),
    "ctsi_gn_bwd_tiles": (_i, [_i, _i, _i], False),
    "ctsi_gn_bwd_workspace_floats": (_sz, [_i, _i, _i, _i, _i, _i], False),
    "ctsi_gn_bwd": (_i, [_vp, _vp, _i, _vp, _vp, _vp, _i, _i, _i, _i, _i, _i, _f, _i, _vp, _i, _vp, _vp, _vp, _vp,
                         _vp, _vp, _vp, _ll, _vp, _vp], True),
    "ctsi_channel_sum_workspace_floats": (_sz, [_ll, _i], False),
    "ctsi_channel_sum": (_i, [_vp, _ll, _i, _i, _vp, _vp, _f, _vp], True),
    "ctsi_add_bf16": (_i, [_vp, _vp, _ll, _vp], True),
    "ctsi_f32_to_bf16": (_i, [_vp, _vp, _ll, _vp], True),
    "ctsi_vae_head_grad": (_i, [_vp, _vp, _i, _i, _i, _i, _i, _f, _i, _vp, _i, _vp], True),
    "ctsi_thin_wgrad_workspace_bytes": (_sz, [_i, _i, _i, _i, _i], False),
    "ctsi_thin_wgrad_supported": (_i, [_i, _i, _i, _i, _i], False),
    "ctsi_thin_wgrad": (_i, [_vp, _i, _i, _vp, _i, _i, _i, _i, _i, _i, _i, _i, _i, _vp, _sz, _vp, _f, _vp], True),
    "ctsi_q_sample": (_i, [_vp, _vp, _vp, _vp, _vp, _vp, _i, _i, _i, _i, _i, _i, _i, _vp], True),
    "ctsi_mse_loss_workspace_doubles": (_sz, [_i], False),
    "ctsi_mse_loss_fwd": (_i, [_vp, _vp, _vp, _vp, _i, _i, _i, _i, _i, _vp, _vp, _vp], True),
    "ctsi_mse_loss_bwd": (_i, [_vp, _vp, _vp, _vp, _vp, _i, _i, _i, _i, _i, _vp, _i, _vp], True),
    "ctsi_time_embed_train_fwd": (_i, [_vp, _i, _i, _i, _vp, _vp, _vp, _vp, _vp, _vp, _i, _vp, _vp, _vp], True),
    "ctsi_linear_bwd": (_i, [_vp, _vp, _vp, _i, _i, _i, _i, _vp, _vp, _vp, _vp], True),
    "ctsi_blend_accumulate": (_i, [_vp, _vp, _vp, _vp, _vp, _vp, _i, _i, _i, _i, _i, _i, _i, _i, _i, _i, _vp], True),
    "ctsi_blend_normalize": (_i, [_vp, _vp, _ll, _vp], True),
    "ctsi_slice_metrics_workspace_doubles": (_sz, [_i, _i, _i, _i, _i], False),
    "ctsi_slice_metrics": (_i, [_vp, _vp, _i, _i, _i, _i, _i, _i, _f, _vp, _vp, _vp], True),
    "ctsi_comm_unique_id": (_i, [_vp], True),
    "ctsi_comm_init": (_i, [C.POINTER(_vp), _vp, _i, _i], True),
    "ctsi_comm_destroy": (None, [_vp], False),
    "ctsi_comm_rank": (_i, [_vp], False),
    "ctsi_comm_world": (_i, [_vp], False),
    "ctsi_halo_exchange": (_i, [_vp, _vp, _vp, _vp, _vp, _sz, _vp], True),
    "ctsi_halo_exchange_reduce": (_i, [_vp, _vp, _vp, _vp, _vp, _sz, _vp, _i, _vp, _ll, _vp], True),
    "ctsi_gn_allreduce": (_i, [_vp, _vp, _i, _vp, _ll, _vp], True),
    "ctsi_comm_allgather": (_i, [_vp, _vp, _vp, _sz, _vp], True),
    "ctsi_memset_async": (_i, [_vp, _i, _sz, _vp], True),
    "ctsi_adamw_chunk_elems": (_i, [], False),
    "ctsi_adamw_multi": (_i, [_vp, _vp, _vp, _i, _vp], True),
    "ctsi_copy_scale_multi": (_i, [_vp, _vp, _i, _vp], True),
    "ctsi_ema_multi": (_i, [_vp, _vp, _vp, _i, _vp], True),
    "ctsi_swap_multi": (_i, [_vp, _vp, _i, _vp], True),
    "ctsi_grad_norm_multi": (_i, [_vp, _vp, _i, _vp, _vp], True),
    "ctsi_grad_norm_finalize": (_i, [_vp, _i, _f, _vp, _vp], True),
    "ctsi_grad_scale_multi": (_i, [_vp, _vp, _i, _vp, _vp], True),
    "ctsi_adamw_ema_multi": (_i, [_vp, _vp, _vp, _i, _vp, _vp, _vp], True),
    "ctsi_msssim_workspace_bytes": (_sz, [_i, _i, _i, _i, _i], False),
    "ctsi_msssim_fwd": (_i, [_vp, _vp, _i, _i, _i, _i, _i, _vp, _vp, _vp], True),
    "ctsi_msssim_bwd": (_i, [_vp, _vp, _i, _i, _i, _i, _vp, _vp, _vp, _vp], True),
    "ctsi_vgg_prep": (_i, [_vp, _vp, _vp, _vp, _i, _i, _i, _i, _i, _vp], True),
    "ctsi_vgg_prep_bwd": (_i, [_vp, _vp, _vp, _vp, _i, _i, _i, _i, _i, _vp], True),
    "ctsi_maxpool2_fwd": (_i, [_vp, _vp, _i, _i, _i, _i, _vp], True),
    "ctsi_maxpool2_bwd": (_i, [_vp, _vp, _vp, _i, _i, _i, _i, _vp], True),
    "ctsi_relu_bf16": (_i, [_vp, _ll, _vp], True),
    "ctsi_feat_loss_blocks": (_i, [], False),
    "ctsi_feat_loss_fwd": (_i, [_vp, _vp, _ll, _i, _vp, _vp], True),
    "ctsi_feat_loss_finalize": (_i, [_vp, _vp, _i, _vp, _vp], True),
    "ctsi_feat_grad_relu_bwd": (_i, [_vp, _vp, _vp, _vp, _ll, _f, _i, _i, _vp, _vp], True),
    "ctsi_lpips_blocks": (_i, [], False),
    "ctsi_lpips_prep": (_i, [_vp, _vp, _i, _i, _i, _i, _i, _vp], True),
    "ctsi_lpips_prep_bwd": (_i, [_vp, _vp, _i, _i, _i, _i, _i, _vp], True),
    "ctsi_lpips_dist_fwd": (_i, [_vp, _vp, _vp, _i, _ll, _i, _vp, _vp], True),
    "ctsi_lpips_finalize": (_i, [_vp, _vp, _i, _i, _vp, _vp, _vp], True),
    "ctsi_lpips_grad_relu_bwd": (_i, [_vp, _vp, _vp, _vp, _vp, _i, _ll, _i, _vp, _vp], True),
    "ctsi_device_error_status": (_i, [C.POINTER(C.c_uint), C.POINTER(C.c_uint), _i], True),
    "ctsi_conv_f32_supported": (_i, [C.POINTER(ConvDesc)], False),
    "ctsi_conv_f32_weight_bytes": (_sz, [C.POINTER(ConvDesc)], False),
    "ctsi_conv_f32_flops": (C.c_double, [C.POINTER(ConvDesc)], False),
    "ctsi_conv_f32_geometry": (_i, [C.POINTER(ConvDesc), _ip, _ip, _ip, _ip, _ip, _ip], True),
    "ctsi_conv_f32_pack_weights": (_i, [C.POINTER(ConvDesc), _vp, _vp, _vp], True),
    "ctsi_conv_f32_fwd": (_i, [C.POINTER(ConvDesc), _vp, _vp, _vp, _vp, _vp, C.POINTER(ConvOut), _vp], True),
    "ctsi_conv_bf16x3_supported": (_i, [C.POINTER(ConvDesc)], False),
    "ctsi_conv_bf16x3_weight_bytes": (_sz, [C.POINTER(ConvDesc)], False),
    "ctsi_conv_bf16x3_flops": (C.c_double, [C.POINTER(ConvDesc)], False),
    "ctsi_conv_bf16x3_geometry": (_i, [C.POINTER(ConvDesc), _ip, _ip, _ip, _ip, _ip, _ip], True),
    "ctsi_conv_bf16x3_pack_weights": (_i, [C.POINTER(ConvDesc), _vp, _vp, _vp], True),
    "ctsi_conv_bf16x3_fwd": (_i, [C.POINTER(ConvDesc), _vp, _vp, _vp, _vp, _vp, C.POINTER(ConvOut), _vp], True),
    "ctsi_gn_colsum_f32_tiles": (_i, [_i, _i, _i], False),
    "ctsi_gn_colsum_f32": (_i, [_vp, _vp, _i, _i, _i, _i, _i, _ip, _vp], True),
    "ctsi_gn_apply_f32": (_i, [_vp, _vp, _vp, _vp, _vp, _i, _i, _i, _i, _i, _i, _i, _f, _i, _vp, _i, _vp, _vp,
                               _i, _vp], True),
    "ctsi_gn_apply_mod": (_i, [_vp, _vp, _vp, _vp, _vp, _i, _i, _i, _i, _i, _i, _i, _f, _i, _vp, _i, _vp, _vp,
                               _i, _i, _i, _f, _vp, _i, _vp], True),
    "ctsi_gn_apply_mod_f32": (_i, [_vp, _vp, _vp, _vp, _vp, _i, _i, _i, _i, _i, _i, _i, _f, _i, _vp, _i, _vp, _vp,
                                   _i, _i, _vp], True),
    "ctsi_gn_bwd_mod_workspace_floats": (_sz, [_i, _i, _i, _i, _i, _i], False),
    "ctsi_gn_bwd_mod": (_i, [_vp, _vp, _vp, _vp, _vp, _i, _i, _i, _i, _i, _i, _f, _vp, _i, _i, _i, _f, _vp, _i, _vp,
                             _vp, _vp, _vp, _vp, _ll, _vp, _vp], True),
    "ctsi_dropout_mask": (_i, [_vp, _i, _i, _ll, _vp, _vp], True),
    "ctsi_dropout_mask_host": (_i, [C.c_ulonglong, _i, _i, _ll, _vp], True),
    "ctsi_philox4x32_10_host": (_i, [_vp, _vp, _vp], True),
    "ctsi_attn_depthsum_f32_tiles": (_i, [_i, _i], False),
    "ctsi_attn_depthsum_f32": (_i, [_vp, _vp, _vp, _i, _i, _i, _i, _i, _vp], True),
    "ctsi_attn_normsum_f32": (_i, [_vp, _vp, _vp, _vp, _vp, _i, _i, _i, _i, _i, _i, _f, _vp], True),
    "ctsi_attn_broadcast_add_f32": (_i, [_vp, _vp, _vp, _i, _i, _i, _i, _i, _vp], True),
    "ctsi_ddim_step_f32": (_i, [_vp, _vp, _vp, _vp, _i, _i, _vp, _vp, _i, _i, _i, _i, _i, _vp, _vp], True),
    "ctsi_ddpm_step_f32": (_i, [_vp, _vp, _vp, _vp, _i, _i, _vp, _vp, _i, _i, _i, _i, _i, _vp], True),
    "ctsi_dpm_step": (_i, [_vp, _vp, _vp, _vp, _i, _i, _vp, _vp, _i, _i, _i, _i, _i, _vp, _vp], True),
    "ctsi_dpm_step_f32": (_i, [_vp, _vp, _vp, _vp, _i, _i, _vp, _vp, _i, _i, _i, _i, _i, _vp, _vp], True),
    "ctsi_heun_step": (_i, [_vp, _vp, _vp, _vp, _vp, _i, _i, _vp, _vp, _i, _i, _i, _i, _i, _vp, _vp], True),
    "ctsi_heun_step_f32": (_i, [_vp, _vp, _vp, _vp, _vp, _i, _i, _vp, _vp, _i, _i, _i, _i, _i, _vp, _vp], True),
    "ctsi_cfg_stats_blocks": (_i, [_ll], False),
    "ctsi_cfg_combine": (_i, [_vp, _vp, _vp, _vp, _i, _i, _i, _i, _i, _vp], True),
    "ctsi_cfg_stats": (_i, [_vp, _vp, _vp, _vp, _i, _i, _i, _i, _i, _vp], True),
    "ctsi_cfg_stats_finalize": (_i, [_vp, _vp, _i, _i, _i, _i, _i, _vp], True),
    "ctsi_cfg_mirror": (_i, [_vp, _vp, _ll, _i, _i, _vp], True),
    "ctsi_pred_to_eps": (_i, [_vp, _vp, _vp, _vp, _vp, _i, _i, _i, _ll, _vp], True),
    "ctsi_q_sample_v": (_i, [_vp, _vp, _vp, _vp, _vp, _vp, _vp, _i, _i, _i, _i, _i, _i, _i, _vp], True),
    "ctsi_x0_step": (_i, [_vp, _vp, _vp, _vp, _vp, _i, _i, _vp, _vp, _i, _i, _i, _i, _i, _vp, _vp], True),
    "ctsi_x0_step_f32": (_i, [_vp, _vp, _vp, _vp, _vp, _i, _i, _vp, _vp, _i, _i, _i, _i, _i, _vp, _vp], True),
    "ctsi_sigma_split": (_i, [_vp, _vp, _vp, _i, _i, _i, _i, _i, _i, _vp], True),
    "ctsi_ddpm_lv_step": (_i, [_vp, _vp, _vp, _vp, _vp, _i, _i, _vp, _vp, _i, _i, _i, _i, _i, _vp], True),
    "ctsi_ddpm_lv_step_f32": (_i, [_vp, _vp, _vp, _vp, _vp, _i, _i, _vp, _vp, _i, _i, _i, _i, _i, _vp], True),
    "ctsi_ddpm_posterior_lv": (_i, [_vp, _vp, _vp, _vp, _vp, _vp, _vp, _i, _ll, _vp], True),
    "ctsi_window_gather": (_i, [_vp, _vp, _vp] + [_i] * 12 + [_vp], True),
    "ctsi_window_gather_f32": (_i, [_vp, _vp, _vp] + [_i] * 12 + [_vp], True),
    "ctsi_window_blend": (_i, [_vp, _vp, _vp, _vp] + [_i] * 15 + [_vp], True),
    "ctsi_hybrid_loss_workspace_doubles": (_sz, [_i], False),
    "ctsi_hybrid_loss_fwd": (_i, [_vp, _vp, _vp, _vp, _vp, _i, _i, _vp, _vp, _vp, _i, _i, _i, _i, _i, _vp, _vp, _vp], True),
    "ctsi_hybrid_loss_bwd": (_i, [_vp, _vp, _vp, _vp, _vp, _i, _i, _vp, _vp, _vp, _vp, _i, _i, _i, _i, _i, _vp, _i, _vp],
                             True),
    "ctsi_z0_pred": (_i, [_vp, _vp, _vp, _i, _vp, _vp, _vp, _vp, _i, _i, _i, _i, _i, _i, _vp, _vp], True),
    "ctsi_loss_bwd_z0": (_i, [_vp, _vp, _vp, _vp, _vp, _vp, _vp, _vp, _i, _i, _i, _i, _i, _vp, _i, _vp], True),
    "ctsi_depth_measure": (_i, [_vp, _vp, _vp, _vp, _i, _i, _i, _i, _vp], True),
    "ctsi_depth_measure_adj": (_i, [_vp, _vp, _vp, _vp, _f, _i, _i, _i, _i, _i, _vp], True),
    "ctsi_depth_project": (_i, [_vp, _vp, _vp, _vp, _vp, _vp, _i, _f, _f, _i, _vp, _i, _i, _i, _i, _vp], True),
    "ctsi_depth_project_blocks": (_i, [_i, _i], False),
    "ctsi_depth_project_finalize": (_i, [_vp, _vp, _i, _i, _i, _vp], True),
    "ctsi_ensemble_accumulate": (_i, [_vp, _i, _ll, _i, _vp, _vp, _vp], True),
    "ctsi_ensemble_blocks": (_i, [_i, _ll], False),
    "ctsi_ensemble_finalize": (_i, [_vp, _vp, _i, _i, _i, _ll, _vp, _vp, _vp], True),
    "ctsi_ensemble_calibration": (_i, [_vp, _vp, _vp, _i, _ll, _vp, _vp, _vp], True),
    "ctsi_guide_z0": (_i, [_vp, _vp, _f, _f, _i, _f, _vp, _i, _i, _i, _i, _i, _vp], True),
    "ctsi_depth_residual_adj": (_i, [_vp, _vp, _vp, _vp, _vp, _vp, _vp, _i, _i, _i, _i, _i, _vp], True),
    "ctsi_guide_apply": (_i, [_vp, _vp, _vp, _vp, _f, _f, _i, _vp, _i, _i, _i, _i, _i, _i, _i, _vp], True),
    "ctsi_graph_begin_capture": (_i, [_vp], True),
    "ctsi_graph_end_capture": (_i, [_vp, C.POINTER(_vp)], True),
    "ctsi_graph_launch": (_i, [_vp, _vp], True),
    "ctsi_graph_destroy": (None, [_vp], False),
    "ctsi_event_create": (_i, [C.POINTER(_vp)], True),
    "ctsi_event_record": (_i, [_vp, _vp], True),
    "ctsi_stream_wait_event": (_i, [_vp, _vp], True),
    "ctsi_event_elapsed_ms": (_i, [_vp, _vp, C.POINTER(C.c_float)], True),
    "ctsi_event_destroy": (None, [_vp], False),
}


def build(force: bool = False) -> Path:
    if force:
        subprocess.run(["make", "-C", str(CSRC_DIR), "clean"], check=True, capture_output=True)
    proc = subprocess.run(["make", "-C", str(CSRC_DIR), "-j4"], capture_output=True, text=True)
    if proc.returncode != 0 or not LIB_PATH.exists():
        raise CtsiError("building libctsi.so failed:\n" + proc.stdout[-4000:] + proc.stderr[-4000:])
    return LIB_PATH


class _Lib:
    def __init__(self, path: Path):
        if not path.exists():
            raise CtsiError(
                f"{path} is missing: build it with `python -c 'import __graft_entry__ as g; g.build()'` "
                f"or `make -C {CSRC_DIR}`.  There is no CPU fallback for the HIP engine.")
        try:
            self._dll = C.CDLL(str(path))
        except OSError as exc:
            raise CtsiError(f"cannot load {path}: {exc}") from exc
        self.raw = {}
        for name, (restype, argtypes, status) in SIGNATURES.items():
            try:
                fn = getattr(self._dll, name)
            except AttributeError as exc:
                raise CtsiError(f"{path} does not export {name}") from exc
            fn.restype = restype
            fn.argtypes = argtypes
            self.raw[name] = fn
            setattr(self, name[len("ctsi_"):], self._checked(name, fn) if status else fn)

    def _checked(self, name, fn):
        last_error = self._dll.ctsi_last_error
        last_error.restype = C.c_char_p

        def call(*args):
            rc = fn(*args)
            if rc != 0:
                msg = last_error()
                raise CtsiError(f"{name} failed (rc={rc}): {msg.decode() if msg else '?'}")
            return rc

        call.__name__ = name
        return call


_LIB = None


def get_lib() -> _Lib:
    global _LIB
    if _LIB is None:
        _LIB = _Lib(Path(os.environ.get("CTSI_LIB", LIB_PATH)))
    return _LIB
```

Measured before the change: 40.39 steps/s.

## Assign weight prefetch to four feeder waves in k32 halo conv pipeline

New measurement: 40.59 steps/s, median of 6. About the same (+0.5%).

```diff
diff --git a/include/ctsi.h b/include/ctsi.h
--- a/include/ctsi.h
+++ b/include/ctsi.h
@@ -229,6 +229,9 @@
                     const float* grad_loss, float* grad_pred, void* stream);
 
 int ctsi_device_error_status(unsigned int* count, unsigned int* detail, int reset);
+
+int ctsi_k32_issue_schedule(int taps, int ups, int npiece, int halo_instr, int need, int nchunks, int feed, int* out, int cap);
+int ctsi_k32_wait_max(void);
 
 int ctsi_conv_f32_supported(const ctsi_conv_desc* desc);
 size_t ctsi_conv_f32_weight_bytes(const ctsi_conv_desc* desc);
diff --git a/video-to-video-diffusion_amd/csrc/conv3_halo_k32.hip b/video-to-video-diffusion_amd/csrc/conv3_halo_k32.hip
--- a/video-to-video-diffusion_amd/csrc/conv3_halo_k32.hip
+++ b/video-to-video-diffusion_amd/csrc/conv3_halo_k32.hip
@@ -1,4 +1,5 @@
 #include "conv3_halo_common.h"
+#include "conv3_halo_k32_sched.h"
 #include <stdlib.h>
 #include <type_traits>
 
@@ -36,7 +37,21 @@
     static constexpr int a_imm(int i) { return (((16 * i) / TW) * HW + (16 * i) % TW) * 32; }
 };
 
+template <int MAXC>
 __device__ __forceinline__ void hk_wait_vm(int allowed) {
+    if constexpr (MAXC <= 7) {
+        switch (allowed) {
+            case 0: asm volatile("s_waitcnt vmcnt(0) lgkmcnt(0)" ::: "memory"); break;
+            case 1: asm volatile("s_waitcnt vmcnt(1) lgkmcnt(0)" ::: "memory"); break;
+            case 2: asm volatile("s_waitcnt vmcnt(2) lgkmcnt(0)" ::: "memory"); break;
+            case 3: asm volatile("s_waitcnt vmcnt(3) lgkmcnt(0)" ::: "memory"); break;
+            case 4: asm volatile("s_waitcnt vmcnt(4) lgkmcnt(0)" ::: "memory"); break;
+            case 5: asm volatile("s_waitcnt vmcnt(5) lgkmcnt(0)" ::: "memory"); break;
+            case 6: asm volatile("s_waitcnt vmcnt(6) lgkmcnt(0)" ::: "memory"); break;
+            default: asm volatile("s_waitcnt vmcnt(7) lgkmcnt(0)" ::: "memory"); break;
+        }
+        return;
+    }
     switch (allowed) {
         case 0: asm volatile("s_waitcnt vmcnt(0) lgkmcnt(0)" ::: "memory"); break;
         case 1: asm volatile("s_waitcnt vmcnt(1) lgkmcnt(0)" ::: "memory"); break;
@@ -45,7 +60,14 @@
         case 4: asm volatile("s_waitcnt vmcnt(4) lgkmcnt(0)" ::: "memory"); break;
         case 5: asm volatile("s_waitcnt vmcnt(5) lgkmcnt(0)" ::: "memory"); break;
         case 6: asm volatile("s_waitcnt vmcnt(6) lgkmcnt(0)" ::: "memory"); break;
-        default: asm volatile("s_waitcnt vmcnt(7) lgkmcnt(0)" ::: "memory"); break;
+        case 7: asm volatile("s_waitcnt vmcnt(7) lgkmcnt(0)" ::: "memory"); break;
+        case 8: asm volatile("s_waitcnt vmcnt(8) lgkmcnt(0)" ::: "memory"); break;
+        case 9: asm volatile("s_waitcnt vmcnt(9) lgkmcnt(0)" ::: "memory"); break;
+        case 10: asm volatile("s_waitcnt vmcnt(10) lgkmcnt(0)" ::: "memory"); break;
+        case 11: asm volatile("s_waitcnt vmcnt(11) lgkmcnt(0)" ::: "memory"); break;
+        case 12: asm volatile("s_waitcnt vmcnt(12) lgkmcnt(0)" ::: "memory"); break;
+        case 13: asm volatile("s_waitcnt vmcnt(13) lgkmcnt(0)" ::: "memory"); break;
+        default: asm volatile("s_waitcnt vmcnt(14) lgkmcnt(0)" ::: "memory"); break;
     }
 }
 
@@ -55,14 +77,23 @@
 #define HK_STAMP(K)                                                                                              \
     if ((CTSI_DBG(p.dbg, 4096)) && tid == 0 && blockIdx.x < HK_NSTAMP) g_hk_stamps[blockIdx.x][K] = __builtin_amdgcn_s_memtime();
 
-template <int TD_, int TH_, int TW_ = 32, int BN_ = 128, int UPS_ = 2, bool TR = false, bool SK = false, bool DS = false, bool DIRECT = false>
+#define HK_STEP0 8
+#define HK_NSTEP 32
+#define HK_STEP_BLOCKS 8
+__device__ unsigned long long g_hk_step_stamps[HK_STEP_BLOCKS][4][2 * HK_NSTEP];
+#define HK_STEP_STAMP(WHICH)                                                                                     \
+    if ((CTSI_DBG(p.dbg, 8192)) && (wave & 2) == 0 && lane == 0 && s >= HK_STEP0 && s < HK_STEP0 + HK_NSTEP)     \
+        s_stamp[2 * (s - HK_STEP0) + (WHICH)] = __builtin_amdgcn_s_memtime();
+
+template <int TD_, int TH_, int TW_ = 32, int BN_ = 128, int UPS_ = 2, bool TR = false, bool SK = false, bool DS = false, bool DIRECT = false,
+          int FEED = HK_FEED_SYM>
 __global__ void __attribute__((amdgpu_flat_work_group_size(1, 512)))
 conv3_halo_k32_kernel(const Conv3HaloParams p) {
     constexpr bool PL = false, RELU = false;
 #include "conv3_halo_k32_body.inc"
 }
 
-template <int TD_, int TH_, int TW_, bool RELU>
+template <int TD_, int TH_, int TW_, bool RELU, int FEED = HK_FEED_SYM>
 __global__ void __attribute__((amdgpu_flat_work_group_size(1, 512)))
 conv3_planar_k32_kernel(const Conv3HaloParams p) {
     constexpr int BN_ = 128, UPS_ = 2;
@@ -138,6 +169,80 @@
 #endif
 }
 
+extern "C" int ctsi_conv3_halo_k32_feed(int tile, int ksplit, int ds, int tr) {
+    (void)tile; (void)ksplit; (void)ds; (void)tr;
+    return HK_FEED_W;
+}
+
+extern "C" int ctsi_k32_wait_max(void) { return HK_WAIT_MAX; }
+extern "C" int ctsi_k32_issue_schedule(int taps, int ups, int npiece, int halo_instr, int need, int nchunks, int feed, int* out,
+                                       int cap) {
+    if (!(taps == 27 || taps == 12 || taps == 9) || !(ups == 2 || ups == 4) || npiece < 1 || npiece > 5 || halo_instr < 1 ||
+        halo_instr > 8 * npiece || need < 0 || nchunks < 1 || feed < 0 || feed >= HK_FEED_COUNT || (cap > 0 && !out))
+        return -1;
+    constexpr int NWS = 4, NWAVE = 8;
+    const int step_taps = 2 * ups, Q = nchunks * taps, S = (Q + step_taps - 1) / step_taps;
+    int n = 0;
+    auto rec = [&](int wave, int kind, int a, int b, int pos) {
+        if (n < cap) {
+            int* r = out + 5 * (size_t)n;
+            r[0] = wave; r[1] = kind; r[2] = a; r[3] = b; r[4] = pos;
+        }
+        ++n;
+    };
+    for (int wave = 0; wave < NWAVE; ++wave) {
+        const int lw_n = hk_feed_w_count(feed, wave);
+        const bool lh_own = hk_feed_h_own(feed, wave) != 0, lh_partner = hk_feed_h_partner(feed, wave) != 0;
+        auto issue_halo = [&](int cc, int i, bool partner, int pos) -> int {
+            const int j = wave + (partner ? 4 : 0) + NWAVE * i;
+            if (j >= halo_instr) return 0;
+            rec(wave, 1, cc, j, pos);
+            return 1;
+        };
+        if (wave == 0) rec(wave, 3, 0, 0, -2);
+        for (int k = 0; k < 2 && S > 0; ++k) rec(wave, 0, 0, wave + NWAVE * k, -2);
+        for (int i = 0; i < npiece; ++i) issue_halo(0, i, false, -2);
+        int n_trail = 0;
+        for (int s = 1; s < NWS - 1; ++s)
+            if (s < S) {
+                for (int k = 0; k < 2; ++k) rec(wave, 0, s, wave + NWAVE * k, -2);
+                n_trail += 2;
+            }
+        int n_late = 0;
+        for (int i = 0; i < npiece; ++i) n_late += (wave + NWAVE * i >= need && wave + NWAVE * i < halo_instr) ? 1 : 0;
+        rec(wave, 2, n_trail == 4 ? n_trail + n_late : n_trail, 0, -1);
+        int n_prev = n_trail == 4 ? 2 : 0;
+        int hc = 1, hp = 0, hfree = 0;
+        const int h_first = hk_halo_first(taps, ups, npiece), h_later = hk_halo_later(taps, ups, npiece);
+        for (int s = 0; s < S; ++s) {
+            rec(wave, 2, n_prev, 0, s);
+            int n_halo = 0, n_w = 0;
+            bool urgent = false;
+            if (hc < nchunks && s >= hfree) {
+                urgent = hk_halo_urgent(taps, ups, hc, s) != 0;
+                const int cnt = hp == 0 ? h_first : h_later;
+                for (int k = 0; k < (h_first > h_later ? h_first : h_later); ++k)
+                    if (k < cnt && hp < npiece) {
+                        if (lh_own) n_halo += issue_halo(hc, hp, false, s);
+                        if (lh_partner) n_halo += issue_halo(hc, hp, true, s);
+                        ++hp;
+                    }
+                if (hp >= npiece) {
+                    hp = 0;
+                    hfree = hk_halo_free_step(taps, ups, hc);
+                    ++hc;
+                }
+            }
+            if (s + NWS - 1 < S) {
+                for (int k = 0; k < lw_n; ++k) rec(wave, 0, s + NWS - 1, hk_feed_w_piece(feed, wave, k), s);
+                n_w = lw_n;
+            }
+            n_prev = hk_group_in_flight(urgent, n_w, n_halo);
+        }
+    }
+    return n;
+}
+
 template <int TD, int TH, int TW, int BN, int UPS, bool TR, bool SK = false, bool DS = false>
 static void hk_launch(const Conv3HaloParams* hp, hipStream_t stream) {
     using Cfg = HkCfg<TD, TH, TW, BN, UPS>;
@@ -146,9 +251,15 @@
 #else
     constexpr bool DIRECT = TD * TH * TW == 512 || TW == 24 || TW == 12 || (SK && !DS);
 #endif
-    auto k = conv3_halo_k32_kernel<TD, TH, TW, BN, UPS, TR, SK, DS, DIRECT>;
+    using Kernel = void (*)(const Conv3HaloParams);
+    static const Kernel kernels[HK_FEED_COUNT] = {conv3_halo_k32_kernel<TD, TH, TW, BN, UPS, TR, SK, DS, DIRECT, HK_FEED_SYM>,
+                                                  conv3_halo_k32_kernel<TD, TH, TW, BN, UPS, TR, SK, DS, DIRECT, HK_FEED_W>,
+                                                  conv3_halo_k32_kernel<TD, TH, TW, BN, UPS, TR, SK, DS, DIRECT, HK_FEED_WH>,
+                                                  conv3_halo_k32_kernel<TD, TH, TW, BN, UPS, TR, SK, DS, DIRECT, HK_FEED_WMIRROR>};
     static CtsiPerDeviceOnce attr_once;
-    if (attr_once.first()) hipFuncSetAttribute((const void*)k, hipFuncAttributeMaxDynamicSharedMemorySize, 160 * 1024);
+    if (attr_once.first())
+        for (Kernel k : kernels) hipFuncSetAttribute((const void*)k, hipFuncAttributeMaxDynamicSharedMemorySize, 160 * 1024);
+    const Kernel k = kernels[hp->feed >= 0 && hp->feed < HK_FEED_COUNT ? hp->feed : HK_FEED_SYM];
     hipLaunchKernelGGL(k, dim3((TR ? 4 : 1) * (SK ? 2 : 1) * hp->mtiles * hp->ntiles_n), dim3(Cfg::NTH), Cfg::LDS_BYTES, stream,
                        *hp);
 }
@@ -239,16 +350,19 @@
 template <int TD, int TH, int TW>
 static void hk_launch_planar(const Conv3HaloParams* hp, int relu, hipStream_t stream) {
     using Cfg = HkCfg<TD, TH, TW, 128, 2, true>;
+    using Kernel = void (*)(const Conv3HaloParams);
+    static const Kernel kernels[2][HK_FEED_COUNT] = {
+        {conv3_planar_k32_kernel<TD, TH, TW, false, HK_FEED_SYM>, conv3_planar_k32_kernel<TD, TH, TW, false, HK_FEED_W>,
+         conv3_planar_k32_kernel<TD, TH, TW, false, HK_FEED_WH>, conv3_planar_k32_kernel<TD, TH, TW, false, HK_FEED_WMIRROR>},
+        {conv3_planar_k32_kernel<TD, TH, TW, true, HK_FEED_SYM>, conv3_planar_k32_kernel<TD, TH, TW, true, HK_FEED_W>,
+         conv3_planar_k32_kernel<TD, TH, TW, true, HK_FEED_WH>, conv3_planar_k32_kernel<TD, TH, TW, true, HK_FEED_WMIRROR>}};
     static CtsiPerDeviceOnce attr_once;
-    if (attr_once.first()) {
-        hipFuncSetAttribute((const void*)conv3_planar_k32_kernel<TD, TH, TW, false>, hipFuncAttributeMaxDynamicSharedMemorySize, 160 * 1024);
-        hipFuncSetAttribute((const void*)conv3_planar_k32_kernel<TD, TH, TW, true>, hipFuncAttributeMaxDynamicSharedMemorySize, 160 * 1024);
-    }
+    if (attr_once.first())
+        for (int r = 0; r < 2; ++r)
+            for (Kernel k : kernels[r]) hipFuncSetAttribute((const void*)k, hipFuncAttributeMaxDynamicSharedMemorySize, 160 * 1024);
     const dim3 grid(hp->mtiles * hp->ntiles_n), block(Cfg::NTH);
-    if (relu)
-        hipLaunchKernelGGL((conv3_planar_k32_kernel<TD, TH, TW, true>), grid, block, Cfg::LDS_BYTES, stream, *hp);
-    else
-        hipLaunchKernelGGL((conv3_planar_k32_kernel<TD, TH, TW, false>), grid, block, Cfg::LDS_BYTES, stream, *hp);
+    const int feed = hp->feed >= 0 && hp->feed < HK_FEED_COUNT ? hp->feed : HK_FEED_SYM;
+    hipLaunchKernelGGL(kernels[relu ? 1 : 0][feed], grid, block, Cfg::LDS_BYTES, stream, *hp);
 }
 
 extern "C" int ctsi_conv3_planar_k32_launch(const Conv3HaloParams* hp, int tile, int relu, void* stream) {
@@ -274,6 +388,14 @@
     return CTSI_OK;
 }
 
+extern "C" int ctsi_debug_k32_step_stamps(unsigned long long* out) {
+    CTSI_HIP(hipMemcpyFromSymbol(out, HIP_SYMBOL(g_hk_step_stamps), sizeof(unsigned long long) * HK_STEP_BLOCKS * 4 * 2 * HK_NSTEP));
+    const unsigned long long z[4 * 2 * HK_NSTEP] = {};
+    for (int b = 0; b < HK_STEP_BLOCKS; ++b)
+        CTSI_HIP(hipMemcpyToSymbol(HIP_SYMBOL(g_hk_step_stamps), z, sizeof(z), sizeof(z) * b));
+    return CTSI_OK;
+}
+
 extern "C" int ctsi_device_error_status(unsigned int* count, unsigned int* detail, int reset) {
     CTSI_CHECK_ARG(count, "ctsi_device_error_status: null argument");
     unsigned int h[2] = {0u, 0u};
diff --git a/video-to-video-diffusion_amd/csrc/conv3_halo_k32_body.inc b/video-to-video-diffusion_amd/csrc/conv3_halo_k32_body.inc
--- a/video-to-video-diffusion_amd/csrc/conv3_halo_k32_body.inc
+++ b/video-to-video-diffusion_amd/csrc/conv3_halo_k32_body.inc
@@ -79,11 +79,18 @@
     const int Q = nchunks * TAPS;
     const int S = (Q + STEP_TAPS - 1) / STEP_TAPS;
     const unsigned w_voff = (unsigned)lane * 16u;
-    auto issue_weights = [&](int s) {
+    constexpr bool HAS_WH = FEED == HK_FEED_WH && !(SK && BM == 512);
+    constexpr int feed = (!HAS_WH && FEED == HK_FEED_WH) ? HK_FEED_W : FEED;
+    constexpr int WAIT_MAX = feed == HK_FEED_SYM ? 7 : HK_WAIT_MAX;
+    const int lw_n = hk_feed_w_count(feed, wave), lw_first = hk_feed_w_piece(feed, wave, 0);
+    const int lw_stride = hk_feed_w_piece(feed, wave, 1) - lw_first;
+    const bool lh_own = hk_feed_h_own(feed, wave) != 0, lh_partner = HAS_WH && hk_feed_h_partner(feed, wave) != 0;
+    auto issue_weights = [&](int s, int n, int first, int stride) {
         const unsigned slot = lds0 + OFF_W + (s % NWS) * WSLOT_BYTES;
 #pragma unroll
-        for (int k = 0; k < 2; ++k) {
-            const int piece = wave + NWAVE * k;
+        for (int k = 0; k < 4; ++k) {
+            if (k >= n) break;
+            const int piece = first + stride * k;
             constexpr int PPT = TAP_BYTES / 1024;
             const int e = piece / PPT, quarter = piece % PPT;
             const unsigned soff = (unsigned)__builtin_amdgcn_readfirstlane(((s * STEP_TAPS + e) * CoutPad) * 32 + quarter * 1024);
@@ -98,28 +105,35 @@
         const v4i_t rsb = h3_make_rsrc(p.bias + n0, (unsigned)(left > 0 ? left * 4 : 0));
         h3_dma16(rsb, (unsigned)__builtin_amdgcn_readfirstlane((int)(lds0 + OFF_CS)), (unsigned)lane * 16u, 0u);
     }
-    if (S > 0) issue_weights(0);
-
-    int hrel[NPIECE];
-#pragma unroll
-    for (int i = 0; i < NPIECE; ++i) {
-        const int j = wave + NWAVE * i;
+    if (S > 0) issue_weights(0, 2, wave, NWAVE);
+
+    int hrel[NPIECE], hrelp[HAS_WH ? NPIECE : 1];
+#pragma unroll
+    for (int i = 0; i < (HAS_WH ? NPIECE : 1); ++i) hrelp[i] = -1;
+    auto halo_rel = [&](int j) -> int {
         const int v = j * 32 + (lane >> 1);
         const int hd = v / (HH * HW), rem = v - hd * (HH * HW);
         const int hh = rem / HW, hw = rem - hh * HW;
         const int gd = d0 + p.dshift - DOFF + hd, gh = h0 - 1 + hh, gw = w0 - 1 + hw;
         if (DS) {
             const bool ok = (j < HALO_INSTR) && (v < HV) && gd >= 0 && gd < p.Di && gh >= 0 && gh < p.Ho && gw >= 0 && gw < p.Wo;
-            hrel[i] = ok ? ((gd - dlo) * p.Hi + 2 * gh) * p.Wi + 2 * gw : -1;
+            return ok ? ((gd - dlo) * p.Hi + 2 * gh) * p.Wi + 2 * gw : -1;
         } else {
             const bool ok = (j < HALO_INSTR) && (v < HV) && gd >= 0 && gd < p.Di && gh >= 0 && gh < p.Hi && gw >= 0 && gw < p.Wi;
-            hrel[i] = ok ? ((gd - dlo) * p.Hi + gh) * p.Wi + gw : -1;
-        }
+            return ok ? ((gd - dlo) * p.Hi + gh) * p.Wi + gw : -1;
+        }
+    };
+#pragma unroll
+    for (int i = 0; i < NPIECE; ++i) hrel[i] = halo_rel(wave + NWAVE * i);
+    if (lh_partner) {
+#pragma unroll
+        for (int i = 0; i < (HAS_WH ? NPIECE : 1); ++i) hrelp[i] = halo_rel(wave + 4 + NWAVE * i);
     }
     const unsigned hq16 = (unsigned)((lane & 1) * 16);
 
-    auto issue_halo = [&](int cc, int i) -> int {
-        const int j = wave + NWAVE * i;
+    auto issue_halo = [&](int cc, int i, auto partner_tag) -> int {
+        constexpr bool PARTNER = decltype(partner_tag)::value;
+        const int j = wave + (PARTNER ? 4 : 0) + NWAVE * i;
         if (j >= HALO_INSTR) return 0;
         const int vc = cbase + cc;
         const int ch0 = (DS ? (vc >> 2) : vc) * 16;
@@ -127,10 +141,11 @@
         const bool second = ch0 >= C1;
         const unsigned cbytes = (unsigned)((second ? C2 : C1) * 2);
         const unsigned soff = (unsigned)__builtin_amdgcn_readfirstlane((second ? ch0 - C1 : ch0) * 2);
-        int hsel = hrel[0];
+        if (PARTNER && !HAS_WH) return 0;
+        int hsel = PARTNER ? hrelp[0] : hrel[0];
 #pragma unroll
         for (int q = 1; q < NPIECE; ++q) {
-            int cand = hrel[q];
+            int cand = (PARTNER && HAS_WH) ? hrelp[q] : hrel[q];
             asm("" : "+v"(cand));
             hsel = (i == q) ? cand : hsel;
         }
@@ -228,12 +243,12 @@
     }
 
 #pragma unroll
-    for (int i = 0; i < NPIECE; ++i) issue_halo(0, i);
+    for (int i = 0; i < NPIECE; ++i) issue_halo(0, i, std::false_type{});
     int n_trail = 0;
 #pragma unroll
     for (int s = 1; s < NWS - 1; ++s)
         if (s < S) {
-            issue_weights(s);
+            issue_weights(s, 2, wave, NWAVE);
             n_trail += 2;
         }
     if (tid < BM) {
@@ -255,7 +270,7 @@
 #pragma unroll
         for (int i = 0; i < NPIECE; ++i) n_late += (wave + NWAVE * i >= NEED && wave + NWAVE * i < HALO_INSTR) ? 1 : 0;
     }
-    hk_wait_vm(n_trail == 4 ? n_trail + n_late : n_trail);
+    hk_wait_vm<WAIT_MAX>(n_trail == 4 ? n_trail + n_late : n_trail);
     __syncthreads();
     HK_STAMP(1);
 #pragma unroll
@@ -281,30 +296,31 @@
 
     int n_prev = n_trail == 4 ? 2 : 0;
     int hc = 1, hp = 0, hfree = 0;
-    constexpr int H_FIRST = PL ? NPIECE : (UPS == 2 && !TR && !DS) ? 2 : 3, H_LATER = PL ? NPIECE : (UPS == 2 && !TR && !DS) ? 1 : 3;
+    constexpr int H_FIRST = hk_halo_first(TAPS, UPS, NPIECE), H_LATER = hk_halo_later(TAPS, UPS, NPIECE);
     auto issue_group = [&](int s) {
         int n_halo = 0, n_w = 0;
         bool urgent = false;
         if (hc < nchunks && s >= hfree && !(CTSI_DBG(p.dbg, 1))) {
-            urgent = s + 2 >= ((TAPS * hc) >> 1) / UPS;
+            urgent = hk_halo_urgent(TAPS, UPS, hc, s) != 0;
             const int cnt = hp == 0 ? H_FIRST : H_LATER;
 #pragma unroll
             for (int k = 0; k < (H_FIRST > H_LATER ? H_FIRST : H_LATER); ++k)
                 if (k < cnt && hp < NPIECE) {
-                    n_halo += issue_halo(hc, hp);
+                    if (lh_own) n_halo += issue_halo(hc, hp, std::false_type{});
+                    if (lh_partner) n_halo += issue_halo(hc, hp, std::true_type{});
                     ++hp;
                 }
             if (hp >= NPIECE) {
                 hp = 0;
-                hfree = ((TAPS * hc - 1) >> 1) / UPS;
+                hfree = hk_halo_free_step(TAPS, UPS, hc);
                 ++hc;
             }
         }
         if (s + NWS - 1 < S && !(CTSI_DBG(p.dbg, 2))) {
-            issue_weights(s + NWS - 1);
-            n_w = 2;
-        }
-        n_prev = urgent ? n_w : n_w + n_halo;
+            issue_weights(s + NWS - 1, lw_n, lw_first, lw_stride);
+            n_w = lw_n;
+        }
+        n_prev = hk_group_in_flight(urgent, n_w, n_halo);
         __builtin_amdgcn_sched_barrier(0);
     };
 #define HK_UNIT(FAc, FAn, BADDR, UU, BADDR_N, UU_N, AADDR_N, MID)                                              \
@@ -319,6 +335,8 @@
         HK_MFMA(FAc, fbh, NJH);                                                                                \
         HK_SCHED();                                                                                            \
     }
+    unsigned long long* s_stamp = reinterpret_cast<unsigned long long*>(smem + OFF_CS + wave * (BN * 8) + 512);
+    if (CTSI_DBG(p.dbg, 8192)) s_stamp[lane] = 0ull;
     for (int s = 0; s < S; ++s) {
         const int baddr = b_lane + (s % NWS) * WSLOT_BYTES;
         const int baddr_n = b_lane + ((s + 1) % NWS) * WSLOT_BYTES;
@@ -334,8 +352,10 @@
             HK_UNIT(fa1, fa0, baddr, 1, baddr, 2, an[1], );
             HK_UNIT(fa0, fa1, baddr, 2, baddr, 3, an[2], );
         }
-        hk_wait_vm(n_prev);
+        hk_wait_vm<WAIT_MAX>(n_prev);
+        HK_STEP_STAMP(0);
         if (!(CTSI_DBG(p.dbg, 64))) __builtin_amdgcn_s_barrier();
+        HK_STEP_STAMP(1);
         __builtin_amdgcn_sched_barrier(0);
         HK_UNIT(fa1, fa0, baddr, UPS - 1, baddr_n, 0, an[UPS - 1], if (wave < 4 || (CTSI_DBG(p.dbg, 16))) issue_group(s));
         if (wave >= 4 && !(CTSI_DBG(p.dbg, 16))) issue_group(s);
@@ -347,6 +367,8 @@
 #undef HK_SCHED
     HK_STAMP(2);
     asm volatile("s_waitcnt vmcnt(0) lgkmcnt(0)" ::: "memory");
+    if ((CTSI_DBG(p.dbg, 8192)) && (wave & 2) == 0 && blockIdx.x % 256 == 0 && blockIdx.x / 256 < HK_STEP_BLOCKS)
+        g_hk_step_stamps[blockIdx.x / 256][(wave >> 2) * 2 + (wave & 1)][lane] = s_stamp[lane];
     if (!(DIRECT && !SK) || (p.dbg_epi_barrier != 0)) __syncthreads();
     HK_STAMP(3);
 
diff --git a/video-to-video-diffusion_amd/csrc/conv3_halo_k32_sched.h b/video-to-video-diffusion_amd/csrc/conv3_halo_k32_sched.h
--- /dev/null
+++ b/video-to-video-diffusion_amd/csrc/conv3_halo_k32_sched.h
@@ -0,0 +1,23 @@
+#pragma once
+#if defined(__HIPCC__) || defined(__CUDACC__)
+#define HKS_FN __host__ __device__ constexpr __forceinline__
+#else
+#define HKS_FN static constexpr inline
+#endif
+
+enum { HK_FEED_SYM = 0, HK_FEED_W = 1, HK_FEED_WH = 2, HK_FEED_WMIRROR = 3, HK_FEED_COUNT = 4 };
+#define HK_WAIT_MAX 14
+
+HKS_FN int hk_feed_feeder(int feed, int wave) {
+    return feed == HK_FEED_SYM ? 1 : feed == HK_FEED_WMIRROR ? (wave >= 4) : (wave < 4);
+}
+HKS_FN int hk_feed_w_count(int feed, int wave) { return feed == HK_FEED_SYM ? 2 : hk_feed_feeder(feed, wave) ? 4 : 0; }
+HKS_FN int hk_feed_w_piece(int feed, int wave, int k) { return feed == HK_FEED_SYM ? wave + 8 * k : (wave & 3) + 4 * k; }
+HKS_FN int hk_feed_h_own(int feed, int wave) { return feed != HK_FEED_WH || wave < 4; }
+HKS_FN int hk_feed_h_partner(int feed, int wave) { return feed == HK_FEED_WH && wave < 4; }
+
+HKS_FN int hk_halo_first(int taps, int ups, int npiece) { return taps == 9 ? npiece : (taps == 27 && ups == 2) ? 2 : 3; }
+HKS_FN int hk_halo_later(int taps, int ups, int npiece) { return taps == 9 ? npiece : (taps == 27 && ups == 2) ? 1 : 3; }
+HKS_FN int hk_halo_urgent(int taps, int ups, int hc, int s) { return s + 2 >= ((taps * hc) >> 1) / ups; }
+HKS_FN int hk_halo_free_step(int taps, int ups, int hc) { return ((taps * hc - 1) >> 1) / ups; }
+HKS_FN int hk_group_in_flight(int urgent, int n_w, int n_halo) { return urgent ? n_w : n_w + n_halo; }
diff --git a/video-to-video-diffusion_amd/csrc/conv_mfma.hip b/video-to-video-diffusion_amd/csrc/conv_mfma.hip
--- a/video-to-video-diffusion_amd/csrc/conv_mfma.hip
+++ b/video-to-video-diffusion_amd/csrc/conv_mfma.hip
@@ -835,6 +835,7 @@
             h.tile_order = to ? atoi(to) : 2;
             const char* eb = getenv("CTSI_CONV_EPI_BARRIER");
             h.dbg_epi_barrier = eb ? atoi(eb) : 0;
+            h.feed = p->k32_feed;
         }
         if (family == CONV_HEAD) {
             if (p->head2 && o->colsum == nullptr)
diff --git a/video-to-video-diffusion_amd/csrc/conv_plan.h b/video-to-video-diffusion_amd/csrc/conv_plan.h
--- a/video-to-video-diffusion_amd/csrc/conv_plan.h
+++ b/video-to-video-diffusion_amd/csrc/conv_plan.h
@@ -44,6 +44,7 @@
     int ds;
     int head2;
     int planar;
+    int k32_feed;
     int ksplit;
     int stem;
     int stream1;
diff --git a/video-to-video-diffusion_amd/csrc/conv_plan.hip b/video-to-video-diffusion_amd/csrc/conv_plan.hip
--- a/video-to-video-diffusion_amd/csrc/conv_plan.hip
+++ b/video-to-video-diffusion_amd/csrc/conv_plan.hip
@@ -1,4 +1,5 @@
 #include "conv_plan.h"
+#include "conv3_halo_k32_sched.h"
 #include <string.h>
 #include <stdlib.h>
 
@@ -43,6 +44,7 @@
     int sk384_min, sk512_min;
     bool has_gsplit; int gsplit;
     int tile_bm, tile_bn;
+    int k32_feed;
 };
 static Tri env_tri(const char* name) {
     const char* e = getenv(name);
@@ -90,6 +92,9 @@
     const char* tile = getenv("CTSI_CONV_TILE");
     e.tile_bm = tile && !strcmp(tile, "128x128") ? 128 : tile && (!strcmp(tile, "256x128") || !strcmp(tile, "256x256")) ? 256 : 0;
     e.tile_bn = tile && !strcmp(tile, "256x256") ? 256 : 128;
+    const char* fd = getenv("CTSI_CONV_K32_FEED");
+    e.k32_feed = !fd ? -1 : !strcmp(fd, "sym") ? HK_FEED_SYM : !strcmp(fd, "w") ? HK_FEED_W : !strcmp(fd, "wh") ? HK_FEED_WH
+                 : !strcmp(fd, "w-mirror") ? HK_FEED_WMIRROR : -1;
     return e;
 }
 
@@ -442,6 +447,8 @@
         choose_box_tile(p);
     }
     finish_tiles(p);
+    if (conv_family(p) == CONV_K32)
+        p->k32_feed = e.k32_feed >= 0 ? e.k32_feed : ctsi_conv3_halo_k32_feed(p->form->code, p->ksplit, p->ds, p->d.transposed);
     if (!p->form) choose_linear_rows(p, e);
     {
         const int cmax = d.c1 > d.c2 ? d.c1 : d.c2;
diff --git a/video-to-video-diffusion_amd/csrc/ctsi_internal.h b/video-to-video-diffusion_amd/csrc/ctsi_internal.h
--- a/video-to-video-diffusion_amd/csrc/ctsi_internal.h
+++ b/video-to-video-diffusion_amd/csrc/ctsi_internal.h
@@ -136,6 +136,7 @@
     int tile_order;
     int nt_store;
     int dbg_epi_barrier;
+    int feed;
 };
 
 extern "C" int ctsi_conv3_halo_pack(const float* w, void* packed, int cout, int cout_pad, int cin, int cin_w,
@@ -188,6 +189,7 @@
 extern "C" size_t ctsi_conv3_halo_k32_weight_bytes(int cin, int cout_pad, int bn, int transposed);
 extern "C" int ctsi_conv3_halo_k32_pack(const float* w, void* packed, int cout, int cout_pad, int cin, int cin_w, int bn,
                                         int transposed, int direct, void* stream);
+extern "C" int ctsi_conv3_halo_k32_feed(int tile, int ksplit, int ds, int tr);
 extern "C" int ctsi_conv3_halo_k32_direct(int tile, int ksplit, int ds);
 extern "C" size_t ctsi_conv3_halo_k32_splitk_bytes(int tiles);
 extern "C" int ctsi_conv3_halo_k32_launch(const Conv3HaloParams* hp, int tile, int bn, void* stream);
diff --git a/video-to-video-diffusion_amd/lib.py b/video-to-video-diffusion_amd/lib.py
--- a/video-to-video-diffusion_amd/lib.py
+++ b/video-to-video-diffusion_amd/lib.py
@@ -175,6 +175,8 @@
     "ctsi_lpips_finalize": (_i, [_vp, _vp, _i, _i, _vp, _vp, _vp], True),
     "ctsi_lpips_grad_relu_bwd": (_i, [_vp, _vp, _vp, _vp, _vp, _i, _ll, _i, _vp, _vp], True),
     "ctsi_device_error_status": (_i, [C.POINTER(C.c_uint), C.POINTER(C.c_uint), _i], True),
+    "ctsi_k32_issue_schedule": (_i, [_i, _i, _i, _i, _i, _i, _i, _ip, _i], False),
+    "ctsi_k32_wait_max": (_i, [], False),
     "ctsi_conv_f32_supported": (_i, [C.POINTER(ConvDesc)], False),
     "ctsi_conv_f32_weight_bytes": (_sz, [C.POINTER(ConvDesc)], False),
     "ctsi_conv_f32_flops": (C.c_double, [C.POINTER(ConvDesc)], False),
```
